# Adredes-weslee/elliptic-gnn-project

Measured on AMD Instinct MI355X. Metric: edges/s full-batch SAGE fwd+bwd, Elliptic 203k/234k/166-feat, 1→8 MI355X, higher is better.
Workload: dtype f32; 1 GPU; configs/sage.yaml + symmetrize_edges=true: SAGE 2L 166->128->2, dropout 0.5, full-batch train step (fwd+masked CE+bwd+clip+Adam); global_nodes=203769, global_edges=468710, feats=166, max_nodes_per_gpu=203769, max_edges_per_gpu=468710, parallelism=single, launch=hip-graph replay of the whole step

## Files before the change

elliptic_gnn_project_amd/_lib.py:

```python
from __future__ import annotations

import ctypes
import os
from pathlib import Path

import torch

PKG_DIR = Path(__file__).resolve().parent
LIB_PATH = Path(os.environ["GNNMP_LIB"]) if os.environ.get("GNNMP_LIB") else PKG_DIR / "libgnnmp.so"
ABI_VERSION = 32

DTYPE_F32 = 0
DTYPE_BF16 = 1

MATH_SPLIT_BF16 = 0
MATH_F32 = 1
MATH_HALF_PAIR = 2

PLANES_SPLIT_BF16 = 0
PLANES_HALF_PAIR = 1

GNN_OK = 0
_STATUS_EXC = {
    1: ValueError,
    2: IndexError,
    3: RuntimeError,
    4: RuntimeError,
    5: NotImplementedError,
}

LOOPS_KEEP = 0
LOOPS_REPLACE = 1

AGG_SUM = 0
AGG_MEAN = 1
AGG_MEAN_BWD = 2
AGG_GCN = 3
AGG_EDGE_W = 4

c_i64 = ctypes.c_int64
c_i32 = ctypes.c_int32
c_ptr = ctypes.c_void_p
c_size = ctypes.c_size_t


class GnnSplit(ctypes.Structure):
    _fields_ = [
        ("seg_len", c_i32),
        ("reserved", c_i32),
        ("num_long", c_i64),
        ("num_pieces", c_i64),
        ("ptr", c_ptr),
        ("nbr", c_ptr),
        ("piece0", c_ptr),
        ("piece_seg", c_ptr),
        ("long_seg", c_ptr),
        ("order", c_ptr),
    ]


class GnnGraph(ctypes.Structure):
    _fields_ = [
        ("num_nodes", c_i64),
        ("num_slots", c_i64),
        ("rowptr", c_ptr),
        ("col", c_ptr),
        ("colptr", c_ptr),
        ("row", c_ptr),
        ("csc2csr", c_ptr),
        ("csr_split", ctypes.POINTER(GnnSplit)),
        ("csc_split", ctypes.POINTER(GnnSplit)),
    ]


class GnnAggParams(ctypes.Structure):
    _fields_ = [
        ("mode", ctypes.c_int),
        ("transpose", c_i32),
        ("nodew", c_ptr),
        ("ew", c_ptr),
        ("heads", c_i32),
        ("addend", c_ptr),
        ("ld_add", c_i64),
        ("bias", c_ptr),
        ("relu", c_i32),
        ("part", c_ptr),
        ("part_bytes", c_size),
        ("dropout_p", ctypes.c_float),
        ("seed", ctypes.c_uint64),
        ("seed_ptr", c_ptr),
        ("addend2", c_ptr),
        ("ld_add2", c_i64),
    ]


class GnnGemmNTParams(ctypes.Structure):
    _fields_ = [
        ("M", c_i64), ("N", c_i64),
        ("a1", c_ptr), ("lda1", c_i64), ("k1", c_i64),
        ("a2", c_ptr), ("lda2", c_i64), ("k2", c_i64),
        ("bt", c_ptr), ("ldb", c_i64),
        ("w1", c_ptr), ("w2", c_ptr), ("ldw1", c_i64), ("ldw2", c_i64),
        ("c", c_ptr), ("ldc", c_i64),
        ("bias", c_ptr),
        ("relu", c_i32),
        ("dropout_p", ctypes.c_float),
        ("seed", ctypes.c_uint64),
        ("seed_ptr", c_ptr),
        ("proj", c_ptr), ("nproj", c_i32), ("z", c_ptr), ("ldz", c_i64),
        ("math", c_i32),
        ("workspace", c_ptr), ("workspace_bytes", c_size),
        ("a_dtype", c_i32), ("c_dtype", c_i32),
        ("mask", c_ptr), ("ldmask", c_i64), ("mask_scale", ctypes.c_float),
        ("a_planes", c_ptr), ("planes_ld", c_i64), ("planes_stride", c_i64), ("planes_col2", c_i64),
        ("planes_format", c_i32), ("keep_mask", c_ptr), ("b_ready", c_i32), ("planes_exp", c_i32),
        ("colsum_part", c_ptr), ("colsum_cap", c_i64),
        ("row_exp", c_ptr),
    ]


class GnnGemmTNParams(ctypes.Structure):
    _fields_ = [
        ("M", c_i64), ("Nr", c_i64),
        ("g", c_ptr), ("ldg", c_i64),
        ("dz", c_ptr), ("lddz", c_i64),
        ("proj", c_ptr), ("nproj", c_i32),
        ("h", c_ptr), ("ldh", c_i64), ("hscale", ctypes.c_float),
        ("gout", c_ptr), ("ldgout", c_i64),
        ("a1", c_ptr), ("lda1", c_i64), ("k1", c_i64),
        ("a2", c_ptr), ("lda2", c_i64), ("k2", c_i64),
        ("math", c_i32),
        ("a_dtype", c_i32), ("h_dtype", c_i32),
        ("a_planes", c_ptr), ("planes_ld", c_i64), ("planes_stride", c_i64), ("planes_col2", c_i64),
        ("planes_format", c_i32), ("g_dtype", c_i32), ("planes_exp", c_i32),
        ("sq_partial", c_ptr), ("sq_step", c_ptr), ("sq_skip_lo", c_i64), ("sq_skip_hi", c_i64), ("sq_cap", c_i64),
        ("row_exp", c_ptr),
        ("g_rowmax", c_ptr),
        ("dz_graph", c_ptr), ("dz_u", c_ptr), ("ldu", c_i64), ("dz_cols", c_i32),
    ]


RANK_TILE = 1024
RANK_BOOT_LDS_MAX_N = 32768
RANK_STATUS_NAN, RANK_STATUS_SEGMENT, RANK_STATUS_INDEX = 1, 2, 4
ROWMAX_ROWS = 16
ACTIVE_ROWS = 16


class GnnAggActive(ctypes.Structure):
    _fields_ = [("row_active", c_ptr), ("active_with", c_ptr), ("ld_active_with", c_i64), ("active_with_cols", c_i32)]


ACT_NONE = 0
ACT_ELU = 1


class GnnGatFwdParams(ctypes.Structure):
    _fields_ = [
        ("heads", c_i32), ("chans", c_i32), ("concat", c_i32),
        ("slope", ctypes.c_float),
        ("xh", c_ptr), ("ld_xh", c_i64),
        ("att_src", c_ptr), ("att_dst", c_ptr),
        ("bias", c_ptr),
        ("act", ctypes.c_int),
        ("dropout_p", ctypes.c_float),
        ("seed", ctypes.c_uint64), ("seed_ptr", c_ptr),
        ("a_src", c_ptr), ("a_dst", c_ptr),
        ("alpha", c_ptr),
        ("out", c_ptr), ("ldo", c_i64),
        ("edge_w", c_ptr),
        ("proj", c_ptr), ("nproj", c_i32), ("z", c_ptr), ("ldz", c_i64),
    ]


ADAM_MAX_TENSORS = 24
ADAM_SELF_MAX = 1 << 15


class GnnAdamTensor(ctypes.Structure):
    _fields_ = [("param", c_ptr), ("grad", c_ptr), ("exp_avg", c_ptr), ("exp_avg_sq", c_ptr), ("numel", c_i64)]


class GnnAdamGroup(ctypes.Structure):
    _fields_ = [
        ("num_tensors", c_i32),
        ("lr", ctypes.c_double), ("beta1", ctypes.c_double), ("beta2", ctypes.c_double), ("eps", ctypes.c_double),
        ("weight_decay", ctypes.c_double), ("max_norm", ctypes.c_double),
        ("tensors", GnnAdamTensor * ADAM_MAX_TENSORS),
        ("skip_nonfinite", c_i32),
        ("bump_counter", c_ptr),
        ("loss_partial", c_ptr), ("loss_nblk", c_i32), ("loss_scale", ctypes.c_float), ("loss_out", c_ptr),
        ("grad_sq_partial", c_ptr), ("grad_sq_nblk", c_i32),
    ]


class GnnCeSpec(ctypes.Structure):
    _fields_ = [
        ("y", c_ptr), ("mask", c_ptr), ("class_w", c_ptr), ("row_w", c_ptr),
        ("inv_denom", ctypes.c_float), ("focal", c_i32), ("focal_gamma", ctypes.c_float),
        ("reserved", c_i32 * 5),
    ]


EXPLAIN_STATUS_BLOCK = 1


FIT_THREADS = 1024
(FIT_STATUS_LABEL, FIT_STATUS_NAN, FIT_STATUS_EMPTY, FIT_STATUS_FLAT, FIT_STATUS_CLAMP_LOW, FIT_STATUS_CLAMP_HIGH,
 FIT_STATUS_MAXIT) = 1, 2, 4, 8, 16, 32, 64
CURVE_OUTPUTS = 8
CALIB_MAX_BINS = 32

REPORT_MAX_SEGMENTS = 2048
REPORT_STATUS_K, JOIN_STATUS_DUPLICATE, JOIN_STATUS_NEGATIVE, JOIN_STATUS_MISMATCH = 8, 16, 32, 64
ENSEMBLE_PROB, ENSEMBLE_LOGIT = 0, 1

LOGREG_MAX_D = 255
LOGREG_ROWS = 128
LOGREG_REDUCE_UNROLL = 4
ISOTONIC_CHUNK = 128
BASELINE_STATUS_ROW, BASELINE_STATUS_NAN = 1, 2

EPOCH_MAX_TENSORS = 64
EPOCH_CHUNK_BYTES = 16384


class GnnEpochTensor(ctypes.Structure):
    _fields_ = [("src", c_ptr), ("dst", c_ptr), ("bytes", c_i64)]


class GnnEpochTable(ctypes.Structure):
    _fields_ = [("num_tensors", c_i32), ("reserved", c_i32), ("tensors", GnnEpochTensor * EPOCH_MAX_TENSORS)]


class GnnEpochState(ctypes.Structure):
    _fields_ = [("epoch", c_i32), ("bad", c_i32), ("best_epoch", c_i32), ("stop_epoch", c_i32), ("status", c_i32),
                ("reserved", c_i32), ("best_val", ctypes.c_double)]


class GnnExplainStepParams(ctypes.Structure):
    _fields_ = [
        ("n", c_i64), ("F", c_i64),
        ("mask", c_ptr), ("ld_mask", c_i64),
        ("grad", c_ptr),
        ("dh", c_ptr), ("ld_dh", c_i64),
        ("x", c_ptr), ("ld_x", c_i64),
        ("h", c_ptr), ("ld_h", c_i64),
        ("exp_avg", c_ptr), ("exp_avg_sq", c_ptr), ("ld_state", c_i64),
        ("hard", c_ptr), ("hard_out", c_ptr), ("ld_hard", c_i64),
        ("block_of", c_ptr), ("num_blocks", c_i32), ("t", c_i32),
        ("size_scale", c_ptr), ("ent_scale", c_ptr),
        ("lr", ctypes.c_double), ("beta1", ctypes.c_double), ("beta2", ctypes.c_double), ("eps", ctypes.c_double),
        ("status", c_ptr),
    ]


SIGNATURES = {
    "gnn_abi_version": (ctypes.c_int, []),
    "gnn_status_string": (ctypes.c_char_p, [ctypes.c_int]),
    "gnn_last_error": (ctypes.c_char_p, []),
    "gnn_graph_workspace_size": (ctypes.c_int, [c_i64, c_i64, ctypes.POINTER(c_size)]),
    "gnn_graph_build": (
        ctypes.c_int,
        [c_ptr, c_i64, c_i64, ctypes.c_int, c_ptr, c_ptr, c_ptr, c_ptr, c_ptr, c_ptr, c_ptr, c_ptr, c_size, c_ptr],
    ),
    "gnn_split_workspace_size": (ctypes.c_int, [c_i64, ctypes.POINTER(c_size)]),
    "gnn_split_count": (ctypes.c_int, [c_ptr, c_i64, c_i32, c_ptr, c_ptr]),
    "gnn_split_build": (
        ctypes.c_int,
        [c_ptr, c_ptr, c_i64, c_i32, c_ptr, c_ptr, c_ptr, c_ptr, c_ptr, c_ptr, c_ptr, c_size, c_ptr],
    ),
    "gnn_in_degree_f32": (ctypes.c_int, [ctypes.POINTER(GnnGraph), c_ptr, c_ptr]),
    "gnn_gcn_norm_f32": (ctypes.c_int, [ctypes.POINTER(GnnGraph), c_ptr, c_ptr]),
    "gnn_aggregate_f32": (
        ctypes.c_int,
        [ctypes.POINTER(GnnGraph), ctypes.POINTER(GnnAggParams), c_ptr, c_i64, c_i64, c_ptr, c_i64, c_ptr],
    ),
    "gnn_aggregate_active_f32": (
        ctypes.c_int,
        [ctypes.POINTER(GnnGraph), ctypes.POINTER(GnnAggParams), c_ptr, c_i64, c_i64, c_ptr, c_i64,
         ctypes.POINTER(GnnAggActive), c_ptr],
    ),
    "gnn_aggregate_bf16": (
        ctypes.c_int,
        [ctypes.POINTER(GnnGraph), ctypes.POINTER(GnnAggParams), c_ptr, c_i64, c_i64, c_ptr, c_i64, c_ptr],
    ),
    "gnn_sage_mean_fwd_f32": (
        ctypes.c_int,
        [ctypes.POINTER(GnnGraph), c_ptr, c_ptr, c_i64, c_i64, c_ptr, c_i64, c_ptr],
    ),
    "gnn_split_planes_f32": (ctypes.c_int, [c_ptr, c_i64, c_i64, c_i64, c_ptr, c_i64, c_i64, c_i64, c_i64, c_ptr]),
    "gnn_sage_mean_fwd_planes": (
        ctypes.c_int,
        [ctypes.POINTER(GnnGraph), c_ptr, c_ptr, c_i64, c_i64, c_ptr, c_i64, c_i64, c_i64, c_ptr],
    ),
    "gnn_split_h2_f32": (ctypes.c_int, [c_ptr, c_i64, c_i64, c_i64, c_ptr, c_i64, c_i64, c_i64, c_i64, c_i32, c_ptr]),
    "gnn_sage_mean_fwd_h2": (
        ctypes.c_int,
        [ctypes.POINTER(GnnGraph), c_ptr, c_ptr, c_i64, c_i64, c_ptr, c_i64, c_i64, c_i64, c_i32,
         c_ptr, c_i64, ctypes.c_float, ctypes.c_uint64, c_ptr, ctypes.POINTER(GnnGemmNTParams),
         ctypes.POINTER(GnnSplit), c_ptr],
    ),
    "gnn_sage_out_mean_ce_f32": (
        ctypes.c_int,
        [ctypes.POINTER(GnnGraph), c_ptr, c_ptr, c_i64, c_i32, c_ptr, c_ptr, c_i64, c_ptr, c_ptr, c_ptr,
         ctypes.c_float, c_ptr, c_i64, c_ptr, c_i64, c_ptr, c_ptr, c_ptr, c_size, c_ptr],
    ),
    "gnn_sage_mean_bwd_f32": (
        ctypes.c_int,
        [ctypes.POINTER(GnnGraph), c_ptr, c_ptr, c_i64, c_i64, c_ptr, c_i64, c_ptr],
    ),
    "gnn_edge_dot_f32": (
        ctypes.c_int,
        [ctypes.POINTER(GnnGraph), c_ptr, c_ptr, c_ptr, c_i64, c_ptr, c_i64, c_i64, c_ptr, c_ptr],
    ),
    "gnn_gat_scores_f32": (
        ctypes.c_int,
        [c_i64, c_i32, c_i32, c_ptr, c_i64, c_ptr, c_ptr, c_ptr, c_ptr, c_ptr],
    ),
    "gnn_gat_fwd_f32": (
        ctypes.c_int,
        [ctypes.POINTER(GnnGraph), c_i32, c_i32, c_i32, ctypes.c_float, c_ptr, c_i64, c_ptr, c_ptr,
         c_ptr, c_ptr, c_ptr, c_i64, c_ptr],
    ),
    "gnn_gat_fwd_fused_f32": (ctypes.c_int, [ctypes.POINTER(GnnGraph), ctypes.POINTER(GnnGatFwdParams), c_ptr]),
    "gnn_gat_out_ce_f32": (
        ctypes.c_int,
        [ctypes.POINTER(GnnGraph), ctypes.POINTER(GnnGatFwdParams), c_ptr, c_ptr, c_ptr, ctypes.c_float, c_ptr, c_i64,
         c_ptr, c_ptr, c_ptr, c_size, c_ptr]),
    "gnn_gat_act_bwd_f32": (
        ctypes.c_int,
        [c_i64, c_i64, ctypes.c_int, ctypes.c_float, ctypes.c_uint64, c_ptr, c_ptr, c_i64, c_ptr, c_i64, c_ptr,
         c_i64, c_ptr],
    ),
    "gnn_gat_bwd_workspace_size": (ctypes.c_int, [c_i64, c_i64, c_i32, c_i32, ctypes.POINTER(c_size)]),
    "gnn_gat_bwd_f32": (
        ctypes.c_int,
        [ctypes.POINTER(GnnGraph), c_i32, c_i32, c_i32, ctypes.c_float, c_ptr, c_i64, c_ptr, c_ptr, c_ptr,
         c_ptr, c_ptr, c_ptr, c_i64, c_ptr, c_i64, c_ptr, c_ptr, c_ptr, c_size, c_ptr],
    ),
    "gnn_gat_bwd_act_proj_f32": (
        ctypes.c_int,
        [ctypes.POINTER(GnnGraph), c_i32, c_i32, ctypes.c_float, c_ptr, c_i64, c_ptr, c_ptr, c_ptr, c_ptr, c_ptr,
         c_i32, ctypes.c_float, ctypes.c_uint64, c_ptr, c_ptr, c_i64, c_ptr, c_i64, c_ptr, c_i32, c_ptr, c_i64,
         c_ptr, c_i64, c_ptr, c_ptr, c_ptr, c_ptr, c_size, c_ptr]),
    "gnn_gat_bwd_act_f32": (
        ctypes.c_int,
        [ctypes.POINTER(GnnGraph), c_i32, c_i32, ctypes.c_float, c_ptr, c_i64, c_ptr, c_ptr, c_ptr, c_ptr, c_ptr,
         c_i32, ctypes.c_float, ctypes.c_uint64, c_ptr, c_ptr, c_i64, c_ptr, c_i64, c_ptr, c_i64, c_ptr, c_i64,
         c_ptr, c_ptr, c_ptr, c_size, c_ptr],
    ),
    "gnn_gat_bwd_ew_f32": (
        ctypes.c_int,
        [ctypes.POINTER(GnnGraph), c_i32, c_i32, c_i32, ctypes.c_float, c_ptr, c_i64, c_ptr, c_ptr, c_ptr,
         c_ptr, c_ptr, c_ptr, c_i64, c_ptr, c_i64, c_ptr, c_ptr, c_ptr, c_ptr, c_ptr, c_size, c_ptr],
    ),
    "gnn_gemm_nt_workspace_size": (ctypes.c_int, [c_i64, c_i64, c_i64, ctypes.POINTER(c_size)]),
    "gnn_gemm_nt_f32": (ctypes.c_int, [ctypes.POINTER(GnnGemmNTParams), c_ptr]),
    "gnn_gemm_nt_prep_b": (ctypes.c_int, [ctypes.POINTER(GnnGemmNTParams), c_ptr]),
    "gnn_masked_ce_finish": (ctypes.c_int, [c_ptr, c_i32, ctypes.c_float, c_ptr, c_ptr]),
    "gnn_gemm_tn_workspace_size": (ctypes.c_int, [c_i64, c_i64, c_i64, c_i32, ctypes.POINTER(c_size)]),
    "gnn_gemm_tn_sq_blocks": (ctypes.c_int, [c_i64, ctypes.POINTER(c_i32)]),
    "gnn_gemm_tn_f32": (ctypes.c_int, [ctypes.POINTER(GnnGemmTNParams), c_ptr, c_ptr, c_size, c_ptr]),
    "gnn_gemm_tn_active_f32": (ctypes.c_int, [ctypes.POINTER(GnnGemmTNParams), c_ptr, c_ptr, c_ptr, c_size, c_ptr]),
    "gnn_gemm_tn_active_pays": (ctypes.c_int, [c_i64]),
    "gnn_gemm_tn_active_split": (ctypes.c_int, []),
    "gnn_gemm_tn_active_ring": (ctypes.c_int, []),
    "gnn_gemm_nt_planes_ok": (ctypes.c_int, [ctypes.POINTER(GnnGemmNTParams)]),
    "gnn_gemm_nt_colsum_blocks": (ctypes.c_int, [ctypes.POINTER(GnnGemmNTParams), ctypes.POINTER(c_i32)]),
    "gnn_colsum_finish_f32": (ctypes.c_int, [c_ptr, c_i32, c_i64, c_ptr, c_ptr]),
    "gnn_gemm_tn_planes_ok": (ctypes.c_int, [ctypes.POINTER(GnnGemmTNParams)]),
    "gnn_colsum_workspace_size": (ctypes.c_int, [c_i64, c_i64, ctypes.POINTER(c_size)]),
    "gnn_colsum_f32": (ctypes.c_int, [c_i64, c_i64, c_ptr, c_i64, c_ptr, c_ptr, c_size, c_ptr]),
    "gnn_masked_ce_workspace_size": (ctypes.c_int, [c_i64, ctypes.POINTER(c_size)]),
    "gnn_masked_ce_f32": (
        ctypes.c_int,
        [c_i64, c_i32, c_ptr, c_i64, c_ptr, c_ptr, c_ptr, ctypes.c_float, c_ptr, c_i64, c_ptr, c_ptr, c_size, c_ptr],
    ),
    "gnn_gcn_out_ce_f32": (
        ctypes.c_int,
        [ctypes.POINTER(GnnGraph), c_ptr, c_ptr, c_i64, c_i32, c_ptr, c_ptr, c_i64, c_ptr, c_ptr, c_ptr,
         ctypes.c_float, c_ptr, c_i64, c_ptr, c_ptr, c_ptr, c_size, c_ptr],
    ),
    "gnn_masked_ce_colsum_f32": (
        ctypes.c_int,
        [c_i64, c_i32, c_ptr, c_i64, c_ptr, c_ptr, c_ptr, ctypes.c_float, c_ptr, c_i64, c_ptr, c_ptr, c_size, c_ptr,
         c_ptr],
    ),
    "gnn_masked_ce_spec_f32": (
        ctypes.c_int,
        [c_i64, c_i32, c_ptr, c_i64, ctypes.POINTER(GnnCeSpec), c_ptr, c_i64, c_ptr, c_ptr, c_size, c_ptr, c_ptr],
    ),
    "gnn_sage_out_mean_ce_spec_f32": (
        ctypes.c_int,
        [ctypes.POINTER(GnnGraph), c_ptr, c_ptr, c_i64, c_i32, c_ptr, c_ptr, c_i64, ctypes.POINTER(GnnCeSpec),
         c_ptr, c_i64, c_ptr, c_i64, c_ptr, c_ptr, c_ptr, c_size, c_ptr],
    ),
    "gnn_gcn_out_ce_spec_f32": (
        ctypes.c_int,
        [ctypes.POINTER(GnnGraph), c_ptr, c_ptr, c_i64, c_i32, c_ptr, c_ptr, c_i64, ctypes.POINTER(GnnCeSpec),
         c_ptr, c_i64, c_ptr, c_ptr, c_ptr, c_size, c_ptr],
    ),
    "gnn_gat_out_ce_spec_f32": (
        ctypes.c_int,
        [ctypes.POINTER(GnnGraph), ctypes.POINTER(GnnGatFwdParams), ctypes.POINTER(GnnCeSpec), c_ptr, c_i64,
         c_ptr, c_ptr, c_ptr, c_size, c_ptr]),
    "gnn_clip_adam_workspace_size": (ctypes.c_int, [ctypes.POINTER(c_size)]),
    "gnn_neighbor_sample_workspace_size": (ctypes.c_int, [c_i64, c_i64, c_i64, ctypes.POINTER(c_size)]),
    "gnn_neighbor_sample": (
        ctypes.c_int,
        [ctypes.POINTER(GnnGraph), c_ptr, c_ptr, c_i64, c_i32, c_ptr, ctypes.c_uint64, c_ptr, c_i64, c_ptr, c_ptr,
         c_ptr, c_i64, c_ptr, c_ptr, c_ptr, c_size, c_ptr],
    ),
    "gnn_clip_adam_f32": (ctypes.c_int, [ctypes.POINTER(GnnAdamGroup), c_ptr, c_ptr, c_ptr, c_size, c_ptr]),
    "gnn_clip_adam_prep_f32": (ctypes.c_int, [ctypes.POINTER(GnnAdamGroup), c_ptr, c_ptr, c_ptr, c_size,
                                              ctypes.POINTER(GnnGemmNTParams), c_i32, c_ptr]),
    "gnn_bn_workspace_size": (ctypes.c_int, [c_i64, ctypes.POINTER(c_size)]),
    "gnn_bn_stats_f32": (
        ctypes.c_int,
        [c_ptr, c_i64, c_i64, c_i64, c_ptr, c_i32, ctypes.c_float, ctypes.c_float, c_ptr, c_ptr, c_ptr, c_ptr,
         c_ptr, c_ptr, c_size, c_ptr],
    ),
    "gnn_bn_finalize_f32": (
        ctypes.c_int, [c_ptr, c_i64, ctypes.c_float, ctypes.c_float, c_ptr, c_ptr, c_ptr, c_ptr, c_ptr, c_ptr],
    ),
    "gnn_bn_act_res_fwd_f32": (
        ctypes.c_int,
        [c_ptr, c_i64, c_ptr, c_i64, c_i64, c_i64, c_ptr, c_ptr, c_ptr, c_ptr, ctypes.c_float, ctypes.c_uint64,
         c_ptr, c_ptr, c_i64, c_ptr],
    ),
    "gnn_bn_act_bwd_reduce_f32": (
        ctypes.c_int,
        [c_ptr, c_i64, c_ptr, c_i64, c_i64, c_i64, c_ptr, c_ptr, c_ptr, c_ptr, ctypes.c_float, ctypes.c_uint64,
         c_ptr, c_ptr, c_ptr, c_size, c_ptr],
    ),
    "gnn_bn_act_bwd_f32": (
        ctypes.c_int,
        [c_ptr, c_i64, c_ptr, c_i64, c_i64, c_i64, c_ptr, c_ptr, c_ptr, c_ptr, ctypes.c_float, ctypes.c_uint64,
         c_ptr, c_ptr, c_ptr, c_ptr, c_i64, c_ptr],
    ),
    "gnn_bn_act_bwd_colsum_blocks": (ctypes.c_int, [c_i64, c_i64, ctypes.POINTER(c_i32)]),
    "gnn_bn_act_bwd_colsum_f32": (
        ctypes.c_int,
        [c_ptr, c_i64, c_ptr, c_i64, c_i64, c_i64, c_ptr, c_ptr, c_ptr, c_ptr, ctypes.c_float, ctypes.c_uint64,
         c_ptr, c_ptr, c_ptr, c_ptr, c_i64, c_ptr, c_ptr],
    ),
    "gnn_time_inject_sin_f32": (
        ctypes.c_int,
        [c_ptr, c_i64, c_i64, c_i64, c_ptr, c_i64, c_i64, c_ptr, c_i64, c_ptr],
    ),
    "gnn_rank_plan_workspace_size": (ctypes.c_int, [c_i64, c_i64, ctypes.POINTER(c_size)]),
    "gnn_rank_plan_build": (
        ctypes.c_int,
        [c_ptr, c_ptr, c_ptr, c_i64, c_i64, c_ptr, c_ptr, c_ptr, c_ptr, c_ptr, c_ptr, c_size, c_ptr],
    ),
    "gnn_rank_ap_workspace_size": (ctypes.c_int, [c_i64, c_i64, ctypes.POINTER(c_size)]),
    "gnn_rank_ap": (
        ctypes.c_int,
        [c_ptr, c_ptr, c_ptr, c_ptr, c_i64, c_i64, c_i64, c_ptr, c_ptr, c_ptr, c_ptr, c_ptr, c_size, c_ptr],
    ),
    "gnn_rank_bootstrap_workspace_size": (ctypes.c_int, [c_i64, c_i64, ctypes.POINTER(c_size)]),
    "gnn_rank_bootstrap": (
        ctypes.c_int,
        [c_ptr, c_ptr, c_ptr, c_ptr, c_ptr, c_ptr, c_ptr, c_ptr, c_i64, c_i64, c_i64, c_ptr, c_ptr, c_ptr, c_ptr,
         c_ptr, c_ptr, c_size, c_ptr],
    ),
    "gnn_edge_drop_workspace_size": (ctypes.c_int, [c_i64, ctypes.POINTER(c_size)]),
    "gnn_edge_drop": (ctypes.c_int, [c_ptr, c_i64, c_i64, ctypes.c_uint64, c_ptr, c_ptr, c_size, c_ptr]),
    "gnn_feature_noise_f32": (
        ctypes.c_int, [c_ptr, c_i64, c_i64, c_i64, ctypes.c_float, ctypes.c_uint64, c_ptr, c_i64, c_ptr]),
    "gnn_explain_mask_step_f32": (ctypes.c_int, [ctypes.POINTER(GnnExplainStepParams), c_ptr]),
    "gnn_temperature_fit_workspace_size": (ctypes.c_int, [c_i64, ctypes.POINTER(c_size)]),
    "gnn_temperature_fit": (
        ctypes.c_int, [c_ptr, c_i64, c_ptr, c_ptr, c_i64, c_ptr, c_ptr, c_ptr, c_ptr, c_size, c_ptr]),
    "gnn_rank_curve_workspace_size": (ctypes.c_int, [c_i64, ctypes.POINTER(c_size)]),
    "gnn_rank_curve": (
        ctypes.c_int,
        [c_ptr, c_ptr, c_ptr, c_ptr, c_ptr, c_i64, c_i64, ctypes.c_double, c_ptr, c_ptr, c_size, c_ptr]),
    "gnn_threshold_calibration_workspace_size": (ctypes.c_int, [c_i64, c_i32, ctypes.POINTER(c_size)]),
    "gnn_threshold_calibration": (
        ctypes.c_int,
        [c_ptr, c_ptr, c_ptr, c_i64, ctypes.c_double, ctypes.POINTER(ctypes.c_double), c_i32, c_ptr, c_ptr, c_ptr,
         c_ptr, c_ptr, c_ptr, c_size, c_ptr]),
    "gnn_hub_rank_workspace_size": (ctypes.c_int, [c_i64, c_i64, ctypes.POINTER(c_size)]),
    "gnn_hub_rank": (ctypes.c_int, [c_ptr, c_i64, c_i64, c_ptr, c_ptr, c_ptr, c_ptr, c_ptr, c_ptr, c_size, c_ptr]),
    "gnn_hub_ablate_workspace_size": (ctypes.c_int, [c_i64, ctypes.POINTER(c_size)]),
    "gnn_hub_ablate": (ctypes.c_int, [c_ptr, c_i64, c_ptr, c_i64, c_i64, c_ptr, c_ptr, c_size, c_ptr]),
    "gnn_rank_hits_at_workspace_size": (ctypes.c_int, [c_i64, ctypes.POINTER(c_size)]),
    "gnn_rank_hits_at": (
        ctypes.c_int, [c_ptr, c_ptr, c_ptr, c_i64, c_i64, c_ptr, c_i64, c_ptr, c_ptr, c_ptr, c_ptr, c_ptr, c_size, c_ptr]),
    "gnn_segment_threshold_counts_workspace_size": (ctypes.c_int, [c_i64, c_i64, ctypes.POINTER(c_size)]),
    "gnn_segment_threshold_counts": (
        ctypes.c_int, [c_ptr, c_ptr, c_ptr, c_ptr, c_i64, c_i64, ctypes.c_double, c_ptr, c_ptr, c_ptr, c_size, c_ptr]),
    "gnn_id_join_workspace_size": (ctypes.c_int, [c_i64, ctypes.POINTER(c_size)]),
    "gnn_id_join": (ctypes.c_int, [c_ptr, c_ptr, c_i64, c_ptr, c_ptr, c_ptr, c_size, c_ptr]),
    "gnn_ensemble_pair": (ctypes.c_int, [c_ptr, c_ptr, c_ptr, c_i64, c_i32, c_ptr, c_ptr, c_ptr]),
    "gnn_column_moments_workspace_size": (ctypes.c_int, [c_i64, c_i64, ctypes.POINTER(c_size)]),
    "gnn_column_moments": (
        ctypes.c_int, [c_ptr, c_i64, c_i64, c_ptr, c_i64, c_i64, c_ptr, c_ptr, c_ptr, c_ptr, c_size, c_ptr]),
    "gnn_logreg_eval_workspace_size": (ctypes.c_int, [c_i64, c_i64, ctypes.POINTER(c_size)]),
    "gnn_logreg_eval": (
        ctypes.c_int,
        [c_ptr, c_i64, c_i64, c_ptr, c_i64, c_i64, c_ptr, c_ptr, c_ptr, ctypes.c_double, ctypes.c_double,
         ctypes.c_double, c_ptr, c_i32, c_ptr, c_ptr, c_ptr, c_ptr, c_ptr, c_size, c_ptr]),
    "gnn_logreg_predict": (
        ctypes.c_int, [c_ptr, c_i64, c_i64, c_ptr, c_i64, c_i64, c_ptr, c_ptr, c_ptr, c_ptr, c_ptr, c_ptr, c_ptr]),
    "gnn_isotonic_fit_workspace_size": (ctypes.c_int, [c_i64, ctypes.POINTER(c_size)]),
    "gnn_isotonic_fit": (
        ctypes.c_int, [c_ptr, c_ptr, c_ptr, c_ptr, c_ptr, c_i64, c_i64, c_ptr, c_ptr, c_ptr, c_ptr, c_size, c_ptr]),
    "gnn_isotonic_apply": (ctypes.c_int, [c_ptr, c_ptr, c_ptr, c_ptr, c_i64, c_ptr, c_ptr, c_ptr, c_ptr]),
    "gnn_epoch_keep_best": (
        ctypes.c_int, [c_ptr, c_ptr, c_ptr, ctypes.POINTER(GnnEpochTable), c_i32, c_i32, c_ptr, c_ptr, c_ptr, c_ptr]),
}

_LIB: ctypes.CDLL | None = None


class GnnmpError(RuntimeError):
    pass


def load() -> ctypes.CDLL:
    global _LIB
    if _LIB is not None:
        return _LIB
    if not LIB_PATH.exists():
        raise GnnmpError(
            f"{LIB_PATH} not found: build it with `make -C {PKG_DIR / 'csrc'}` "
            "(or __graft_entry__.build()).  The MI355X kernels are required; there is no CPU fallback."
        )
    lib = ctypes.CDLL(str(LIB_PATH), mode=ctypes.RTLD_GLOBAL)
    for name, (res, args) in SIGNATURES.items():
        fn = getattr(lib, name)
        fn.restype = res
        fn.argtypes = args
    ver = lib.gnn_abi_version()
    if ver != ABI_VERSION:
        raise GnnmpError(f"libgnnmp ABI {ver} != expected {ABI_VERSION}; rebuild the library")
    _LIB = lib
    return lib


def check(status: int, what: str = "") -> None:
    if status == GNN_OK:
        return
    lib = load()
    msg = lib.gnn_last_error().decode(errors="replace")
    kind = lib.gnn_status_string(status).decode()
    exc = _STATUS_EXC.get(status, GnnmpError)
    raise exc(f"libgnnmp {what or 'call'} failed ({kind}): {msg}")


def stream_handle(device: torch.device | None = None) -> int:
    return torch.cuda.current_stream(device).cuda_stream


def ptr(t: torch.Tensor | None) -> int | None:
    return None if t is None else t.data_ptr()


CALLS = [0]


def call(name: str, *args) -> None:
    lib = load()
    CALLS[0] += 1
    check(getattr(lib, name)(*args), name)
```

elliptic_gnn_project_amd/csrc/gemm_common.hpp:

```cpp
#pragma once
#include "common.hpp"

#include <utility>

typedef float floatx16 __attribute__((ext_vector_type(16)));

namespace gnnmp {

template <typename F, int... I>
__device__ __forceinline__ void static_for_impl(F&& f, std::integer_sequence<int, I...>) {
  (f(std::integral_constant<int, I>{}), ...);
}
template <int N, typename F>
__device__ __forceinline__ void static_for(F&& f) {
  static_for_impl(f, std::make_integer_sequence<int, N>{});
}

namespace gemm {
inline bool aligned(const void* ptr, int bytes) { return (reinterpret_cast<uintptr_t>(ptr) % bytes) == 0; }
}

template <int V, int... Vs, typename F>
void with_rung(int v, F&& f) {
  if constexpr (sizeof...(Vs) == 0) f(std::integral_constant<int, V>{});
  else if (v <= V) f(std::integral_constant<int, V>{});
  else with_rung<Vs...>(v, f);
}

constexpr uint32_t kDropGolden = 0x9E3779B1u;
__device__ __forceinline__ bool keep_premixed(uint32_t h, uint64_t seed, uint32_t keep_thresh) {
  h ^= (uint32_t)(seed >> 32);
  h ^= h >> 16;
  h *= 0x85EBCA6Bu;
  h ^= h >> 13;
  h *= 0xC2B2AE35u;
  h ^= h >> 16;
  return (h >> 8) < keep_thresh;
}
__device__ __forceinline__ bool keep_elem(uint64_t seed, uint32_t idx, uint32_t keep_thresh) {
  uint32_t h = idx * kDropGolden + (uint32_t)seed;
  h ^= (uint32_t)(seed >> 32);
  h ^= h >> 16;
  h *= 0x85EBCA6Bu;
  h ^= h >> 13;
  h *= 0xC2B2AE35u;
  h ^= h >> 16;
  return (h >> 8) < keep_thresh;
}

constexpr int BN = 128;

struct NTArgs {
  int64_t M;
  int32_t Nc;
  const float* a1; int64_t lda1; int32_t k1;
  const float* a2; int64_t lda2; int32_t k2;
  const float* bt; int64_t ldb;
  const float* w1; const float* w2; int64_t ldw1, ldw2;
  int32_t wvec2;
  int32_t wvec;
  float* c; int64_t ldc;
  const float* bias;
  int32_t relu;
  int32_t dropout; uint32_t keep_thresh; float drop_scale; uint64_t seed; const uint64_t* seed_ptr;
  const float* proj; int32_t nproj; float* z; int64_t ldz;
  int32_t a_bf16;
  int32_t c_bf16;
  const float* mask; int64_t ldmask; float mask_scale;
  const uint16_t* ap; int32_t ap_ld; int32_t ap_col2; int64_t ap_ps;
  int32_t ap_h2;
  int32_t ap_exp;
  const uint32_t* kmask;
  float* colsum_part;
  int32_t* rowexp;
};

struct H2Prep {
  const float* w1; const float* w2;
  int64_t ldw1, ldw2;
  int32_t k1, k2, Nc, col2;
  int32_t blocks;
  uint4* img; float* colscale;
  float a_unscale;
  int32_t gblocks;
};

__device__ __forceinline__ float bf16_to_f32(uint16_t b) { return __uint_as_float((uint32_t)b << 16); }
__device__ __forceinline__ uint16_t f32_to_bf16(float f) {
  return __builtin_bit_cast(uint16_t, (__bf16)f);
}

template <bool CBF = false>
__device__ __forceinline__ void nt_epilogue(const NTArgs& a, floatx16 (&acc)[4], int64_t m0, int n0, int lane,
                                            int wave, uint64_t seed) {
#pragma unroll
  for (int once = 0; once < 1; ++once) {
    const int64_t rbase = m0 + wave * 32 + 4 * (lane >> 5);
    const uint32_t hstep = (uint32_t)a.Nc * kDropGolden;
#pragma unroll
    for (int t = 0; t < 4; ++t) {
      const int col = n0 + t * 32 + (lane & 31);
      const bool colok = col < a.Nc;
      const float bv = (a.bias && colok) ? a.bias[col] : 0.0f;
      const uint32_t h0 = ((uint32_t)rbase * (uint32_t)a.Nc + (uint32_t)col) * kDropGolden + (uint32_t)seed;
#pragma unroll
      for (int r = 0; r < 16; ++r) {
        const int64_t row = rbase + (r & 3) + 8 * (r >> 2);
        float v = acc[t][r] + bv;
        if (a.relu) v = fmaxf(v, 0.0f);
        if (a.dropout)
          v = keep_premixed(h0 + (uint32_t)((r & 3) + 8 * (r >> 2)) * hstep, seed, a.keep_thresh) ? v * a.drop_scale
                                                                                                 : 0.0f;
        if (!colok) v = 0.0f;
        if constexpr (CBF) {
          const uint16_t b = f32_to_bf16(v);
          v = bf16_to_f32(b);
          if (a.c && row < a.M && colok) reinterpret_cast<uint16_t*>(a.c)[row * a.ldc + col] = b;
        } else {
          if (a.c && row < a.M && colok) a.c[row * a.ldc + col] = v;
        }
        acc[t][r] = v;
      }
    }
    if (a.nproj > 0) {
      float pw[4][4];
#pragma unroll
      for (int q = 0; q < 4; ++q)
#pragma unroll
        for (int t = 0; t < 4; ++t) {
          const int col = n0 + t * 32 + (lane & 31);
          pw[q][t] = (q < a.nproj && col < a.Nc) ? a.proj[(int64_t)q * a.Nc + col] : 0.0f;
        }
      const bool hi16 = lane & 16, hi8 = lane & 8;
      const int qsel = (hi16 ? 2 : 0) + (hi8 ? 1 : 0);
#pragma unroll
      for (int r = 0; r < 16; ++r) {
        float ps[4];
#pragma unroll
        for (int q = 0; q < 4; ++q) {
          float sum = acc[0][r] * pw[q][0];
          sum = fmaf(acc[1][r], pw[q][1], sum);
          sum = fmaf(acc[2][r], pw[q][2], sum);
          ps[q] = fmaf(acc[3][r], pw[q][3], sum);
        }
        const float s0 = hi16 ? ps[0] : ps[2], s1 = hi16 ? ps[1] : ps[3];
        const float k0 = (hi16 ? ps[2] : ps[0]) + __shfl_xor(s0, 16);
        const float k1 = (hi16 ? ps[3] : ps[1]) + __shfl_xor(s1, 16);
        float m = (hi8 ? k1 : k0) + __shfl_xor(hi8 ? k0 : k1, 8);
        m += __shfl_xor(m, 4);
        m += __shfl_xor(m, 2);
        m += __shfl_xor(m, 1);
        const int64_t row = rbase + (r & 3) + 8 * (r >> 2);
        if ((lane & 7) == 0 && qsel < a.nproj && row < a.M) a.z[row * a.ldz + qsel] = m;
      }
    }
  }
}

constexpr int TN_THREADS = 1024;
constexpr int KT_PER_WAVE = 3;
constexpr int KMAX = 4 * KT_PER_WAVE * 32;
constexpr int TN_APITCH = KMAX;
constexpr int MAXPROJ = 4;

struct TNArgs {
  int64_t M;
  int32_t Nr;
  const float* g; int64_t ldg;
  const float* dz; int64_t lddz; const float* proj; int32_t nproj;
  const float* h; int64_t ldh; float hscale;
  float* gout; int64_t ldgout;
  const float* a1; int64_t lda1; int32_t k1;
  const float* a2; int64_t lda2; int32_t k2;
  float* slab; int64_t slab_stride;
  int64_t rows_per_block;
  int32_t want_db;
  int32_t a_bf16;
  int32_t h_bf16;
  int32_t g_bf16;
  const uint16_t* ap; int32_t ap_ld; int32_t ap_col2; int64_t ap_ps;
  int32_t ap_h2;
  int32_t ap_exp;
  const int32_t* rowexp;
  const uint32_t* growmax;
  const int32_t* cptr; const int32_t* cnbr; const float* cu; int64_t ldu; int32_t ccols;
  const uint8_t* dz_active;
  int32_t slab_empty;
};
template <typename F>
void tn_forms(const TNArgs& a, F&& f) {
  auto pick = [](bool v, auto&& g) { if (v) g(std::true_type{}); else g(std::false_type{}); };
  pick(a.dz != nullptr, [&](auto proj) {
    pick(a.h != nullptr, [&](auto mask) { pick(a.gout != nullptr, [&](auto gout) { f(proj, mask, gout); }); });
  });
}

template <typename Args>
bool image_cols_ok(const Args& a) {
  return gemm::aligned(a.ap, 16) && a.k1 >= 1 && a.k1 <= a.ap_col2 && a.ap_col2 % 8 == 0 && a.ap_col2 + a.k2 <= a.ap_ld;
}
template <typename Args>
bool image_planes_ok(const Args& a, int planes) {
  return a.ap_ps >= a.M * (int64_t)a.ap_ld && planes * a.ap_ps * 2 < ((int64_t)1 << 31);
}

constexpr int TN_ACT_CAP = 512;

void launch_nt_f32(const NTArgs& a, int avec, hipStream_t st);
void launch_tn_f32(const TNArgs& a, int nblk, hipStream_t st);
constexpr int kRedOut = 16;
void launch_slab_reduce(const float* slab, int64_t stride, int nred, float* out, int64_t n_out,
                        const gnn_gemm_tn_params* sq, hipStream_t st, bool empty = false);

void launch_nt_x3(const NTArgs& a, void* ws, size_t ws_bytes, hipStream_t st);
size_t nt_x3_workspace(int64_t k1, int64_t k2);
void launch_tn_x3(const TNArgs& a, int nblk, hipStream_t st);
bool nt_h2s_ok(const NTArgs& a);
size_t nt_h2s_workspace(int64_t k1, int64_t k2);
void launch_nt_h2s(const NTArgs& a, void* ws, hipStream_t st);
bool tn_h2s_ok(const TNArgs& a);
void launch_tn_h2s(const TNArgs& a, int nblk, hipStream_t st);

bool nt_ws_ok(const NTArgs& a);
size_t nt_ws_tail_offset(int64_t k1, int64_t k2);
void launch_nt_ws(const NTArgs& a, uint4* img, hipStream_t st);
bool nt_planes_ok(const NTArgs& a);
constexpr int NT_PHASE_PREP = 1, NT_PHASE_RUN = 2, NT_PHASE_ALL = 3;
void launch_nt_ws_planes(const NTArgs& a, uint4* img, hipStream_t st, int phase = NT_PHASE_ALL);
bool nt_img16_ok(const NTArgs& a);
void launch_nt_img16(const NTArgs& a, uint4* img, hipStream_t st, int phase = NT_PHASE_ALL);
bool nt_h2_ok(const NTArgs& a);
H2Prep h2_prep_of(const NTArgs& a, uint4* img);
gnn_status nt_h2_prep_from_params(const gnn_gemm_nt_params* p, H2Prep* out, const char* fn);
void launch_nt_h2(const NTArgs& a, uint4* img, hipStream_t st, int phase = NT_PHASE_ALL);
void launch_prep_h2(const H2Prep& p, hipStream_t st);
bool tn_h2_ok(const TNArgs& a);
constexpr int TN_ACT_SPLIT = 4, TN_ACT_RING = 1;
void launch_tn_h2(const TNArgs& a, int nblk, hipStream_t st, bool ks = false, bool act_split = false);
bool tn_planes_ok(const TNArgs& a);
void launch_tn_planes(const TNArgs& a, int nblk, hipStream_t st);
bool tn_img16_ok(const TNArgs& a);
void launch_tn_img16(const TNArgs& a, int nblk, hipStream_t st);
__device__ __forceinline__ void split3_pair(float a, float b, uint32_t& h, uint32_t& m, uint32_t& l) {
  typedef __bf16 bf16x2_ __attribute__((ext_vector_type(2)));
  typedef float f32x2_ __attribute__((ext_vector_type(2)));
  h = __builtin_bit_cast(uint32_t, __builtin_convertvector(f32x2_{a, b}, bf16x2_));
  a -= __uint_as_float(h << 16);
  b -= __uint_as_float(h & 0xffff0000u);
  m = __builtin_bit_cast(uint32_t, __builtin_convertvector(f32x2_{a, b}, bf16x2_));
  a -= __uint_as_float(m << 16);
  b -= __uint_as_float(m & 0xffff0000u);
  l = __builtin_bit_cast(uint32_t, __builtin_convertvector(f32x2_{a, b}, bf16x2_));
}

__device__ __forceinline__ void split_h2_pair(float a, float b, uint32_t& h, uint32_t& l) {
  typedef _Float16 h2_ __attribute__((ext_vector_type(2)));
  typedef float f32x2_ __attribute__((ext_vector_type(2)));
  const h2_ hv = __builtin_convertvector(f32x2_{a, b}, h2_);
  h = __builtin_bit_cast(uint32_t, hv);
  const float ra = (a - (float)hv[0]) * 2048.0f;
  const float rb = (b - (float)hv[1]) * 2048.0f;
  l = __builtin_bit_cast(uint32_t, __builtin_convertvector(f32x2_{ra, rb}, h2_));
}

__device__ __forceinline__ uint32_t h2_scale_pair(uint32_t h, float s) {
  typedef _Float16 h2_ __attribute__((ext_vector_type(2)));
  typedef float f32x2_ __attribute__((ext_vector_type(2)));
  const h2_ v = __builtin_bit_cast(h2_, h);
  return __builtin_bit_cast(uint32_t, __builtin_convertvector(f32x2_{(float)v[0] * s, (float)v[1] * s}, h2_));
}

enum NTSkinny { SKINNY_NONE, SKINNY_N, SKINNY_K };
NTSkinny nt_skinny_form(const NTArgs& a);
void launch_nt_skinny(const NTArgs& a, hipStream_t st);
int nt_skinny_k_blocks(const NTArgs& a);
int tn_skinny_blocks(int64_t M);
bool tn_skinny_ok(const TNArgs& a);
void launch_tn_skinny(const TNArgs& a, int nblk, hipStream_t st);


__device__ __forceinline__ float h2_col_exp2(float m) {
  if (!(m > 0.f) || !isfinite(m)) return 1.0f;
  int E;
  frexpf(m, &E);
  return ldexpf(1.0f, E - 4);
}
template <int NW>
__device__ __forceinline__ void ws_prep_h2_finish(const H2Prep& a, int n, const float (&v)[12]) {
  constexpr int ROW = 16 * 24 + 4;
  __shared__ float wrow[NW][ROW];
  const int lane = threadIdx.x & 63, wave = threadIdx.x >> 6;
  const bool live = n < a.Nc;
  float* row = wrow[wave];
  const int ncols = 16 * a.blocks;
  for (int kk = lane; kk < ncols; kk += 64) row[kk] = 0.f;
  float m = 0.f;
#pragma unroll
  for (int i = 0; i < 6; ++i) {
    m = fmaxf(m, lane + 64 * i < a.k1 ? fabsf(v[i]) : 0.f);
    m = fmaxf(m, lane + 64 * i < a.k2 ? fabsf(v[6 + i]) : 0.f);
  }
#pragma unroll
  for (int o = 32; o >= 1; o >>= 1) m = fmaxf(m, __shfl_xor(m, o));
  const float sc = live ? h2_col_exp2(m) : 1.0f;
  if (lane == 0) a.colscale[n] = sc * (1.0f / 2048.0f) * a.a_unscale;
#pragma unroll
  for (int i = 0; i < 6; ++i) {
    const int k = lane + 64 * i;
    if (live && k < a.k1) row[k] = v[i];
    if (live && k < a.k2) row[a.col2 + k] = v[6 + i];
  }
  __builtin_amdgcn_s_waitcnt(0xc07f);
  __builtin_amdgcn_wave_barrier();
  const float inv = 1.0f / sc;
  for (int q = lane; q < 2 * a.blocks; q += 64) {
    const int s = q >> 1, kh = q & 1;
    uint32_t hw[4], lw[4], pw[4];
#pragma unroll
    for (int j = 0; j < 4; ++j) {
      const float v0 = row[16 * s + 8 * kh + 2 * j] * inv, v1 = row[16 * s + 8 * kh + 2 * j + 1] * inv;
      split_h2_pair(v0, v1, hw[j], lw[j]);
      pw[j] = h2_scale_pair(hw[j], 2048.0f);
    }
    const int64_t slot = 2 * n + kh;
    a.img[((int64_t)s * 3 + 0) * 256 + slot] = make_uint4(pw[0], pw[1], pw[2], pw[3]);
    a.img[((int64_t)s * 3 + 1) * 256 + slot] = make_uint4(hw[0], hw[1], hw[2], hw[3]);
    a.img[((int64_t)s * 3 + 2) * 256 + slot] = make_uint4(lw[0], lw[1], lw[2], lw[3]);
  }
}
template <int NTH>
__device__ __forceinline__ void ws_prep_h2_cols(const H2Prep& a, int blk) {
  constexpr int NW = NTH / 64;
  const int lane = threadIdx.x & 63, wave = threadIdx.x >> 6;
  const int n = blk * NW + wave;
  if (n >= BN) return;
  const int nc = n < a.Nc ? n : 0;
  const int k1m = a.k1 - 1, k2m = a.k2 > 0 ? a.k2 - 1 : 0;
  const float* w1 = a.w1 + (int64_t)nc * a.ldw1;
  const float* w2 = (a.w2 ? a.w2 : a.w1) + (int64_t)nc * (a.w2 ? a.ldw2 : a.ldw1);
  float v[12];
#pragma unroll
  for (int i = 0; i < 6; ++i) {
    v[i] = w1[min(lane + 64 * i, k1m)];
    v[6 + i] = w2[min(lane + 64 * i, k2m)];
  }
  ws_prep_h2_finish<NW>(a, n, v);
}
constexpr int WS_PREP_THREADS = 1024;

}
```

elliptic_gnn_project_amd/csrc/gemm_dispatch.hip:

```cpp
#include "common.hpp"

#include <algorithm>
#include <cstdlib>

#include "gemm_common.hpp"

using namespace gnnmp;
using gemm::aligned;

namespace {

bool bad_dtype(int32_t d) { return d != GNN_DTYPE_F32 && d != GNN_DTYPE_BF16; }
bool bad_math(int32_t m) { return m != GNN_MATH_SPLIT_BF16 && m != GNN_MATH_F32 && m != GNN_MATH_HALF_PAIR; }

template <typename P, typename A>
void image_args(const P* p, A* a) {
  if (!p->a_planes) return;
  a->ap = static_cast<const uint16_t*>(p->a_planes);
  a->ap_ld = (int32_t)std::min<int64_t>(p->planes_ld, INT32_MAX);
  a->ap_col2 = (int32_t)std::min<int64_t>(p->planes_col2, INT32_MAX);
  a->ap_ps = p->planes_stride;
  a->ap_h2 = p->planes_format == GNN_PLANES_HALF_PAIR;
  a->ap_exp = a->ap_h2 ? p->planes_exp : 0;
}
template <typename P>
const char* image_args_bad(const P* p) {
  if (!p->a_planes) return nullptr;
  if (p->planes_format != GNN_PLANES_SPLIT_BF16 && p->planes_format != GNN_PLANES_HALF_PAIR) return "bad planes_format";
  if (p->planes_format == GNN_PLANES_HALF_PAIR && (p->planes_exp < -100 || p->planes_exp > 100))
    return "planes_exp outside [-100, 100]";
  return nullptr;
}


gnn_status nt_args(const gnn_gemm_nt_params* p, NTArgs* out, const char* fn) {
  if (!p) return fail(GNN_ERR_INVALID_ARG, fn, "null params");
  NTArgs a{};
  a.M = p->M; a.Nc = (int32_t)p->N;
  a.a1 = p->a1; a.lda1 = p->lda1; a.k1 = (int32_t)p->k1;
  a.a2 = p->a2; a.lda2 = p->lda2; a.k2 = (int32_t)p->k2;
  a.bt = p->bt; a.ldb = p->ldb; a.w1 = p->w1; a.w2 = p->w2; a.ldw1 = p->ldw1; a.ldw2 = p->ldw2; a.c = p->c;
  a.ldc = p->ldc; a.bias = p->bias; a.relu = p->relu;
  a.dropout = p->dropout_p > 0.f;
  a.keep_thresh = (uint32_t)((1.0 - (double)p->dropout_p) * 16777216.0);
  a.drop_scale = a.dropout ? (float)(1.0 / (1.0 - (double)p->dropout_p)) : 1.0f;
  a.seed = p->seed; a.seed_ptr = p->seed_ptr;
  a.proj = p->proj; a.nproj = p->nproj; a.z = p->z; a.ldz = p->ldz;
  a.wvec2 = a.w1 && (a.ldw1 % 2 == 0) && (a.k1 % 2 == 0) && aligned(a.w1, 8) &&
            (a.k2 == 0 || ((a.ldw2 % 2 == 0) && (a.k2 % 2 == 0) && aligned(a.w2, 8)));
  auto wv = [&](int v) {
    return a.w1 && (a.ldw1 % v == 0) && (a.k1 % v == 0) && aligned(a.w1, 4 * v) &&
           (a.k2 == 0 || ((a.ldw2 % v == 0) && (a.k2 % v == 0) && aligned(a.w2, 4 * v)));
  };
  a.wvec = wv(4) ? 4 : (wv(2) ? 2 : 1);
  a.a_bf16 = p->a_dtype == GNN_DTYPE_BF16; a.c_bf16 = p->c_dtype == GNN_DTYPE_BF16;
  a.mask = p->mask; a.ldmask = p->ldmask; a.mask_scale = p->mask_scale;
  image_args(p, &a);
  a.kmask = p->a_planes ? p->keep_mask : nullptr; a.colsum_part = p->colsum_part; a.rowexp = p->row_exp;
  *out = a;
  if (!fn) return GNN_OK;

  const bool planes_only = p->a_planes && !p->a1;
  if (p->M < 0 || p->N < 1 || p->k1 < 1 || p->k2 < 0 || (!p->a1 && !p->a_planes) ||
      (p->k2 > 0 && !p->a2 && !planes_only))
    return fail(GNN_ERR_INVALID_ARG, fn, "bad shapes / null operands");
  if (!p->bt && !(p->w1 && (p->k2 == 0 || p->w2)))
    return fail(GNN_ERR_INVALID_ARG, fn, "need bt or w1 (and w2 when k2 > 0)");
  if (p->w1 && (p->N > BN || p->ldw1 < p->k1 || (p->k2 > 0 && p->ldw2 < p->k2)))
    return fail(GNN_ERR_INVALID_ARG, fn, "w1/w2 form needs N <= 128 and ldw >= k");
  if ((!planes_only && (p->lda1 < p->k1 || (p->k2 > 0 && p->lda2 < p->k2))) || (p->bt && p->ldb < p->N) ||
      (p->c && p->ldc < p->N))
    return fail(GNN_ERR_INVALID_ARG, fn, "bad leading dimensions");
  if (p->nproj < 0 || p->nproj > 4 || (p->nproj > 0 && (p->N > BN || !p->proj || !p->z || p->ldz < p->nproj)))
    return fail(GNN_ERR_INVALID_ARG, fn, "projection needs N <= 128, nproj <= 4, proj and z");
  if (p->dropout_p < 0.f || p->dropout_p >= 1.f) return fail(GNN_ERR_INVALID_ARG, fn, "dropout p in [0,1)");
  if (p->dropout_p > 0.f && (int64_t)p->M * (int64_t)p->N >= ((int64_t)1 << 32))
    return fail(GNN_ERR_UNSUPPORTED, fn, "dropout element index (rows x width) must be < 2^32");
  if (bad_math(p->math)) return fail(GNN_ERR_INVALID_ARG, fn, "bad math mode");
  if (bad_dtype(p->a_dtype) || bad_dtype(p->c_dtype)) return fail(GNN_ERR_INVALID_ARG, fn, "bad dtype");
  if (p->M == 0) return GNN_OK;
  if (p->mask && p->ldmask < p->N) return fail(GNN_ERR_INVALID_ARG, fn, "bad ldmask");
  if (const char* why = image_args_bad(p)) return fail(GNN_ERR_INVALID_ARG, fn, why);
  if (a.kmask && (!a.ap_h2 || !a.dropout || !aligned(a.kmask, 4)))
    return fail(GNN_ERR_INVALID_ARG, fn, "keep_mask needs a half-pair image A and dropout_p > 0");
  return GNN_OK;
}

enum NTKernel {
  NT_NONE, NT_IMG_H2, NT_IMG_BF16, NT_IMG_SPLIT,
  NT_SKINNY_N, NT_SKINNY_K, NT_X3_BF16, NT_H2S, NT_X3, NT_F32_V4, NT_F32_V2, NT_F32_V1
};
struct NTPick { NTKernel kernel; gnn_status status; const char* why; };

NTPick nt_select(const gnn_gemm_nt_params* p, const NTArgs& a, int phase) {
  auto run = [](NTKernel k) { return NTPick{k, GNN_OK, nullptr}; };
  auto no = [](gnn_status s, const char* why) { return NTPick{NT_NONE, s, why}; };
  auto ws = [&](size_t need) { return p->workspace && p->workspace_bytes >= need; };
  if (p->row_exp && (p->a_planes || p->colsum_part || phase != NT_PHASE_ALL))
    return no(GNN_ERR_UNSUPPORTED, "row_exp needs the in-kernel half-pair NT over f32 A1 / A2");
  if (a.M == 0 && phase != NT_PHASE_PREP) return run(NT_NONE);
  const NTSkinny skinny = nt_skinny_form(a);
  if (p->colsum_part) {
    if (skinny != SKINNY_K || p->a_planes || phase != NT_PHASE_ALL)
      return no(GNN_ERR_UNSUPPORTED, "colsum_part needs the skinny-K form (k1 <= 8, k2 = 0, 8 < N <= 256)");
    if (p->colsum_cap < (int64_t)nt_skinny_k_blocks(a) * p->N || !aligned(p->colsum_part, 4))
      return no(GNN_ERR_INVALID_ARG, "colsum_cap < gnn_gemm_nt_colsum_blocks x N");
    return run(NT_SKINNY_K);
  }
  const bool split = p->math != GNN_MATH_F32;
  if (p->a_planes) {
    const bool img = split && !p->mask, planes_only = !p->a1;
    const size_t img_bytes = (size_t)(a.ap_ld / 16) * 3 * 256 * sizeof(uint4);
    if (a.ap_h2) {
      if (img && nt_h2_ok(a) && ws(img_bytes + BN * sizeof(float))) return run(NT_IMG_H2);
      if (planes_only) return no(GNN_ERR_UNSUPPORTED, "half-pair image A outside the half-pair kernel's shapes");
    }
    if (a.a_bf16) {
      if (img && nt_img16_ok(a) && ws(img_bytes)) return run(NT_IMG_BF16);
      return no(GNN_ERR_UNSUPPORTED, "bf16 image A outside the image kernel's shapes");
    }
    if (img && nt_planes_ok(a) && ws(img_bytes)) return run(NT_IMG_SPLIT);
    if (planes_only) return no(GNN_ERR_UNSUPPORTED, "split-image A outside the planes kernel's shapes");
  }
  if (phase != NT_PHASE_ALL)
    return no(phase == NT_PHASE_PREP ? GNN_ERR_UNSUPPORTED : GNN_ERR_INVALID_ARG,
              "a separate B prep (prep_b / b_ready) needs an image-A kernel (gnn_gemm_nt_planes_ok)");
  const bool h2s = p->math == GNN_MATH_HALF_PAIR && nt_h2s_ok(a) && ws(nt_h2s_workspace(a.k1, a.k2));
  if (p->row_exp && !h2s)
    return no(GNN_ERR_UNSUPPORTED, "row_exp needs the in-kernel half-pair NT (GNN_MATH_HALF_PAIR, the w1/w2 "
                                   "form, N <= 128, k1 / k2 multiples of 16, k1 + k2 <= 128, f32, a workspace)");
  if (!p->row_exp && skinny != SKINNY_NONE)
    return run(skinny == SKINNY_N ? NT_SKINNY_N : NT_SKINNY_K);
  if (p->mask) return no(GNN_ERR_UNSUPPORTED, "the mask epilogue needs a skinny shape (K <= 8 or N <= 8)");
  if (a.a_bf16 || a.c_bf16) {
    if (!a.a_bf16 || !a.w1 || a.Nc > BN || !split)
      return no(GNN_ERR_UNSUPPORTED, "bf16 NT needs bf16 A, the w1/w2 form, N <= 128 and split math");
    return run(NT_X3_BF16);
  }
  if (h2s) return run(NT_H2S);
  if (split && a.w1 && a.Nc <= BN) return run(NT_X3);
  auto av = [&](int v) {
    return (a.k1 % v == 0) && (a.lda1 % v == 0) && aligned(a.a1, 4 * v) &&
           (a.k2 == 0 || ((a.k2 % v == 0) && (a.lda2 % v == 0) && aligned(a.a2, 4 * v)));
  };
  return run(av(4) ? NT_F32_V4 : av(2) ? NT_F32_V2 : NT_F32_V1);
}

NTPick nt_select_query(const gnn_gemm_nt_params* p, NTArgs* a, bool colsum) {
  gnn_gemm_nt_params q = *p;
  q.workspace = &q; q.workspace_bytes = SIZE_MAX; q.b_ready = 0;
  if (colsum) { q.colsum_part = reinterpret_cast<float*>(&q); q.colsum_cap = INT64_MAX; }
  nt_args(&q, a, nullptr);
  return nt_select(&q, *a, NT_PHASE_ALL);
}

gnn_status gemm_nt_dispatch(const gnn_gemm_nt_params* p, gnn_stream_t stream, const char* fn, int phase) {
  NTArgs a;
  if (const gnn_status s = nt_args(p, &a, fn)) return s;
  if (phase == NT_PHASE_ALL && p->b_ready) phase = NT_PHASE_RUN;
  const NTPick k = nt_select(p, a, phase);
  if (k.why) return fail(k.status, fn, k.why);
  hipStream_t st = (hipStream_t)stream;
  uint4* img = static_cast<uint4*>(p->workspace);
  if (k.kernel > NT_IMG_SPLIT) a.ap = nullptr;
  switch (k.kernel) {
    case NT_NONE: return GNN_OK;
    case NT_IMG_H2: launch_nt_h2(a, img, st, phase); break;
    case NT_IMG_BF16: launch_nt_img16(a, img, st, phase); break;
    case NT_IMG_SPLIT: launch_nt_ws_planes(a, img, st, phase); break;
    case NT_SKINNY_N:
    case NT_SKINNY_K: launch_nt_skinny(a, st); break;
    case NT_X3_BF16:
    case NT_X3: launch_nt_x3(a, p->workspace, p->workspace_bytes, st); break;
    case NT_H2S: launch_nt_h2s(a, p->workspace, st); break;
    default: launch_nt_f32(a, k.kernel == NT_F32_V4 ? 4 : k.kernel == NT_F32_V2 ? 2 : 1, st); break;
  }
  return hip_check(hipGetLastError(), fn);
}

}

extern "C" gnn_status gnn_gemm_nt_workspace_size(int64_t N, int64_t k1, int64_t k2, size_t* bytes) {
  if (!bytes || N < 1 || k1 < 1 || k2 < 0) return fail(GNN_ERR_INVALID_ARG, __func__, "bad args");
  *bytes = N <= BN ? std::max(nt_x3_workspace(k1, k2), (size_t)21 * 3 * 256 * 16 + BN * sizeof(float)) : 0;
  return GNN_OK;
}

extern "C" gnn_status gnn_gemm_nt_f32(const gnn_gemm_nt_params* p, gnn_stream_t stream) {
  return gemm_nt_dispatch(p, stream, __func__, NT_PHASE_ALL);
}
extern "C" gnn_status gnn_gemm_nt_prep_b(const gnn_gemm_nt_params* p, gnn_stream_t stream) {
  return gemm_nt_dispatch(p, stream, __func__, NT_PHASE_PREP);
}

extern "C" gnn_status gnn_gemm_nt_colsum_blocks(const gnn_gemm_nt_params* p, int32_t* nb) {
  if (!p || !nb) return fail(GNN_ERR_INVALID_ARG, __func__, "null");
  NTArgs a;
  *nb = nt_select_query(p, &a, true).kernel == NT_SKINNY_K ? nt_skinny_k_blocks(a) : 0;
  return GNN_OK;
}

extern "C" int gnn_gemm_nt_planes_ok(const gnn_gemm_nt_params* p) {
  if (!p || !p->a_planes) return 0;
  NTArgs a;
  const NTKernel k = nt_select_query(p, &a, false).kernel;
  return k >= NT_IMG_H2 && k <= NT_IMG_SPLIT;
}

namespace gnnmp {
gnn_status nt_h2_prep_from_params(const gnn_gemm_nt_params* p, H2Prep* out, const char* fn) {
  NTArgs a;
  if (const gnn_status s = nt_args(p, &a, fn)) return s;
  if (nt_select(p, a, NT_PHASE_PREP).kernel != NT_IMG_H2 || !aligned(p->workspace, 16))
    return fail(GNN_ERR_UNSUPPORTED, fn, "prep_b needs NT params that select the half-pair NT (and its workspace)");
  *out = h2_prep_of(a, static_cast<uint4*>(p->workspace));
  return GNN_OK;
}
}


namespace {

struct TNRows { int blocks; int64_t rows; };
TNRows tn_rows(int64_t M, int cap) {
  const int64_t chunks = ceil_div(M, 32);
  if (chunks <= 0) return {1, 0};
  const int64_t per = ceil_div(chunks, cap);
  return {(int)ceil_div(chunks, per), per * 32};
}
constexpr int kTnBlocks = 256, kTnBlocksNarrow = 768;
bool tn_narrow(int64_t Nr, int64_t Kc, int32_t nproj) { return Nr <= 64 && Kc <= 128 && !nproj; }

int64_t tn_ksplit_max_m() {
  static const int64_t v = [] {
    const char* e = std::getenv("GNNMP_TN_KSPLIT_MAXM");
    return e ? std::atoll(e) : (int64_t)32768;
  }();
  return v;
}
TNRows tn_dz_rows(int64_t M) { return tn_rows(M, M <= tn_ksplit_max_m() ? kTnBlocks / 2 : kTnBlocks); }

bool tn_wave_per_group(int64_t rows_per_block) { return (rows_per_block + 63) / 64 + 1 <= 8; }
bool tn_csc_in_kernel(int64_t rows_per_block) {
  static const int v = [] {
    const char* e = std::getenv("GNNMP_TN_CSC_INKERNEL");
    return e ? std::atoi(e) : -1;
  }();
  if (rows_per_block > 1792) return false;
  if (v >= 0) return v != 0;
  return tn_wave_per_group(rows_per_block);
}
bool tn_active_pays(int64_t M) { return M >= 16 && !tn_wave_per_group(tn_dz_rows(M).rows); }
int64_t tn_active_bytes(int64_t M) { return (ceil_div(M, GNN_ACTIVE_ROWS) + 15) / 16 * 16; }
bool env_off(const char* name) {
  const char* e = std::getenv(name);
  return e && e[0] == '0' && !e[1];
}
bool tn_active_split() { return !env_off("GNNMP_TN_ACTIVE_SPLIT"); }
bool tn_empty_skip() { return !env_off("GNNMP_TN_EMPTY_SKIP"); }

int64_t tn_out_floats(int64_t Nr, int64_t Kc, int32_t nproj) { return Nr * Kc + Nr + (int64_t)nproj * Nr + nproj; }
int64_t tn_slab_stride(int64_t n_out) { return (n_out + 63) / 64 * 64; }
unsigned red_blocks(int64_t n_out) { return (unsigned)ceil_div(ceil_div(n_out, 4), kRedOut); }

gnn_status tn_args(const gnn_gemm_tn_params* p, TNArgs* out, const char* fn) {
  TNArgs a{};
  a.M = p->M; a.Nr = (int32_t)p->Nr;
  a.g = p->g; a.ldg = p->ldg; a.dz = p->dz; a.lddz = p->lddz; a.proj = p->proj; a.nproj = p->dz ? p->nproj : 0;
  a.h = p->h; a.ldh = p->ldh; a.hscale = p->hscale;
  a.gout = p->gout; a.ldgout = p->ldgout;
  a.a1 = p->a1; a.lda1 = p->lda1; a.k1 = (int32_t)p->k1;
  a.a2 = p->a2; a.lda2 = p->lda2; a.k2 = (int32_t)p->k2;
  a.slab_stride = tn_slab_stride(tn_out_floats(p->Nr, p->k1 + p->k2, a.nproj));
  a.rows_per_block = tn_rows(p->M, kTnBlocks).rows;
  a.a_bf16 = p->a_dtype == GNN_DTYPE_BF16; a.h_bf16 = p->h_dtype == GNN_DTYPE_BF16; a.g_bf16 = p->g_dtype == GNN_DTYPE_BF16;
  image_args(p, &a);
  a.growmax = (a.ap_h2 && !a.dz && a.g) ? p->g_rowmax : nullptr;
  a.rowexp = p->row_exp;
  if (const gnn_graph* cg = p->dz_graph) {
    a.cptr = cg->colptr; a.cnbr = cg->row; a.cu = p->dz_u; a.ldu = p->ldu; a.ccols = p->dz_cols;
  }
  *out = a;
  if (!fn) return GNN_OK;

  if (p->M < 0 || p->Nr < 1 || p->Nr > 128 || p->k1 < 1 || p->k2 < 0 || p->k1 + p->k2 > KMAX)
    return fail(GNN_ERR_UNSUPPORTED, fn, "needs 1 <= Nr <= 128 and k1 + k2 <= 384");
  const bool planes_only = p->a_planes && !p->a1;
  if (!planes_only && (!p->a1 || (p->k2 > 0 && !p->a2) || p->lda1 < p->k1 || (p->k2 > 0 && p->lda2 < p->k2)))
    return fail(GNN_ERR_INVALID_ARG, fn, "bad A operands");
  if (p->dz) {
    if (p->nproj < 1 || p->nproj > MAXPROJ || !p->proj || p->lddz < p->nproj)
      return fail(GNN_ERR_INVALID_ARG, fn, "dz form needs 1 <= nproj <= 4 and proj");
  } else if (!p->g || p->ldg < p->Nr) {
    return fail(GNN_ERR_INVALID_ARG, fn, "need g (or dz + proj)");
  }
  if (p->h && p->ldh < p->Nr) return fail(GNN_ERR_INVALID_ARG, fn, "bad ldh");
  if (bad_math(p->math)) return fail(GNN_ERR_INVALID_ARG, fn, "bad math mode");
  if (p->gout && p->ldgout < p->Nr) return fail(GNN_ERR_INVALID_ARG, fn, "bad ldgout");
  return GNN_OK;
}

enum TNKernel { TN_IMG_H2, TN_IMG_BF16, TN_IMG_SPLIT, TN_SKINNY, TN_H2S, TN_X3, TN_F32 };
enum TNCsc { TN_CSC_READ, TN_CSC_IN_KERNEL, TN_CSC_CALL_SIDE };
enum TNFlags { TN_FLAGS_NONE, TN_FLAGS_CALLER, TN_FLAGS_WORKSPACE };
struct TNPlan {
  TNKernel kernel;
  int blocks, nred;
  int64_t rows_per_block;
  bool ksplit;
  bool act_split;
  bool empty;
  TNCsc csc;
  TNFlags flags;
  size_t flags_off;
  gnn_status status; const char* why;
};

TNPlan tn_plan(const gnn_gemm_tn_params* p, const TNArgs& a, size_t ws_bytes, const uint8_t* dz_active) {
  TNPlan pl{};
  auto run = [&](TNKernel k) { pl.kernel = k; return pl; };
  auto no = [&](gnn_status s, const char* why) { pl.status = s; pl.why = why; return pl; };
  auto rows = [&](TNRows r) { pl.blocks = pl.nred = r.blocks; pl.rows_per_block = r.rows; };
  const size_t slab_bytes = (size_t)a.slab_stride * sizeof(float);
  rows(tn_rows(a.M, kTnBlocks));
  const size_t slabs_end = (size_t)pl.blocks * slab_bytes;
  const gnn_graph* cg = p->dz_graph;
  if (cg && (!p->dz || !p->dz_u || !cg->colptr || !cg->row || cg->num_nodes != p->M || p->dz_cols < 1 ||
             p->dz_cols > 2 || p->dz_cols > p->nproj || p->ldu < p->dz_cols))
    return no(GNN_ERR_INVALID_ARG, "dz_graph needs the dz form, dz_u, 1 <= dz_cols <= 2 and num_nodes == M");
  if (bad_dtype(p->a_dtype) || bad_dtype(p->h_dtype) || bad_dtype(p->g_dtype)) return no(GNN_ERR_INVALID_ARG, "bad dtype");
  if (a.g_bf16 && !(a.ap && a.a_bf16))
    return no(GNN_ERR_UNSUPPORTED, "bf16 g / gout need the bf16-image TN (a bf16 a_planes)");
  if (a.h_bf16 && !a.a_bf16) return no(GNN_ERR_UNSUPPORTED, "bf16 h needs bf16 A");
  if (const char* why = image_args_bad(p)) return no(GNN_ERR_INVALID_ARG, why);
  const bool split = p->math != GNN_MATH_F32, planes_only = a.ap && !a.a1;
  if (a.ap_h2) {
    if (dz_active && !(tn_h2_ok(a) && a.dz && !a.gout && !a.cptr))
      return no(GNN_ERR_UNSUPPORTED, "dz_active outside the half-pair dz-form TN's shapes");
    if (split && tn_h2_ok(a)) {
      if (a.dz) rows(tn_dz_rows(a.M));
      pl.csc = !a.cptr ? TN_CSC_READ : tn_csc_in_kernel(pl.rows_per_block) ? TN_CSC_IN_KERNEL : TN_CSC_CALL_SIDE;
      if (dz_active) {
        pl.flags = TN_FLAGS_CALLER;
      } else if (pl.csc == TN_CSC_CALL_SIDE && tn_active_pays(a.M)) {
        pl.flags = TN_FLAGS_WORKSPACE;
        pl.flags_off = slabs_end;
        if (ws_bytes < slabs_end + (size_t)tn_active_bytes(a.M) || !aligned(a.slab, 16))
          return no(GNN_ERR_WORKSPACE, "workspace too small for the activity flags (gnn_gemm_tn_workspace_size)");
      }
      if (pl.flags != TN_FLAGS_NONE && pl.rows_per_block / GNN_ACTIVE_ROWS > TN_ACT_CAP)
        return no(GNN_ERR_UNSUPPORTED, "dz_active: row block beyond the chunk list's capacity");
      pl.ksplit = a.dz && a.M <= tn_ksplit_max_m() && pl.flags == TN_FLAGS_NONE;
      if (pl.ksplit) pl.blocks = 2 * pl.nred;
      if (pl.flags != TN_FLAGS_NONE) {
        pl.act_split = tn_active_split();
        if (pl.act_split) pl.blocks = TN_ACT_SPLIT * pl.nred;
        pl.empty = tn_empty_skip() && a.slab_stride > tn_out_floats(a.Nr, a.k1 + a.k2, a.nproj);
      }
      return run(TN_IMG_H2);
    }
    if (planes_only) return no(GNN_ERR_UNSUPPORTED, "half-pair image A outside the half-pair kernel's shapes");
  }
  if (a.cptr)
    return no(GNN_ERR_UNSUPPORTED, "dz_graph outside the half-pair dz-form TN (gnn_gemm_tn_planes_ok)");
  if (a.ap && !a.ap_h2) {
    if (a.a_bf16) {
      if (!split || !tn_img16_ok(a)) return no(GNN_ERR_UNSUPPORTED, "bf16 image A outside the image kernel's shapes");
      return run(TN_IMG_BF16);
    }
    if (split && tn_planes_ok(a)) return run(TN_IMG_SPLIT);
    if (planes_only) return no(GNN_ERR_UNSUPPORTED, "split-image A outside the planes kernel's shapes");
  }
  if (tn_skinny_ok(a)) {
    pl.blocks = pl.nred = tn_skinny_blocks(a.M);
    if (ws_bytes < (size_t)pl.blocks * slab_bytes) return no(GNN_ERR_WORKSPACE, "workspace too small");
    return run(TN_SKINNY);
  }
  const int64_t ldmax = std::max({a.lda1, a.k2 > 0 ? a.lda2 : 0, a.h ? a.ldh : 0, a.g ? a.ldg : 0, a.dz ? a.lddz : 0});
  const bool off32 = (a.M + 32) * ldmax < ((int64_t)1 << 31);
  if (a.a_bf16 && (!split || !off32 || a.M < 16))
    return no(GNN_ERR_UNSUPPORTED, "bf16 TN needs split math, M >= 16 and M*ld < 2^31");
  if (p->math == GNN_MATH_HALF_PAIR && tn_h2s_ok(a) && off32) {
    const TNRows narrow = tn_rows(a.M, kTnBlocksNarrow);
    if (tn_narrow(a.Nr, a.k1 + a.k2, a.nproj) && ws_bytes >= (size_t)narrow.blocks * slab_bytes) rows(narrow);
    return run(TN_H2S);
  }
  if (split && off32 && a.M >= 16) return run(TN_X3);
  return run(TN_F32);
}

gnn_status gemm_tn_dispatch(const gnn_gemm_tn_params* p, float* out, void* workspace, size_t workspace_bytes,
                            gnn_stream_t stream, const uint8_t* dz_active = nullptr) {
  const char* fn = dz_active ? "gnn_gemm_tn_active_f32" : "gnn_gemm_tn_f32";
  if (!p || !out) return fail(GNN_ERR_INVALID_ARG, fn, "null params/out");
  if (dz_active) {
    if (!p->dz || !p->h || p->gout || p->dz_graph || !p->a_planes || p->planes_format != GNN_PLANES_HALF_PAIR ||
        p->math == GNN_MATH_F32 || p->M < 16)
      return fail(GNN_ERR_UNSUPPORTED, fn, "dz_active needs the half-pair dz form with h, no gout, no dz_graph, M >= 16");
    if (!aligned(dz_active, 16)) return fail(GNN_ERR_INVALID_ARG, fn, "dz_active must be 16-byte aligned");
  }
  TNArgs a;
  if (const gnn_status s = tn_args(p, &a, fn)) return s;
  a.slab = static_cast<float*>(workspace);
  const int64_t n_out = tn_out_floats(a.Nr, a.k1 + a.k2, a.nproj);
  if (!workspace || workspace_bytes < (size_t)tn_rows(a.M, kTnBlocks).blocks * a.slab_stride * sizeof(float))
    return fail(GNN_ERR_WORKSPACE, fn, "workspace too small");
  if (p->sq_partial && (!p->sq_step || p->sq_cap < 2 * (int64_t)red_blocks(n_out) + 1 || p->sq_skip_lo > p->sq_skip_hi))
    return fail(GNN_ERR_INVALID_ARG, fn, "sq_partial needs sq_step, sq_cap >= 2 nb + 1, skip_lo <= skip_hi");
  hipStream_t st = (hipStream_t)stream;
  if (p->M == 0) {
    if (!p->sq_partial) return hip_check(hipMemsetAsync(out, 0, n_out * sizeof(float), st), fn);
    launch_slab_reduce(a.slab, a.slab_stride, 0, out, n_out, p, st);
    return hip_check(hipGetLastError(), fn);
  }
  const TNPlan pl = tn_plan(p, a, workspace_bytes, dz_active);
  if (pl.why) return fail(pl.status, fn, pl.why);
  uint8_t* ws_flags = pl.flags == TN_FLAGS_WORKSPACE ? static_cast<uint8_t*>(workspace) + pl.flags_off : nullptr;
  if (pl.csc == TN_CSC_CALL_SIDE) {
    gnn_agg_params ag{};
    ag.mode = GNN_AGG_SUM; ag.transpose = 1;
    gnn_agg_active act{ws_flags, p->dz + p->dz_cols, p->lddz, a.nproj - p->dz_cols};
    const gnn_status s = gnn_aggregate_active_f32(p->dz_graph, &ag, p->dz_u, p->ldu, p->dz_cols,
                                                  const_cast<float*>(p->dz), p->lddz, &act, stream);
    if (s != GNN_OK) return s;
    a.cptr = nullptr;
  }
  a.rows_per_block = pl.rows_per_block;
  a.dz_active = pl.flags == TN_FLAGS_CALLER ? dz_active : ws_flags;
  a.slab_empty = pl.empty;
  if (pl.kernel >= TN_SKINNY) a.ap = nullptr;
  if (pl.kernel <= TN_SKINNY) a.rowexp = nullptr;
  switch (pl.kernel) {
    case TN_IMG_H2: launch_tn_h2(a, pl.blocks, st, pl.ksplit, pl.act_split); break;
    case TN_IMG_BF16: launch_tn_img16(a, pl.blocks, st); break;
    case TN_IMG_SPLIT: launch_tn_planes(a, pl.blocks, st); break;
    case TN_SKINNY: launch_tn_skinny(a, pl.blocks, st); break;
    case TN_H2S: launch_tn_h2s(a, pl.blocks, st); break;
    case TN_X3: launch_tn_x3(a, pl.blocks, st); break;
    case TN_F32: launch_tn_f32(a, pl.blocks, st); break;
  }
  if (const gnn_status s = hip_check(hipGetLastError(), fn)) return s;
  launch_slab_reduce(a.slab, a.slab_stride, pl.nred, out, n_out, p, st, pl.empty);
  return hip_check(hipGetLastError(), fn);
}

}

extern "C" gnn_status gnn_gemm_tn_workspace_size(int64_t M, int64_t Nr, int64_t Kc, int32_t nproj, size_t* bytes) {
  if (!bytes || M < 0 || Nr < 1 || Kc < 1 || nproj < 0) return fail(GNN_ERR_INVALID_ARG, __func__, "bad args");
  int64_t nb = tn_rows(M, kTnBlocks).blocks;
  if (Nr <= 8 && nproj == 0) nb = std::max<int64_t>(nb, tn_skinny_blocks(M));
  if (tn_narrow(Nr, Kc, nproj)) nb = std::max<int64_t>(nb, tn_rows(M, kTnBlocksNarrow).blocks);
  *bytes = (size_t)nb * tn_slab_stride(tn_out_floats(Nr, Kc, nproj)) * sizeof(float);
  if (nproj > 0 && tn_active_pays(M)) *bytes += (size_t)tn_active_bytes(M);
  return GNN_OK;
}

extern "C" int gnn_gemm_tn_active_pays(int64_t M) { return tn_active_pays(M) ? 1 : 0; }
extern "C" int gnn_gemm_tn_active_split(void) { return TN_ACT_SPLIT; }
extern "C" int gnn_gemm_tn_active_ring(void) { return TN_ACT_RING; }
extern "C" gnn_status gnn_gemm_tn_sq_blocks(int64_t n_out, int32_t* nb) {
  if (!nb || n_out < 1) return fail(GNN_ERR_INVALID_ARG, __func__, "bad args");
  *nb = (int32_t)red_blocks(n_out);
  return GNN_OK;
}

extern "C" gnn_status gnn_gemm_tn_f32(const gnn_gemm_tn_params* p, float* out, void* workspace,
                                      size_t workspace_bytes, gnn_stream_t stream) {
  return gemm_tn_dispatch(p, out, workspace, workspace_bytes, stream);
}
extern "C" gnn_status gnn_gemm_tn_active_f32(const gnn_gemm_tn_params* p, const uint8_t* dz_active, float* out,
                                             void* workspace, size_t workspace_bytes, gnn_stream_t stream) {
  return gemm_tn_dispatch(p, out, workspace, workspace_bytes, stream, dz_active);
}

extern "C" int gnn_gemm_tn_planes_ok(const gnn_gemm_tn_params* p) {
  if (!p || !p->a_planes || p->M < 1 || p->Nr < 1 || p->Nr > 128) return 0;
  TNArgs a;
  tn_args(p, &a, nullptr);
  const TNPlan pl = tn_plan(p, a, SIZE_MAX, nullptr);
  return !pl.why && pl.kernel <= TN_IMG_SPLIT && pl.csc != TN_CSC_CALL_SIDE;
}
```

elliptic_gnn_project_amd/csrc/gemm_planes.hip:

```cpp
#include "gemm_common.hpp"

typedef __bf16 bf16x8 __attribute__((ext_vector_type(8)));
typedef short s16x4 __attribute__((ext_vector_type(4)));
typedef unsigned int u32x4 __attribute__((ext_vector_type(4)));
typedef __bf16 bf16x2v_t __attribute__((ext_vector_type(2)));
typedef float f32x2v_t __attribute__((ext_vector_type(2)));

namespace gnnmp {
using gemm::aligned;
namespace {

__global__ __launch_bounds__(256) void split_planes_kernel(const float* __restrict__ x, int64_t ldx, int64_t rows,
                                                           int32_t F, uint16_t* __restrict__ img, int64_t ld,
                                                           int64_t ps, int32_t width) {
  const int hw = width >> 1;
  const int64_t i = (int64_t)blockIdx.x * 256 + threadIdx.x;
  if (i >= rows * hw) return;
  const int64_t r = i / hw;
  const int c = 2 * (int)(i - r * hw);
  const float* xr = x + r * ldx;
  const float a = c < F ? xr[c] : 0.0f;
  const float b = c + 1 < F ? xr[c + 1] : 0.0f;
  uint32_t h, m, l;
  split3_pair(a, b, h, m, l);
  uint32_t* d = reinterpret_cast<uint32_t*>(img + r * ld + c);
  d[0] = h;
  d[ps >> 1] = m;
  d[ps] = l;
}

__global__ __launch_bounds__(256) void split_h2_kernel(const float* __restrict__ x, int64_t ldx, int64_t rows,
                                                       int32_t F, uint16_t* __restrict__ img, int64_t ld, int64_t ps,
                                                       int32_t width, float s) {
  const int hw = width >> 1;
  const int64_t i = (int64_t)blockIdx.x * 256 + threadIdx.x;
  if (i >= rows * hw) return;
  const int64_t r = i / hw;
  const int c = 2 * (int)(i - r * hw);
  const float* xr = x + r * ldx;
  const float a = c < F ? xr[c] * s : 0.0f;
  const float b = c + 1 < F ? xr[c + 1] * s : 0.0f;
  uint32_t h, l;
  split_h2_pair(a, b, h, l);
  uint32_t* d = reinterpret_cast<uint32_t*>(img + r * ld + c);
  d[0] = h;
  d[ps >> 1] = l;
}

constexpr int PT_ROWS = 16;
constexpr int PT_AP = 352;
constexpr int PT_APL = PT_ROWS * PT_AP;
constexpr int PT_GP = 24;
constexpr int PT_GPL = 128 * PT_GP;
constexpr int PT_MAXLD = 336;

__device__ __forceinline__ s16x4 tr_read(const uint16_t* p) {
  return __builtin_amdgcn_ds_read_tr16_b64_v4i16((__attribute__((address_space(3))) s16x4*)(p));
}

__device__ __forceinline__ bf16x8 cat_frag(s16x4 a, s16x4 b) {
  typedef short s16x8 __attribute__((ext_vector_type(8)));
  const s16x8 v = {a[0], a[1], a[2], a[3], b[0], b[1], b[2], b[3]};
  return __builtin_bit_cast(bf16x8, v);
}

template <bool PROJ, bool MASK, int KT, bool GOUT, int LAB = 0, int KS = 1, int NW = 4>
__global__ __launch_bounds__(64 * NW) void gemm_tn_planes_kernel(TNArgs a) {
  constexpr int RG = NW / KS;
  static_assert((NW == 4 || NW == 8) && (RG == 2 || RG == 4) && RG * KS == NW, "wave layout");
  constexpr bool EVEN = KT % KS == 0;
  constexpr int KW = (KT + KS - 1) / KS;
  constexpr int T = 64 * NW;
  constexpr int NP = (3 * PT_ROWS * (PT_MAXLD / 8) + T - 1) / T;
  constexpr int RP = PT_ROWS / (T / 128);
  __shared__ __attribute__((aligned(16))) uint16_t Gt[2][3 * PT_GPL];
  __shared__ __attribute__((aligned(16))) uint16_t At[2][3 * PT_APL];
  __shared__ float dzL[2][256];
  constexpr int NU = 2 * NP + RP / 2 + 2 * RP + RP + 3;
  const int tid = threadIdx.x;
  const int lane = tid & 63;
  const int wave = tid >> 6;
  const int ld = a.ap_ld;
  const int pr = ld >> 3;
  const int64_t mbeg = (int64_t)blockIdx.x * a.rows_per_block;
  const int64_t mend = min(a.M, mbeg + a.rows_per_block);
  const int nch = mend > mbeg ? (int)((mend - mbeg + PT_ROWS - 1) / PT_ROWS) : 0;

  const int wr = wave % RG;
  const int kg = wave / RG;
  const int t0 = kg * KT / KS;
  const int ntl = (kg + 1) * KT / KS - t0;
  floatx16 acc[KW];
#pragma unroll
  for (int t = 0; t < KW; ++t)
#pragma unroll
    for (int r = 0; r < 16; ++r) acc[t][r] = 0.0f;

  const __amdgpu_buffer_rsrc_t arsrc =
      __builtin_amdgcn_make_buffer_rsrc(const_cast<uint16_t*>(a.ap), 0, (int)(3 * a.ap_ps * 2), 0x00020000);
  uint32_t goff[NP], loff[NP];
#pragma unroll
  for (int j = 0; j < NP; ++j) {
    const int q = tid + T * j;
    const int per_plane = PT_ROWS * pr;
    const bool ok = q < 3 * per_plane;
    const int p = q / per_plane, rr = q - p * per_plane;
    const int row = rr / pr, c16 = rr - row * pr;
    goff[j] = ok ? (uint32_t)(((int64_t)p * a.ap_ps + (int64_t)row * ld + 8 * c16) * 2) : 0u;
    loff[j] = ok ? (uint32_t)((p * PT_APL + row * PT_AP + 8 * c16) * 2)
                 : (uint32_t)(((tid & 15) * PT_AP + PT_MAXLD + 8 * ((tid >> 4) & 1)) * 2);
  }

  const int gn = tid & 127, go = tid >> 7;
  const bool gcol = gn < a.Nr;
  const int gnc = gcol ? gn : 0;
  const float* gbase = MASK ? a.h + gnc : a.g + gnc;
  const int gld = MASK ? (int)a.ldh : (int)a.ldg;
  const float* g2base = a.g + gnc;
  const int g2ld = (int)a.ldg;
  const int zr = (tid & 63) / MAXPROJ, zq = (tid & 63) % MAXPROJ;
  const int zqc = PROJ ? min(zq, a.nproj - 1) : 0;
  float pcol[MAXPROJ];
#pragma unroll
  for (int q = 0; q < MAXPROJ; ++q) pcol[q] = (PROJ && q < a.nproj && gcol) ? a.proj[q * a.Nr + gn] : 0.0f;

  const int Mi = (int)a.M;
  auto ldbase = [&](int c) { return min((int)mbeg + c * PT_ROWS, Mi - PT_ROWS); };
  const int clast = max(nch - 1, 0);
  u32x4 ra[NP];
  float rg[RP], rg2[RP];
  float rz = 0.f;
  auto load_a = [&](int j, int c) {
    ra[j] = __builtin_amdgcn_raw_buffer_load_b128(arsrc, (int)goff[j], ldbase(c) * ld * 2, 0);
  };
  auto load_g = [&](int c) {
    const int mb = ldbase(c);
    if constexpr (MASK || !PROJ) {
      uint32_t o = (uint32_t)((mb + RP * go) * gld);
#pragma unroll
      for (int i = 0; i < RP; ++i) {
        rg[i] = gbase[o];
        o += (uint32_t)gld;
      }
    }
    if constexpr (MASK && !PROJ) {
      uint32_t o2 = (uint32_t)((mb + RP * go) * g2ld);
#pragma unroll
      for (int i = 0; i < RP; ++i) {
        rg2[i] = g2base[o2];
        o2 += (uint32_t)g2ld;
      }
    }
  };
  auto load_z = [&](int c) {
    if constexpr (PROJ) rz = a.dz[(uint32_t)((ldbase(c) + zr) * (int)a.lddz + zqc)];
  };
  auto put_z = [&](int k) {
    if constexpr (PROJ) {
      const int mb = ldbase(k);
      const bool ok = tid < PT_ROWS * MAXPROJ && zq < a.nproj && zr >= (int)mbeg + k * PT_ROWS - mb &&
                      zr < (int)mend - mb;
      if (T == 256 || tid < 256) dzL[k & 1][tid] = ok ? rz : 0.0f;
    }
  };

  float db = 0.f, dzs = 0.f;
  float dw2[MAXPROJ] = {0.f, 0.f, 0.f, 0.f};
  float e[RP];
  uint32_t w[RP / 2][3];
  float4 zv[RP];
  float zsv[RP];
  auto z_read = [&](int c, int i0, int n) {
    if constexpr (PROJ) {
      const int buf = c & 1;
#pragma unroll
      for (int i = i0; i < i0 + n; ++i) {
        const int r = RP * go + i;
        zv[i] = *reinterpret_cast<const float4*>(&dzL[buf][r * MAXPROJ]);
        zsv[i] = dzL[buf][r * MAXPROJ + (gn & (MAXPROJ - 1))];
      }
    }
  };
  auto put_a = [&](int j, int c) {
    *reinterpret_cast<u32x4*>(reinterpret_cast<char*>(At[c & 1]) + loff[j]) = ra[j];
  };
  auto g_row = [&](int i, int c, int half) {
    if (half == 0) {
      if constexpr (PROJ) {
        const float4 z = zv[i];
        float g = z.x * pcol[0];
        g = fmaf(z.y, pcol[1], g);
        g = fmaf(z.z, pcol[2], g);
        e[i] = fmaf(z.w, pcol[3], g);
        if constexpr (MASK) {
          dw2[0] = fmaf(z.x, rg[i], dw2[0]);
          dw2[1] = fmaf(z.y, rg[i], dw2[1]);
          dw2[2] = fmaf(z.z, rg[i], dw2[2]);
          dw2[3] = fmaf(z.w, rg[i], dw2[3]);
        }
      } else {
        e[i] = MASK ? rg2[i] : rg[i];
      }
      return;
    }
    const int mb = ldbase(c);
    const int r = RP * go + i;
    const bool ok = r >= (int)mbeg + c * PT_ROWS - mb && r < (int)mend - mb && gcol;
    float g = e[i];
    if constexpr (PROJ) dzs += gn < MAXPROJ ? zsv[i] : 0.0f;
    if constexpr (MASK) g = rg[i] > 0.0f ? g * a.hscale : 0.0f;
    if constexpr (!PROJ) g = ok ? g : 0.0f;
    db += g;
    if constexpr (GOUT) {
      if (a.gout && ok) a.gout[(int64_t)(mb + r) * a.ldgout + gn] = g;
    }
    e[i] = g;
  };
  auto split_half = [&](int j, int half) {
    typedef __bf16 bf16x2_ __attribute__((ext_vector_type(2)));
    typedef float f32x2_ __attribute__((ext_vector_type(2)));
    float& x0 = e[2 * j];
    float& x1 = e[2 * j + 1];
    if (half == 0) {
      const uint32_t h = __builtin_bit_cast(uint32_t, __builtin_convertvector(f32x2_{x0, x1}, bf16x2_));
      w[j][0] = h;
      x0 -= __uint_as_float(h << 16);
      x1 -= __uint_as_float(h & 0xffff0000u);
    } else {
      const uint32_t m = __builtin_bit_cast(uint32_t, __builtin_convertvector(f32x2_{x0, x1}, bf16x2_));
      w[j][1] = m;
      const float y0 = x0 - __uint_as_float(m << 16);
      const float y1 = x1 - __uint_as_float(m & 0xffff0000u);
      w[j][2] = __builtin_bit_cast(uint32_t, __builtin_convertvector(f32x2_{y0, y1}, bf16x2_));
    }
  };
  auto g_put = [&](int c) {
    uint16_t* gd = Gt[c & 1] + gn * PT_GP + RP * go;
#pragma unroll
    for (int p = 0; p < 3; ++p) {
      if constexpr (RP == 8) *reinterpret_cast<uint4*>(gd + p * PT_GPL) = make_uint4(w[0][p], w[1][p], w[2][p], w[3][p]);
      else *reinterpret_cast<uint2*>(gd + p * PT_GPL) = make_uint2(w[0][p], w[1][p]);
    }
  };
  auto unit = [&](int k, int c) {
    constexpr int A0 = 0, Z0 = 2 * NP, G0 = Z0 + RP / 2, S0 = G0 + 2 * RP, P0 = S0 + RP;
    if (k < Z0) {
      if (k & 1) load_a(k >> 1, min(c + 2, clast));
      else put_a(k >> 1, c + 1);
    } else if (k < G0) {
      z_read(c + 1, 2 * (k - Z0), 2);
    } else if (k < S0) {
      g_row((k - G0) >> 1, c + 1, (k - G0) & 1);
    } else if (k < P0) {
      split_half((k - S0) >> 1, (k - S0) & 1);
    } else if (k == P0) {
      g_put(c + 1);
    } else if (k == P0 + 1) {
      load_g(min(c + 2, clast));
    } else if (k == P0 + 2) {
      put_z(c + 2);
      load_z(min(c + 3, clast));
    }
    (void)A0;
  };
  static_assert(2 * NP + RP / 2 + 2 * RP + RP + 3 == NU, "slot count");

  const int gfo = (32 * wr + (lane & 31)) * PT_GP + 8 * (lane >> 5);
  const int grp = lane >> 4, li = lane & 15;
  const int afo = (8 * (grp >> 1) + (li >> 2)) * PT_AP + 16 * (grp & 1) + 4 * (li & 3);
  auto afrag = [&](const uint16_t* base, int t, int p) {
    const uint16_t* q = base + p * PT_APL + t * 32;
    return cat_frag(tr_read(q), tr_read(q + 4 * PT_AP));
  };
#define PT_FENCE __builtin_amdgcn_sched_barrier(0)
  auto compute = [&](int c) {
    const int buf = c & 1;
    bf16x8 gf[3], af[2][3];
#pragma unroll
    for (int p = 0; p < 3; ++p) gf[p] = *reinterpret_cast<const bf16x8*>(Gt[buf] + p * PT_GPL + gfo);
    const uint16_t* ab = At[buf] + afo;
#pragma unroll
    for (int p = 0; p < 3; ++p) af[0][p] = afrag(ab, t0, p);
    constexpr int pa[6] = {1, 2, 0, 1, 0, 0}, pb[6] = {1, 0, 2, 0, 1, 0};
#pragma unroll
    for (int t = 0; t < KW; ++t) {
      if (t + 1 < KW && !(LAB & 4)) {
#pragma unroll
        for (int p = 0; p < 3; ++p) af[(t + 1) & 1][p] = afrag(ab, t0 + t + 1, p);
      }
#pragma unroll
      for (int m = 0; m < 6; ++m) {
        PT_FENCE;
        if constexpr (!(LAB & 1)) {
          if (EVEN || t < ntl)
            acc[t] = __builtin_amdgcn_mfma_f32_32x32x16_bf16(gf[pa[m]], af[(LAB & 4) ? 0 : (t & 1)][pb[m]], acc[t], 0, 0, 0);
        }
        PT_FENCE;
        if (6 * t + m < NU && !(LAB & 2)) unit(6 * t + m, c);
      }
      PT_FENCE;
    }
#pragma unroll
    for (int u = 6 * KW; u < NU; ++u)
      if (!(LAB & 2)) unit(u, c);
    if constexpr ((LAB & 1) != 0) {
#pragma unroll
      for (int t = 0; t < KW; ++t) acc[t][0] += (float)gf[0][0] + (float)af[0][0][0] + (float)af[1][1][1];
    }
  };
#undef PT_FENCE

  if (nch > 0) {
    rz = PROJ ? a.dz[(uint32_t)((ldbase(0) + zr) * (int)a.lddz + zqc)] : 0.f;
    put_z(0);
    load_z(min(1, clast));
    put_z(1);
    load_z(min(2, clast));
#pragma unroll
    for (int j = 0; j < NP; ++j) load_a(j, 0);
    load_g(0);
    __syncthreads();
#pragma unroll
    for (int j = 0; j < NP; ++j) put_a(j, 0);
    z_read(0, 0, RP);
#pragma unroll
    for (int i = 0; i < RP; ++i) {
      g_row(i, 0, 0);
      g_row(i, 0, 1);
    }
#pragma unroll
    for (int j = 0; j < RP / 2; ++j) split3_pair(e[2 * j], e[2 * j + 1], w[j][0], w[j][1], w[j][2]);
    g_put(0);
#pragma unroll
    for (int j = 0; j < NP; ++j) load_a(j, min(1, clast));
    load_g(min(1, clast));
    __syncthreads();
    for (int c = 0; c < nch; ++c) {
      compute(c);
      if constexpr (!(LAB & 8)) __syncthreads();
    }
  }

  float* slab = a.slab + (int64_t)blockIdx.x * a.slab_stride;
  const int Kc = a.k1 + a.k2;
#pragma unroll
  for (int t = 0; t < KW; ++t) {
    if (!EVEN && t >= ntl) break;
    const int kp = (t0 + t) * 32 + (lane & 31);
    const bool s1 = kp < a.k1;
    const bool s2 = kp >= a.ap_col2 && kp < a.ap_col2 + a.k2;
#pragma unroll
    for (int r = 0; r < 16; ++r) {
      const int row = 32 * wr + (r & 3) + 8 * (r >> 2) + 4 * (lane >> 5);
      const int64_t idx = s1 ? (int64_t)row * a.k1 + kp : (int64_t)a.Nr * a.k1 + (int64_t)row * a.k2 + (kp - a.ap_col2);
      if (row < a.Nr && (s1 || s2)) slab[idx] = acc[t][r];
    }
  }
  __syncthreads();
  float* red = reinterpret_cast<float*>(&At[0][0]);
  constexpr int ns = 2 + MAXPROJ;
  red[(go * 128 + gn) * ns + 0] = db;
  red[(go * 128 + gn) * ns + 1] = dzs;
#pragma unroll
  for (int q = 0; q < MAXPROJ; ++q) red[(go * 128 + gn) * ns + 2 + q] = dw2[q];
  __syncthreads();
  constexpr int NGO = T / 128;
  auto comb = [&](int col, int f) {
    float v = red[col * ns + f];
#pragma unroll
    for (int o = 1; o < NGO; ++o) v += red[(o * 128 + col) * ns + f];
    return v;
  };
  if (tid < 128 && tid < a.Nr) {
    float* side = slab + (int64_t)a.Nr * Kc;
    side[tid] = comb(tid, 0);
    for (int q = 0; q < a.nproj; ++q) side[a.Nr + q * a.Nr + tid] = comb(tid, 2 + q);
  }
  if (PROJ && tid < a.nproj) slab[(int64_t)a.Nr * Kc + a.Nr + a.nproj * a.Nr + tid] = comb(tid, 1);
}

template <int NW>
__device__ __forceinline__ float tn_csc_fold(const TNArgs& a, int64_t mbeg, int64_t mend, float* buf, float* dzb,
                                             int lane, int wave) {
  constexpr int CAP = 256, NI = CAP / 64, LCAP = 32;
  const int F = a.ccols, nq = a.nproj;
  const int64_t nrows = a.M;
  float* dz = const_cast<float*>(a.dz);
  float zm = 0.f;
  for (int64_t r0 = ((mbeg >> 6) + wave) * 64; r0 < mend; r0 += 64 * NW) {
    const int64_t r = r0 + lane;
    const bool rok = r < nrows;
    const int32_t pbeg = a.cptr[rok ? r : nrows];
    const int32_t pend = a.cptr[rok ? r + 1 : nrows];
    const int32_t base = __builtin_amdgcn_readfirstlane(a.cptr[r0]);
    const int32_t wend = __builtin_amdgcn_readfirstlane(a.cptr[min(r0 + 64, nrows)]);
    float dv[MAXPROJ];
    const int64_t rc = min(r, nrows - 1);
#pragma unroll
    for (int q = 0; q < MAXPROJ; ++q) dv[q] = a.dz[rc * a.lddz + min(max(q, F), nq - 1)];
    float acc[2] = {0.f, 0.f};
    for (int32_t pb = base; pb < wend; pb += CAP) {
      const int32_t pe = min(pb + CAP, wend);
      int32_t nn[NI];
#pragma unroll
      for (int i = 0; i < NI; ++i) {
        const int32_t k = pb + lane + 64 * i;
        nn[i] = a.cnbr[k < pe ? k : pb];
      }
      float xv[NI][2];
#pragma unroll
      for (int i = 0; i < NI; ++i) {
        const float* xr = a.cu + (int64_t)nn[i] * a.ldu;
#pragma unroll
        for (int f = 0; f < 2; ++f) xv[i][f] = xr[f < F ? f : 0];
      }
#pragma unroll
      for (int i = 0; i < NI; ++i) {
#pragma unroll
        for (int f = 0; f < 2; ++f) buf[f * CAP + lane + 64 * i] = f < F ? xv[i][f] : 0.0f;
      }
      __builtin_amdgcn_s_waitcnt(0xc07f);
      __builtin_amdgcn_wave_barrier();
      const int32_t lo = max(pbeg, pb), hi0 = min(pend, pe);
      const int32_t hi = min(hi0, lo + LCAP);
      float q1[2] = {0.f, 0.f}, q2[2] = {0.f, 0.f}, q3[2] = {0.f, 0.f};
      int32_t k = lo;
      for (; k + 3 < hi; k += 4) {
#pragma unroll
        for (int f = 0; f < 2; ++f) {
          acc[f] += buf[f * CAP + (k - pb)];
          q1[f] += buf[f * CAP + (k + 1 - pb)];
          q2[f] += buf[f * CAP + (k + 2 - pb)];
          q3[f] += buf[f * CAP + (k + 3 - pb)];
        }
      }
      for (; k < hi; ++k) {
#pragma unroll
        for (int f = 0; f < 2; ++f) acc[f] += buf[f * CAP + (k - pb)];
      }
#pragma unroll
      for (int f = 0; f < 2; ++f) acc[f] += (q1[f] + q2[f]) + q3[f];
      uint64_t longm = __ballot(hi0 - lo > LCAP);
      while (longm) {
        const int L = __builtin_ctzll(longm);
        longm &= longm - 1;
        const int32_t s0 = __builtin_amdgcn_readlane(lo, L) + LCAP, s1 = __builtin_amdgcn_readlane(hi0, L);
        float part[2] = {0.f, 0.f};
        for (int32_t k2 = s0 + lane; k2 < s1; k2 += 64) {
#pragma unroll
          for (int f = 0; f < 2; ++f) part[f] += buf[f * CAP + (k2 - pb)];
        }
#pragma unroll
        for (int f = 0; f < 2; ++f) {
#pragma unroll
          for (int off = 32; off >= 1; off >>= 1) part[f] += __shfl_xor(part[f], off);
          if (lane == L) acc[f] += part[f];
        }
      }
      __builtin_amdgcn_wave_barrier();
    }
    if (rok && r >= mbeg && r < mend) {
#pragma unroll
      for (int f = 0; f < 2; ++f)
        if (f < F) dz[r * a.lddz + f] = acc[f];
      float v[MAXPROJ];
#pragma unroll
      for (int q = 0; q < MAXPROJ; ++q) v[q] = q == 0 ? acc[0] : (q == 1 && F > 1) ? acc[1] : dv[q];
      float sr = 0.f;
#pragma unroll
      for (int q = 0; q < MAXPROJ; ++q) {
        sr += q < nq ? fabsf(v[q]) : 0.f;
        dzb[(r - mbeg) * MAXPROJ + q] = v[q];
      }
      zm = fmaxf(zm, sr);
    }
  }
  return zm;
}

template <int KT, bool GOUT, int LAB = 0, int NW = 4, bool GF = false, int KS = 1, bool CSC = false, bool ACT = false,
          int RD = 1>
__global__ __launch_bounds__(64 * NW) void gemm_tn_h2_kernel(TNArgs a) {
  static_assert(NW == 4 || NW == 8, "4 or 8 waves");
  static_assert(KS == 1 || (KS == 2 && NW == 8) || (ACT && KS <= 4), "split-K: the 8-wave form (ACT: up to 4 ways)");
  static_assert(!ACT || (NW == 8 && !GOUT && !GF && !CSC && !(LAB & 16)), "ACT: the plain dz form");
  static_assert(RD == 1 || (ACT && RD <= 4), "the deep register ring: the flag-driven form");
  constexpr int T = 64 * NW;
  constexpr int KTB = (KT + KS - 1) / KS;
  constexpr int NPA = ((ACT && KS > 1 ? 2 * PT_ROWS * 4 * KTB : 2 * PT_ROWS * (PT_MAXLD / 8)) + T - 1) / T;
  constexpr int RP = PT_ROWS / (T / 128);
  constexpr int KTW = NW == 4 ? KTB : (KTB + 1) / 2;
  __shared__ __attribute__((aligned(16))) uint16_t Gt[2][3 * PT_GPL];
  __shared__ __attribute__((aligned(16))) uint16_t At[2][2 * PT_APL];
  __shared__ float dzL[2][256];
  __shared__ float redm[2 * NW];
  __shared__ int32_t clist[ACT ? TN_ACT_CAP : 1];
  __shared__ int32_t actw[NW];
  constexpr int NU = 2 * NPA + RP / 2 + 2 * RP + RP / 2 + 3;
  constexpr int NG = 3 * KTW;
  constexpr int RING = (LAB & 16) ? 2 : RD;
  constexpr int RGN = RD;
  constexpr int RZ = RD;
  const int tid = threadIdx.x;
  const int lane = tid & 63;
  const int wave = tid >> 6;
  const int ld = a.ap_ld;
  const int kpart = KS == 1 ? 0 : (int)(blockIdx.x % KS);
  const int rblk = KS == 1 ? (int)blockIdx.x : (int)(blockIdx.x / KS);
  const int kt0 = (kpart * KT + KS - 1) / KS;
  const int ktb = ((kpart + 1) * KT + KS - 1) / KS - kt0;
  const int pr = min(4 * ktb, (ld - 32 * kt0) >> 3);
  const int64_t mbeg = (int64_t)rblk * a.rows_per_block;
  const int64_t mend = min(a.M, mbeg + a.rows_per_block);
  const int Mi = (int)a.M;
  int nch = mend > mbeg ? (int)((mend - mbeg + PT_ROWS - 1) / PT_ROWS) : 0;
  if constexpr (ACT) {
    const int nf = (Mi + PT_ROWS - 1) / PT_ROWS;
    const int q0 = (int)(mbeg / PT_ROWS), q1 = min(nf, (int)((mbeg + a.rows_per_block) / PT_ROWS));
    const int q = q0 + tid;
    const bool on = q < q1 && a.dz_active[q] != 0;
    const uint64_t bm = __ballot(on);
    if (lane == 0) actw[wave] = __popcll(bm);
    __syncthreads();
    int wbase = 0, n_act = 0;
#pragma unroll
    for (int w2 = 0; w2 < NW; ++w2) {
      const int v = actw[w2];
      wbase += w2 < wave ? v : 0;
      n_act += v;
    }
    const int pos = wbase + __popcll(bm & ((1ull << lane) - 1ull));
    if (on && pos < TN_ACT_CAP) clist[pos] = q;
    __syncthreads();
    nch = min(n_act, TN_ACT_CAP);
    if (a.slab_empty) {
      if (kpart == 0 && tid == 0)
        reinterpret_cast<uint32_t*>(a.slab + (int64_t)rblk * a.slab_stride)[a.slab_stride - 1] = nch == 0 ? 1u : 0u;
      if (nch == 0) return;
    }
  }
  typedef _Float16 f16x8 __attribute__((ext_vector_type(8)));
  const int wrow = 32 * (wave & 3);
  const int tbase = NW == 4 ? 0 : (wave >> 2) * KTW;
  const int ntl = NW == 4 ? KT : max(0, min(KTW, ktb - tbase));

  floatx16 acc[KTW];
#pragma unroll
  for (int t = 0; t < KTW; ++t)
#pragma unroll
    for (int r = 0; r < 16; ++r) acc[t][r] = 0.0f;

  const __amdgpu_buffer_rsrc_t arsrc =
      __builtin_amdgcn_make_buffer_rsrc(const_cast<uint16_t*>(a.ap), 0, (int)(2 * a.ap_ps * 2), 0x00020000);
  uint32_t goff[NPA], loff[NPA];
#pragma unroll
  for (int j = 0; j < NPA; ++j) {
    const int q = tid + T * j;
    const int per_plane = PT_ROWS * pr;
    const bool ok = q < 2 * per_plane;
    const int p = q / per_plane, rr = q - p * per_plane;
    const int row = rr / pr, c16 = rr - row * pr;
    goff[j] = ok ? (uint32_t)(((int64_t)p * a.ap_ps + (int64_t)row * ld + 32 * kt0 + 8 * c16) * 2) : 0u;
    loff[j] = ok ? (uint32_t)((p * PT_APL + row * PT_AP + 8 * c16) * 2)
                 : (uint32_t)(((tid & 15) * PT_AP + PT_MAXLD + 8 * ((tid >> 4) & 1)) * 2);
  }

  const int gn = tid & 127, go = tid >> 7;
  const bool gcol = gn < a.Nr;
  const int gnc = gcol ? gn : 0;
  const float* hb = GF ? a.g + gnc : a.h + gnc;
  const int hld = GF ? (int)a.ldg : (int)a.ldh;
  const int zr = (tid & 63) / MAXPROJ, zq = (tid & 63) % MAXPROJ;
  const int zqc = min(zq, a.nproj - 1);
  float pcol[MAXPROJ];
#pragma unroll
  for (int q = 0; q < MAXPROJ; ++q) pcol[q] = (!GF && q < a.nproj && gcol) ? a.proj[q * a.Nr + gn] : 0.0f;

  float gsc = 1.f, gunsc = 1.f;
  float zm_fold = 0.f;
  auto scan_scale = [&]() __attribute__((always_inline)) {
    float zm = zm_fold;
    const int nq = a.nproj;
    if (GF && a.growmax) {
      const int64_t q1 = (mend + GNN_ROWMAX_ROWS - 1) / GNN_ROWMAX_ROWS;
      for (int64_t q = mbeg / GNN_ROWMAX_ROWS + tid; q < q1; q += T) zm = fmaxf(zm, __uint_as_float(a.growmax[q]));
    } else if constexpr (GF) {
      constexpr int SU = 16;
      const int n4 = (a.Nr + 3) >> 2;
      const int64_t npc = (mend - mbeg) * n4;
      for (int64_t q0 = tid; q0 < npc; q0 += SU * T) {
        float4 v[SU];
#pragma unroll
        for (int u = 0; u < SU; ++u) {
          const int64_t q = min(q0 + (int64_t)T * u, npc - 1);
          const int64_t r = mbeg + q / n4;
          const int c4 = (int)(q - (q / n4) * n4) * 4;
          v[u] = *reinterpret_cast<const float4*>(a.g + r * a.ldg + c4);
        }
#pragma unroll
        for (int u = 0; u < SU; ++u) {
          const int64_t q = q0 + (int64_t)T * u;
          const int c4 = (int)(min(q, npc - 1) % n4) * 4;
          float m = fabsf(v[u].x);
          m = fmaxf(m, c4 + 1 < a.Nr ? fabsf(v[u].y) : 0.f);
          m = fmaxf(m, c4 + 2 < a.Nr ? fabsf(v[u].z) : 0.f);
          m = fmaxf(m, c4 + 3 < a.Nr ? fabsf(v[u].w) : 0.f);
          zm = fmaxf(zm, q < npc ? m : 0.f);
        }
      }
    }
    if constexpr (ACT) {
      constexpr int CP = T / PT_ROWS;
      for (int k0 = tid / PT_ROWS; k0 < nch; k0 += 4 * CP) {
        float v[4][MAXPROJ];
#pragma unroll
        for (int u = 0; u < 4; ++u) {
          const int64_t r = min(clist[min(k0 + CP * u, nch - 1)] * PT_ROWS + (tid & (PT_ROWS - 1)), Mi - 1);
#pragma unroll
          for (int q = 0; q < MAXPROJ; ++q) v[u][q] = a.dz[r * a.lddz + min(q, nq - 1)];
        }
#pragma unroll
        for (int u = 0; u < 4; ++u) {
          float s = 0.f;
#pragma unroll
          for (int q = 0; q < MAXPROJ; ++q) s += q < nq ? fabsf(v[u][q]) : 0.f;
          zm = fmaxf(zm, k0 + CP * u < nch ? s : 0.f);
        }
      }
    }
    for (int64_t r0 = mbeg + tid; !GF && !CSC && !ACT && r0 < mend; r0 += 4 * T) {
      float v[4][MAXPROJ];
#pragma unroll
      for (int u = 0; u < 4; ++u) {
        const int64_t r = min(r0 + (int64_t)T * u, mend - 1);
#pragma unroll
        for (int q = 0; q < MAXPROJ; ++q) v[u][q] = a.dz[r * a.lddz + min(q, nq - 1)];
      }
#pragma unroll
      for (int u = 0; u < 4; ++u) {
        float s = 0.f;
#pragma unroll
        for (int q = 0; q < MAXPROJ; ++q) s += q < nq ? fabsf(v[u][q]) : 0.f;
        zm = fmaxf(zm, r0 + (int64_t)T * u < mend ? s : 0.f);
      }
    }
    float pm = 0.f;
#pragma unroll
    for (int q = 0; q < MAXPROJ; ++q) pm = fmaxf(pm, fabsf(pcol[q]));
#pragma unroll
    for (int o = 32; o > 0; o >>= 1) {
      zm = fmaxf(zm, __shfl_xor(zm, o));
      pm = fmaxf(pm, __shfl_xor(pm, o));
    }
    if (lane == 0) {
      redm[wave] = zm;
      redm[NW + wave] = pm;
    }
    __syncthreads();
    zm = redm[0];
    pm = redm[NW];
#pragma unroll
    for (int w = 1; w < NW; ++w) {
      zm = fmaxf(zm, redm[w]);
      pm = fmaxf(pm, redm[NW + w]);
    }
    const float bound = GF ? zm : zm * pm * a.hscale;
    int E = 0;
    if (bound > 0.f && isfinite(bound)) frexpf(bound, &E);
    gsc = ldexpf(1.0f, 4 - E);
    gunsc = ldexpf(1.0f, E - 4 - 11 - a.ap_exp);
  };

  const int clast = max(nch - 1, 0);
  auto cid = [&](int c) __attribute__((always_inline)) { return __builtin_amdgcn_readfirstlane(clist[c]); };
  auto ldbase = [&](int c) __attribute__((always_inline)) {
    if constexpr (ACT) return min(cid(c) * PT_ROWS, Mi - PT_ROWS);
    else return min((int)mbeg + c * PT_ROWS, Mi - PT_ROWS);
  };
  auto zrange = [&](int k, int& lo, int& hi) __attribute__((always_inline)) {
    if constexpr (ACT) {
      const int q = cid(min(k, clast)), mb = min(q * PT_ROWS, Mi - PT_ROWS);
      lo = k < nch ? q * PT_ROWS - mb : PT_ROWS;
      hi = min(Mi, (q + 1) * PT_ROWS) - mb;
    } else {
      const int mb = ldbase(k);
      lo = (int)mbeg + k * PT_ROWS - mb;
      hi = (int)mend - mb;
    }
  };
  int ab2 = 0, ab3 = 0, az2lo = 0, az2hi = 0, glo = 0;
  u32x4 ra[RING][NPA];
  float rg[RGN][RP];
  float rz[RZ] = {};
  auto load_a_at = [&](int s, int j, int mb) __attribute__((always_inline)) {
    ra[s][j] = __builtin_amdgcn_raw_buffer_load_b128(arsrc, (int)goff[j], mb * ld * 2, 0);
  };
  auto load_a = [&](int s, int j, int c) __attribute__((always_inline)) { load_a_at(s, j, ldbase(c)); };
  auto load_g_at = [&](int sg, int mb) __attribute__((always_inline)) {
    uint32_t o = (uint32_t)((mb + RP * go) * hld);
#pragma unroll
    for (int i = 0; i < RP; ++i) {
      rg[sg][i] = hb[o];
      o += (uint32_t)hld;
    }
  };
  auto load_g = [&](int sg, int c) __attribute__((always_inline)) { load_g_at(sg, ldbase(c)); };
  auto load_z_at = [&](int sz, int mb) __attribute__((always_inline)) {
    if constexpr (!GF) rz[sz] = a.dz[(uint32_t)((mb + zr) * (int)a.lddz + zqc)];
  };
  auto load_z = [&](int sz, int c) __attribute__((always_inline)) { load_z_at(sz, ldbase(c)); };
  auto put_zlh = [&](int k, int lo, int hi, float v) __attribute__((always_inline)) {
    if constexpr (GF) return;
    const bool ok = tid < PT_ROWS * MAXPROJ && zq < a.nproj && zr >= lo && zr < hi;
    if (T == 256 || tid < 256) dzL[k & 1][tid] = ok ? v : 0.0f;
  };
  auto put_zv = [&](int k, float v) __attribute__((always_inline)) {
    if constexpr (GF) return;
    int lo, hi;
    zrange(k, lo, hi);
    put_zlh(k, lo, hi, v);
  };
  auto put_z = [&](int k) __attribute__((always_inline)) { put_zv(k, rz[0]); };

  float db = 0.f, dzs = 0.f;
  float dw2[MAXPROJ] = {0.f, 0.f, 0.f, 0.f};
  float e[RP];
  uint32_t w[RP / 2][3];
  float4 zv[RP];
  float zsv[RP];
  auto z_read = [&](int c, int i0, int n) __attribute__((always_inline)) {
    if constexpr (GF) return;
    const int buf = c & 1;
#pragma unroll
    for (int i = i0; i < i0 + n; ++i) {
      const int r = RP * go + i;
      zv[i] = *reinterpret_cast<const float4*>(&dzL[buf][r * MAXPROJ]);
      zsv[i] = dzL[buf][r * MAXPROJ + (gn & (MAXPROJ - 1))];
    }
  };
  auto put_a = [&](int s, int j, int c) __attribute__((always_inline)) {
    *reinterpret_cast<u32x4*>(reinterpret_cast<char*>(At[c & 1]) + loff[j]) = ra[s][j];
  };
  auto g_row = [&](int i, int c, int half, int sg) __attribute__((always_inline)) {
    if constexpr (GF) {
      if (half == 0) return;
      const int mb = ldbase(c);
      const int r = RP * go + i;
      const bool ok = r >= (int)mbeg + c * PT_ROWS - mb && r < (int)mend - mb && gcol;
      const float g = ok ? rg[sg][i] : 0.0f;
      db += g;
      e[i] = g * gsc;
      return;
    }
    if constexpr (ACT) rg[sg][i] = RP * go + i >= glo ? rg[sg][i] : 0.0f;
    if (half == 0) {
      const float4 z = zv[i];
      float g = z.x * pcol[0];
      g = fmaf(z.y, pcol[1], g);
      g = fmaf(z.z, pcol[2], g);
      e[i] = fmaf(z.w, pcol[3], g);
      dw2[0] = fmaf(z.x, rg[sg][i], dw2[0]);
      dw2[1] = fmaf(z.y, rg[sg][i], dw2[1]);
      dw2[2] = fmaf(z.z, rg[sg][i], dw2[2]);
      dw2[3] = fmaf(z.w, rg[sg][i], dw2[3]);
      return;
    }
    float g = e[i];
    dzs += gn < MAXPROJ ? zsv[i] : 0.0f;
    g = rg[sg][i] > 0.0f ? g * a.hscale : 0.0f;
    db += g;
    if constexpr (GOUT) {
      const int mb = ldbase(c);
      const int r = RP * go + i;
      const bool ok = r >= (int)mbeg + c * PT_ROWS - mb && r < (int)mend - mb && gcol;
      if (a.gout && ok) a.gout[(int64_t)(mb + r) * a.ldgout + gn] = g;
    }
    e[i] = g * gsc;
  };
  auto split_pair = [&](int j) __attribute__((always_inline)) {
    split_h2_pair(e[2 * j], e[2 * j + 1], w[j][1], w[j][2]);
    w[j][0] = h2_scale_pair(w[j][1], 2048.0f);
  };
  auto g_put = [&](int c) __attribute__((always_inline)) {
    uint16_t* gd = Gt[c & 1] + gn * PT_GP + RP * go;
#pragma unroll
    for (int p = 0; p < 3; ++p) {
      if constexpr (RP == 8) *reinterpret_cast<uint4*>(gd + p * PT_GPL) = make_uint4(w[0][p], w[1][p], w[2][p], w[3][p]);
      else *reinterpret_cast<uint2*>(gd + p * PT_GPL) = make_uint2(w[0][p], w[1][p]);
    }
  };
  auto unit = [&](int k, int c, int par) __attribute__((always_inline)) {
    constexpr int Z0 = 2 * NPA, G0 = Z0 + RP / 2, S0 = G0 + 2 * RP, P0 = S0 + RP / 2;
    const int sa = RING == 1 ? 0 : (par + 1) % RING;
    const int sg = RGN == 1 ? 0 : (par + 1) % RGN;
    const int sz = RZ == 1 ? 0 : (par + 2) % RZ;
    if (k < Z0) {
      if (k & 1) {
        if constexpr (ACT) load_a_at(sa, k >> 1, ab2);
        else load_a(sa, k >> 1, min(c + 1 + RING, clast));
      } else {
        put_a(sa, k >> 1, c + 1);
      }
    } else if (k < G0) {
      z_read(c + 1, 2 * (k - Z0), 2);
    } else if (k < S0) {
      g_row((k - G0) >> 1, c + 1, (k - G0) & 1, sg);
    } else if (k < P0) {
      split_pair(k - S0);
    } else if (k == P0) {
      g_put(c + 1);
    } else if (k == P0 + 1) {
      if constexpr (ACT) load_g_at(sg, ab2);
      else load_g(sg, min(c + 1 + RGN, clast));
    } else if (k == P0 + 2) {
      if constexpr (ACT) {
        put_zlh(c + 2, az2lo, az2hi, rz[sz]);
        load_z_at(sz, ab3);
      } else {
        put_z(c + 2);
        load_z(0, min(c + 3, clast));
      }
    }
  };

  const int gfo = (wrow + (lane & 31)) * PT_GP + 8 * (lane >> 5);
  const int grp = lane >> 4, li = lane & 15;
  const int afo = (8 * (grp >> 1) + (li >> 2)) * PT_AP + 16 * (grp & 1) + 4 * (li & 3);
  auto afrag = [&](const uint16_t* base, int t, int p) __attribute__((always_inline)) {
    const uint16_t* q = base + p * PT_APL + t * 32;
    return __builtin_bit_cast(f16x8, cat_frag(tr_read(q), tr_read(q + 4 * PT_AP)));
  };
#define TH_FENCE __builtin_amdgcn_sched_barrier(0)
  auto compute = [&](int c, auto parc) __attribute__((always_inline)) {
    constexpr int par = decltype(parc)::value;
    const int buf = c & 1;
    if constexpr (ACT) {
      glo = az2lo;
      zrange(c + 2, az2lo, az2hi);
      ab2 = ldbase(min(c + 1 + RD, clast));
      ab3 = ldbase(min(c + 2 + RD, clast));
    }
    f16x8 gf[3], af[2][2];
#pragma unroll
    for (int p = 0; p < 3; ++p) gf[p] = *reinterpret_cast<const f16x8*>(Gt[buf] + p * PT_GPL + gfo);
    const uint16_t* ab = At[buf] + afo;
#pragma unroll
    for (int p = 0; p < 2; ++p) af[0][p] = afrag(ab, tbase, p);
    constexpr int pg[3] = {2, 1, 0}, pa[3] = {0, 1, 0};
    static_for<KTW>([&](auto tc) __attribute__((always_inline)) {
      constexpr int t = decltype(tc)::value;
      if constexpr (t + 1 < KTW && !(LAB & 4)) {
#pragma unroll
        for (int p = 0; p < 2; ++p) af[(t + 1) & 1][p] = afrag(ab, tbase + t + 1, p);
      }
      static_for<3>([&](auto mc) __attribute__((always_inline)) {
        constexpr int m = decltype(mc)::value;
        constexpr int gap = 3 * t + m;
        TH_FENCE;
        if constexpr (!(LAB & 1)) {
          if (NW == 4 || t < ntl)
            acc[t] = __builtin_amdgcn_mfma_f32_32x32x16_f16(gf[pg[m]], af[(LAB & 4) ? 0 : (t & 1)][pa[m]], acc[t], 0, 0, 0);
        }
        TH_FENCE;
        if constexpr (!(LAB & 2)) {
          static_for<(gap + 1) * NU / NG - gap * NU / NG>([&](auto uc) __attribute__((always_inline)) {
            unit(gap * NU / NG + decltype(uc)::value, c, par);
          });
        }
      });
      TH_FENCE;
    });
    if constexpr (NU > NG) {}
    if constexpr ((LAB & 1) != 0) {
#pragma unroll
      for (int t = 0; t < KTW; ++t) acc[t][0] += (float)gf[0][0] + (float)af[0][0][0] + (float)af[1][1][1];
    }
  };
#undef TH_FENCE

  if (nch > 0) {
#pragma unroll
    for (int j = 0; j < NPA; ++j) load_a(0, j, 0);
#pragma unroll
    for (int s = 1; s < RING; ++s) {
#pragma unroll
      for (int j = 0; j < NPA; ++j) load_a(s, j, min(s, clast));
    }
    load_g(0, 0);
#pragma unroll
    for (int s = 1; s < RGN; ++s) load_g(s, min(s, clast));
    float* dzb = reinterpret_cast<float*>(&At[0][0]) + NW * 2 * 256;
    if constexpr (CSC && !GF) {
      zm_fold = tn_csc_fold<NW>(a, mbeg, mend, reinterpret_cast<float*>(&At[0][0]) + wave * 2 * 256, dzb, lane, wave);
      __syncthreads();
    }
    float rz0 = 0.f, rz1 = 0.f;
    if constexpr (CSC && !GF) {
      auto dzb_at = [&](int c) __attribute__((always_inline)) {
        const int64_t rl = ldbase(c) + zr - mbeg;
        return (rl >= 0 && rl < mend - mbeg) ? dzb[rl * MAXPROJ + zq] : 0.f;
      };
      rz0 = dzb_at(0);
      rz1 = dzb_at(min(1, clast));
    } else if constexpr (!GF) {
      rz0 = a.dz[(uint32_t)((ldbase(0) + zr) * (int)a.lddz + zqc)];
      rz1 = a.dz[(uint32_t)((ldbase(min(1, clast)) + zr) * (int)a.lddz + zqc)];
    }
#pragma unroll
    for (int s = 0; s < RZ; ++s) load_z((2 + s) % RZ, min(2 + s, clast));
    put_zv(0, rz0);
    put_zv(1, rz1);
    scan_scale();
#pragma unroll
    for (int j = 0; j < NPA; ++j) put_a(0, j, 0);
    z_read(0, 0, RP);
    if constexpr (ACT) {
      zrange(0, glo, az2hi);
      zrange(1, az2lo, az2hi);
    }
#pragma unroll
    for (int i = 0; i < RP; ++i) {
      g_row(i, 0, 0, 0);
      g_row(i, 0, 1, 0);
    }
#pragma unroll
    for (int j = 0; j < RP / 2; ++j) split_pair(j);
    g_put(0);
#pragma unroll
    for (int j = 0; j < NPA; ++j) load_a(0, j, min(RING, clast));
    load_g(0, min(RGN, clast));
    __syncthreads();
    if constexpr (RD == 1) {
      for (int c = 0; c < nch; c += 2) {
        compute(c, std::integral_constant<int, 0>{});
        __syncthreads();
        if (c + 1 < nch) {
          compute(c + 1, std::integral_constant<int, 1>{});
          __syncthreads();
        }
      }
    } else {
      for (int c = 0; c < nch; c += RD) {
        static_for<RD>([&](auto ic) __attribute__((always_inline)) {
          constexpr int i = decltype(ic)::value;
          if (c + i < nch) {
            compute(c + i, ic);
            __syncthreads();
          }
        });
      }
    }
  }

  float* slab = a.slab + (int64_t)rblk * a.slab_stride;
  const int Kc = a.k1 + a.k2;
#pragma unroll
  for (int t = 0; t < KTW; ++t) {
    if (NW == 8 && t >= ntl) break;
    const int kp = (kt0 + tbase + t) * 32 + (lane & 31);
    const bool s1 = kp < a.k1;
    const bool s2 = kp >= a.ap_col2 && kp < a.ap_col2 + a.k2;
#pragma unroll
    for (int r = 0; r < 16; ++r) {
      const int row = wrow + (r & 3) + 8 * (r >> 2) + 4 * (lane >> 5);
      const int64_t idx = s1 ? (int64_t)row * a.k1 + kp : (int64_t)a.Nr * a.k1 + (int64_t)row * a.k2 + (kp - a.ap_col2);
      if constexpr ((LAB & 128) != 0) {
        if (row < a.Nr && (s1 || s2) && acc[t][r] == 1.2345f) slab[idx] = 0.f;
      } else {
        if (row < a.Nr && (s1 || s2)) slab[idx] = acc[t][r] * gunsc;
      }
    }
  }
  __syncthreads();
  float* red = reinterpret_cast<float*>(&At[0][0]);
  constexpr int ns = 2 + MAXPROJ;
  red[(go * 128 + gn) * ns + 0] = db;
  red[(go * 128 + gn) * ns + 1] = dzs;
#pragma unroll
  for (int q = 0; q < MAXPROJ; ++q) red[(go * 128 + gn) * ns + 2 + q] = dw2[q];
  __syncthreads();
  constexpr int NGO = T / 128;
  auto comb = [&](int col, int f) __attribute__((always_inline)) {
    float v = red[col * ns + f];
#pragma unroll
    for (int o = 1; o < NGO; ++o) v += red[(o * 128 + col) * ns + f];
    return v;
  };
  if (kpart != 0) return;
  if (tid < 128 && tid < a.Nr) {
    float* side = slab + (int64_t)a.Nr * Kc;
    side[tid] = comb(tid, 0);
    for (int q = 0; q < a.nproj; ++q) side[a.Nr + q * a.Nr + tid] = comb(tid, 2 + q);
  }
  if (tid < a.nproj) slab[(int64_t)a.Nr * Kc + a.Nr + a.nproj * a.Nr + tid] = comb(tid, 1);
}

template <bool PROJ, bool MASK, int KT, bool GOUT, int D, bool GB = false>
__global__ __launch_bounds__(256) void gemm_tn_img16_kernel(TNArgs a) {
  constexpr int NPA = 3;
  __shared__ __attribute__((aligned(16))) uint16_t Gt[2][PT_GPL];
  __shared__ __attribute__((aligned(16))) uint16_t At[2][PT_APL];
  __shared__ float dzL[2][256];
  const int tid = threadIdx.x;
  const int lane = tid & 63;
  const int wave = tid >> 6;
  const int ld = a.ap_ld;
  const int pr = ld >> 3;
  const int64_t mbeg = (int64_t)blockIdx.x * a.rows_per_block;
  const int64_t mend = min(a.M, mbeg + a.rows_per_block);
  const int nch = mend > mbeg ? (int)((mend - mbeg + PT_ROWS - 1) / PT_ROWS) : 0;

  floatx16 acc[KT];
#pragma unroll
  for (int t = 0; t < KT; ++t)
#pragma unroll
    for (int r = 0; r < 16; ++r) acc[t][r] = 0.0f;

  const __amdgpu_buffer_rsrc_t arsrc =
      __builtin_amdgcn_make_buffer_rsrc(const_cast<uint16_t*>(a.ap), 0, (int)(a.ap_ps * 2), 0x00020000);
  uint32_t goff[NPA], loff[NPA];
#pragma unroll
  for (int j = 0; j < NPA; ++j) {
    const int q = tid + 256 * j;
    const bool ok = q < PT_ROWS * pr;
    const int row = q / pr, c16 = q - row * pr;
    goff[j] = ok ? (uint32_t)(((int64_t)row * ld + 8 * c16) * 2) : 0u;
    loff[j] = ok ? (uint32_t)((row * PT_AP + 8 * c16) * 2)
                 : (uint32_t)(((tid & 15) * PT_AP + PT_MAXLD + 8 * ((tid >> 4) & 1)) * 2);
  }
  const int gc4 = tid & 31, rp = tid >> 5;
  const int n0 = 4 * gc4;
  const bool gcol = n0 < a.Nr;
  const int n0c = gcol ? n0 : 0;
  const uint16_t* hbase = reinterpret_cast<const uint16_t*>(a.h) + n0c;
  const float* gbase = a.g + n0c;
  const uint16_t* gbase16 = reinterpret_cast<const uint16_t*>(a.g) + n0c;
  const int zr = (tid & 63) / MAXPROJ, zq = (tid & 63) % MAXPROJ;
  const int zqc = PROJ ? min(zq, a.nproj - 1) : 0;
  float pcol[4][MAXPROJ];
#pragma unroll
  for (int j = 0; j < 4; ++j)
#pragma unroll
    for (int q = 0; q < MAXPROJ; ++q) pcol[j][q] = (PROJ && q < a.nproj && gcol) ? a.proj[q * a.Nr + n0 + j] : 0.0f;

  const int Mi = (int)a.M;
  auto ldbase = [&](int c) { return min((int)mbeg + c * PT_ROWS, Mi - PT_ROWS); };
  const int clast = max(nch - 1, 0);
  u32x4 ra[D][NPA];
  uint2 rh[D][2];
  float4 rg[D][2];
  uint2 rgb[D][2];
  float rz[D];
  auto load_chunk = [&](int d, int c) {
    const int mb = ldbase(c);
#pragma unroll
    for (int j = 0; j < NPA; ++j) ra[d][j] = __builtin_amdgcn_raw_buffer_load_b128(arsrc, (int)goff[j], mb * ld * 2, 0);
#pragma unroll
    for (int i = 0; i < 2; ++i) {
      const uint32_t row = (uint32_t)(mb + 2 * rp + i);
      if constexpr (MASK) rh[d][i] = *reinterpret_cast<const uint2*>(hbase + row * (uint32_t)a.ldh);
      if constexpr (!PROJ && GB) rgb[d][i] = *reinterpret_cast<const uint2*>(gbase16 + row * (uint32_t)a.ldg);
      else if constexpr (!PROJ) rg[d][i] = *reinterpret_cast<const float4*>(gbase + row * (uint32_t)a.ldg);
    }
  };
  auto load_z = [&](int d, int c) {
    if constexpr (PROJ) rz[d] = a.dz[(uint32_t)((ldbase(c) + zr) * (int)a.lddz + zqc)];
  };
  auto put_z = [&](int d, int k) {
    if constexpr (PROJ) {
      const int mb = ldbase(k);
      const bool ok = tid < PT_ROWS * MAXPROJ && zq < a.nproj && zr >= (int)mbeg + k * PT_ROWS - mb && zr < (int)mend - mb;
      dzL[k & 1][tid] = ok ? rz[d] : 0.0f;
    }
  };

  float db[4] = {0.f, 0.f, 0.f, 0.f};
  float dzs[MAXPROJ] = {0.f, 0.f, 0.f, 0.f};
  float dw2[4][MAXPROJ];
#pragma unroll
  for (int j = 0; j < 4; ++j)
#pragma unroll
    for (int q = 0; q < MAXPROJ; ++q) dw2[j][q] = 0.f;
  auto put_chunk = [&](int d, int c) {
    const int buf = c & 1;
#pragma unroll
    for (int j = 0; j < NPA; ++j) *reinterpret_cast<u32x4*>(reinterpret_cast<char*>(At[buf]) + loff[j]) = ra[d][j];
    const int mb = ldbase(c);
    float gv[2][4];
#pragma unroll
    for (int i = 0; i < 2; ++i) {
      const int r = 2 * rp + i;
      const bool ok = r >= (int)mbeg + c * PT_ROWS - mb && r < (int)mend - mb && gcol;
      float hv[4];
      if constexpr (MASK) {
        hv[0] = __uint_as_float(rh[d][i].x << 16);
        hv[1] = __uint_as_float(rh[d][i].x & 0xffff0000u);
        hv[2] = __uint_as_float(rh[d][i].y << 16);
        hv[3] = __uint_as_float(rh[d][i].y & 0xffff0000u);
      }
      float4 z = {0.f, 0.f, 0.f, 0.f};
      if constexpr (PROJ) {
        z = *reinterpret_cast<const float4*>(&dzL[buf][r * MAXPROJ]);
        if (gc4 == 0) {
          dzs[0] += z.x; dzs[1] += z.y; dzs[2] += z.z; dzs[3] += z.w;
        }
      }
#pragma unroll
      for (int j = 0; j < 4; ++j) {
        float e;
        if constexpr (PROJ) {
          e = z.x * pcol[j][0];
          e = fmaf(z.y, pcol[j][1], e);
          e = fmaf(z.z, pcol[j][2], e);
          e = fmaf(z.w, pcol[j][3], e);
          if constexpr (MASK) {
            dw2[j][0] = fmaf(z.x, hv[j], dw2[j][0]);
            dw2[j][1] = fmaf(z.y, hv[j], dw2[j][1]);
            dw2[j][2] = fmaf(z.z, hv[j], dw2[j][2]);
            dw2[j][3] = fmaf(z.w, hv[j], dw2[j][3]);
          }
        } else if constexpr (GB) {
          const uint32_t wd = j < 2 ? rgb[d][i].x : rgb[d][i].y;
          e = __uint_as_float((j & 1) ? (wd & 0xffff0000u) : (wd << 16));
        } else {
          e = j == 0 ? rg[d][i].x : j == 1 ? rg[d][i].y : j == 2 ? rg[d][i].z : rg[d][i].w;
        }
        float g = e;
        if constexpr (MASK) g = hv[j] > 0.0f ? g * a.hscale : 0.0f;
        if constexpr (!PROJ) g = ok ? g : 0.0f;
        db[j] += g;
        gv[i][j] = g;
      }
      if constexpr (GOUT && GB) {
        if (a.gout && ok)
          *reinterpret_cast<uint2*>(reinterpret_cast<uint16_t*>(a.gout) + (int64_t)(mb + r) * a.ldgout + n0) = make_uint2(
              __builtin_bit_cast(uint32_t, __builtin_convertvector((f32x2v_t){gv[i][0], gv[i][1]}, bf16x2v_t)),
              __builtin_bit_cast(uint32_t, __builtin_convertvector((f32x2v_t){gv[i][2], gv[i][3]}, bf16x2v_t)));
      } else if constexpr (GOUT) {
        if (a.gout && ok)
          *reinterpret_cast<float4*>(a.gout + (int64_t)(mb + r) * a.ldgout + n0) =
              make_float4(gv[i][0], gv[i][1], gv[i][2], gv[i][3]);
      }
    }
#pragma unroll
    for (int j = 0; j < 4; ++j)
      *reinterpret_cast<uint32_t*>(Gt[buf] + (n0 + j) * PT_GP + 2 * rp) =
          __builtin_bit_cast(uint32_t, __builtin_convertvector((f32x2v_t){gv[0][j], gv[1][j]}, bf16x2v_t));
  };

  const int gfo = (32 * wave + (lane & 31)) * PT_GP + 8 * (lane >> 5);
  const int grp = lane >> 4, li = lane & 15;
  const int afo = (8 * (grp >> 1) + (li >> 2)) * PT_AP + 16 * (grp & 1) + 4 * (li & 3);
  auto compute = [&](int c) {
    const int buf = c & 1;
    const bf16x8 gf = *reinterpret_cast<const bf16x8*>(Gt[buf] + gfo);
    const uint16_t* ab = At[buf] + afo;
#pragma unroll
    for (int t = 0; t < KT; ++t) {
      const uint16_t* q = ab + t * 32;
      acc[t] = __builtin_amdgcn_mfma_f32_32x32x16_bf16(gf, cat_frag(tr_read(q), tr_read(q + 4 * PT_AP)), acc[t], 0, 0, 0);
    }
  };

  if (nch > 0) {
#pragma unroll
    for (int d = 0; d < D; ++d) {
      load_chunk(d, min(d, clast));
      load_z(d, min(d, clast));
    }
    put_z(0, 0);
    put_z(1, 1);
    load_z(0, min(D, clast));
    load_z(1, min(D + 1, clast));
    __syncthreads();
    put_chunk(0, 0);
    load_chunk(0, min(D, clast));
    __syncthreads();
    for (int c0 = 0; c0 < nch; c0 += D) {
      static_for<D>([&](auto dc) {
        constexpr int d = decltype(dc)::value;
        const int c = c0 + d;
        if (c < nch) {
          constexpr int d1 = (d + 1) % D, d2 = (d + 2) % D;
          put_chunk(d1, c + 1);
          load_chunk(d1, min(c + 1 + D, clast));
          put_z(d2, c + 2);
          load_z(d2, min(c + 2 + D, clast));
          compute(c);
          __syncthreads();
        }
      });
    }
  }

  float* slab = a.slab + (int64_t)blockIdx.x * a.slab_stride;
  const int Kc = a.k1 + a.k2;
#pragma unroll
  for (int t = 0; t < KT; ++t) {
    const int kp = t * 32 + (lane & 31);
    const bool s1 = kp < a.k1;
    const bool s2 = kp >= a.ap_col2 && kp < a.ap_col2 + a.k2;
#pragma unroll
    for (int r = 0; r < 16; ++r) {
      const int row = 32 * wave + (r & 3) + 8 * (r >> 2) + 4 * (lane >> 5);
      const int64_t idx = s1 ? (int64_t)row * a.k1 + kp : (int64_t)a.Nr * a.k1 + (int64_t)row * a.k2 + (kp - a.ap_col2);
      if (row < a.Nr && (s1 || s2)) slab[idx] = acc[t][r];
    }
  }
  constexpr int ns = 1 + MAXPROJ;
#pragma unroll
  for (int j = 0; j < 4; ++j) {
    db[j] += __shfl_xor(db[j], 32);
#pragma unroll
    for (int q = 0; q < MAXPROJ; ++q) dw2[j][q] += __shfl_xor(dw2[j][q], 32);
  }
#pragma unroll
  for (int q = 0; q < MAXPROJ; ++q) dzs[q] += __shfl_xor(dzs[q], 32);
  __syncthreads();
  float* red = reinterpret_cast<float*>(&At[0][0]);
  if (lane < 32) {
#pragma unroll
    for (int j = 0; j < 4; ++j) {
      red[(wave * 128 + n0 + j) * ns] = db[j];
#pragma unroll
      for (int q = 0; q < MAXPROJ; ++q) red[(wave * 128 + n0 + j) * ns + 1 + q] = dw2[j][q];
    }
    if (gc4 == 0) {
#pragma unroll
      for (int q = 0; q < MAXPROJ; ++q) red[4 * 128 * ns + wave * MAXPROJ + q] = dzs[q];
    }
  }
  __syncthreads();
  if (tid < 128 && tid < a.Nr) {
    float* side = slab + (int64_t)a.Nr * Kc;
    const float* rr = red + tid * ns;
    side[tid] = ((rr[0] + rr[128 * ns]) + rr[2 * 128 * ns]) + rr[3 * 128 * ns];
    for (int q = 0; q < a.nproj; ++q)
      side[a.Nr + q * a.Nr + tid] = ((rr[1 + q] + rr[128 * ns + 1 + q]) + rr[2 * 128 * ns + 1 + q]) + rr[3 * 128 * ns + 1 + q];
  }
  if (PROJ && tid < a.nproj) {
    const float* rz4 = red + 4 * 128 * ns;
    slab[(int64_t)a.Nr * Kc + a.Nr + a.nproj * a.Nr + tid] =
        ((rz4[tid] + rz4[MAXPROJ + tid]) + rz4[2 * MAXPROJ + tid]) + rz4[3 * MAXPROJ + tid];
  }
}

}

bool tn_img16_ok(const TNArgs& a) {
  if (!a.ap || a.ap_h2 || !a.a_bf16 || (a.h && !a.h_bf16)) return false;
  const int gb = a.g_bf16 ? 8 : 16;
  if (a.Nr % 4 || (a.h && (a.ldh % 4 || !aligned(a.h, 8))) || (a.g && !a.dz && (a.ldg % 4 || !aligned(a.g, gb))) ||
      (a.gout && (a.ldgout % 4 || !aligned(a.gout, gb))))
    return false;
  if ((a.ap_ld != 256 && a.ap_ld != 336) || !image_cols_ok(a) || !image_planes_ok(a, 1) || a.M < PT_ROWS) return false;
  const int64_t ldmax = std::max({a.h ? a.ldh : 0, a.g ? a.ldg : 0, a.dz ? a.lddz : 0});
  return (a.M + 32) * ldmax < ((int64_t)1 << 31);
}

void launch_tn_img16(const TNArgs& a, int nblk, hipStream_t st) {
  with_rung<8, 11>(a.ap_ld == 256 ? 8 : 11, [&](auto kt) {
    tn_forms(a, [&](auto proj, auto mask, auto gout) {
      if (a.g_bf16) gemm_tn_img16_kernel<proj(), mask(), kt(), gout(), 4, true><<<nblk, 256, 0, st>>>(a);
      else gemm_tn_img16_kernel<proj(), mask(), kt(), gout(), 4><<<nblk, 256, 0, st>>>(a);
    });
  });
}

bool tn_h2_ok(const TNArgs& a) {
  if (!a.ap || !a.ap_h2 || a.a_bf16 || a.h_bf16 || a.g_bf16) return false;
  const bool gf = !a.dz && a.g && !a.h && !a.gout;
  if (gf) {
    if ((a.ap_ld != 336 && a.ap_ld != 176) || a.ldg % 4 || !aligned(a.g, 16)) return false;
  } else if (!a.dz || !a.proj || !a.h || a.nproj < 1 || a.ap_ld != 336) {
    return false;
  }
  if (a.cptr && (gf || a.gout || !a.cnbr || !a.cu || a.ccols < 1 || a.ccols > 2 || a.ccols > a.nproj ||
                 a.ldu < a.ccols || a.M * a.ldu >= ((int64_t)1 << 31)))
    return false;
  if (!image_cols_ok(a) || !image_planes_ok(a, 2) || a.M < PT_ROWS) return false;
  const int64_t ldmax = gf ? a.ldg : std::max({a.ldh, a.lddz});
  return (a.M + 32) * ldmax < ((int64_t)1 << 31);
}

void launch_tn_h2(const TNArgs& a, int nblk, hipStream_t st, bool ks, bool act_split) {
  if (!a.dz) {
    if (a.ap_ld == 176) gemm_tn_h2_kernel<6, false, 0, 8, true><<<nblk, 512, 0, st>>>(a);
    else gemm_tn_h2_kernel<11, false, 0, 8, true><<<nblk, 512, 0, st>>>(a);
    return;
  }
  if (a.dz_active) {
    if (act_split) gemm_tn_h2_kernel<11, false, 0, 8, false, TN_ACT_SPLIT, false, true, TN_ACT_RING><<<nblk, 512, 0, st>>>(a);
    else gemm_tn_h2_kernel<11, false, 0, 8, false, 1, false, true><<<nblk, 512, 0, st>>>(a);
    return;
  }
  if (a.cptr) {
    if (ks) gemm_tn_h2_kernel<11, false, 0, 8, false, 2, true><<<nblk, 512, 0, st>>>(a);
    else gemm_tn_h2_kernel<11, false, 0, 8, false, 1, true><<<nblk, 512, 0, st>>>(a);
    return;
  }
  if (ks) {
    if (a.gout) gemm_tn_h2_kernel<11, true, 0, 8, false, 2><<<nblk, 512, 0, st>>>(a);
    else gemm_tn_h2_kernel<11, false, 0, 8, false, 2><<<nblk, 512, 0, st>>>(a);
    return;
  }
  if (a.gout) gemm_tn_h2_kernel<11, true, 0, 8><<<nblk, 512, 0, st>>>(a);
  else gemm_tn_h2_kernel<11, false, 0, 8><<<nblk, 512, 0, st>>>(a);
}

bool tn_planes_ok(const TNArgs& a) {
  if (!a.ap || a.ap_h2 || a.a_bf16 || a.h_bf16 || a.g_bf16) return false;
  if (a.ap_ld % 16 || a.ap_ld > PT_MAXLD || a.ap_ld < 32) return false;
  if (!image_cols_ok(a) || !image_planes_ok(a, 3) || a.M < PT_ROWS) return false;
  const int64_t ldmax = std::max({a.h ? a.ldh : 0, a.g ? a.ldg : 0, a.dz ? a.lddz : 0});
  return (a.M + 32) * ldmax < ((int64_t)1 << 31);
}

void launch_tn_planes(const TNArgs& a, int nblk, hipStream_t st) {
  with_rung<4, 6, 8, 11>((a.ap_ld + 31) / 32, [&](auto kt) {
    tn_forms(a, [&](auto proj, auto mask, auto gout) {
      constexpr bool P = proj(), MK = mask(), GO = gout();
      constexpr int KT = kt();
      if (a.Nr <= 64) {
        gemm_tn_planes_kernel<P, MK, KT, GO, 0, 4, 8><<<nblk, 512, 0, st>>>(a);
      } else if constexpr (KT <= 8) {
        gemm_tn_planes_kernel<P, MK, KT, GO, 0, 2, 8><<<nblk, 512, 0, st>>>(a);
      } else {
        gemm_tn_planes_kernel<P, MK, KT, GO><<<nblk, 256, 0, st>>>(a);
      }
    });
  });
}

}

using namespace gnnmp;

extern "C" gnn_status gnn_split_h2_f32(const float* x, int64_t ldx, int64_t rows, int64_t F, void* img, int64_t ld,
                                       int64_t plane_stride, int64_t col0, int64_t width, int32_t scale_exp,
                                       gnn_stream_t stream) {
  if (scale_exp < -100 || scale_exp > 100) return fail(GNN_ERR_INVALID_ARG, __func__, "scale_exp outside [-100, 100]");
  if (rows < 0 || F < 0 || ldx < F || width < F || (width & 1) || (col0 & 1) || col0 < 0 || col0 + width > ld ||
      plane_stride < rows * ld || (plane_stride & 1) || (ld & 1))
    return fail(GNN_ERR_INVALID_ARG, __func__, "bad shapes (width >= F, even width / col0 / ld / plane_stride)");
  if (rows == 0 || width == 0) return GNN_OK;
  if (!x && F > 0) return fail(GNN_ERR_INVALID_ARG, __func__, "null x");
  if (!img || (reinterpret_cast<uintptr_t>(img) & 3)) return fail(GNN_ERR_INVALID_ARG, __func__, "null or unaligned image");
  const int64_t n = rows * (width / 2);
  split_h2_kernel<<<(unsigned)ceil_div(n, 256), 256, 0, (hipStream_t)stream>>>(
      x, ldx, rows, (int32_t)F, static_cast<uint16_t*>(img) + col0, ld, plane_stride, (int32_t)width,
      ldexpf(1.0f, scale_exp));
  return hip_check(hipGetLastError(), __func__);
}

extern "C" gnn_status gnn_split_planes_f32(const float* x, int64_t ldx, int64_t rows, int64_t F, void* img, int64_t ld,
                                           int64_t plane_stride, int64_t col0, int64_t width, gnn_stream_t stream) {
  if (rows < 0 || F < 0 || ldx < F || width < F || (width & 1) || (col0 & 1) || col0 < 0 || col0 + width > ld ||
      plane_stride < rows * ld || (plane_stride & 1) || (ld & 1))
    return fail(GNN_ERR_INVALID_ARG, __func__, "bad shapes (width >= F, even width / col0 / ld / plane_stride)");
  if (rows == 0 || width == 0) return GNN_OK;
  if (!x && F > 0) return fail(GNN_ERR_INVALID_ARG, __func__, "null x");
  if (!img || (reinterpret_cast<uintptr_t>(img) & 3)) return fail(GNN_ERR_INVALID_ARG, __func__, "null or unaligned image");
  const int64_t n = rows * (width / 2);
  split_planes_kernel<<<(unsigned)ceil_div(n, 256), 256, 0, (hipStream_t)stream>>>(
      x, ldx, rows, (int32_t)F, static_cast<uint16_t*>(img) + col0, ld, plane_stride, (int32_t)width);
  return hip_check(hipGetLastError(), __func__);
}
```

elliptic_gnn_project_amd/csrc/lab/lab_tn_active.hip:

```cpp
#define GNNMP_LAB 1
#include "../gemm_planes.hip"
#include "../gemm_ws.hip"
#include "../gemm_f32.hip"

#include <algorithm>
#include <cmath>
#include <cstdio>
#include <cstdlib>
#include <cstring>
#include <random>
#include <vector>

namespace gnnmp {
void set_last_error(const std::string&) {}
}

#define CK(x)                                                                         \
  do {                                                                                \
    hipError_t e_ = (x);                                                              \
    if (e_ != hipSuccess) {                                                           \
      std::fprintf(stderr, "%s:%d %s\n", __FILE__, __LINE__, hipGetErrorString(e_)); \
      std::exit(1);                                                                   \
    }                                                                                 \
  } while (0)

using namespace gnnmp;

__global__ void split_h2_kernel(const float* x, int64_t n2, uint16_t* img, int64_t ps) {
  const int64_t i = (int64_t)blockIdx.x * 256 + threadIdx.x;
  if (i >= n2) return;
  uint32_t h, l;
  split_h2_pair(x[2 * i], x[2 * i + 1], h, l);
  reinterpret_cast<uint32_t*>(img)[i] = h;
  reinterpret_cast<uint32_t*>(img + ps)[i] = l;
}

constexpr int NRB = 255;
template <int LAB, int KS, int RD>
void tn(const TNArgs& a) {
  gemm_tn_h2_kernel<11, false, LAB, 8, false, KS, false, true, RD><<<KS * NRB, 512>>>(a);
}

int main(int argc, char** argv) {
  const int rounds = argc > 1 ? std::atoi(argv[1]) : 15;
  const int64_t M = 203769, F = 166, LD = 336, NR = 128;
  const int64_t rpb = ceil_div(ceil_div(M, 32), 256) * 32;
  const int b_lo = 100, b_hi = 150;
  std::vector<float> hx(M * LD, 0.f);
  {
    std::mt19937 g(1);
    std::normal_distribution<float> d(0.f, 1.f);
    for (int64_t r = 0; r < M; ++r)
      for (int c = 0; c < F; ++c) {
        hx[r * LD + c] = d(g) * 0.7f;
        hx[r * LD + 168 + c] = d(g);
      }
  }
  auto up = [](const std::vector<float>& h) {
    float* p;
    CK(hipMalloc(&p, h.size() * 4));
    CK(hipMemcpy(p, h.data(), h.size() * 4, hipMemcpyHostToDevice));
    return p;
  };
  float* xa = up(hx);
  uint16_t* imh;
  CK(hipMalloc(&imh, 2 * M * LD * 2));
  split_h2_kernel<<<(unsigned)ceil_div(M * LD / 2, 256), 256>>>(xa, M * LD / 2, imh, M * LD);
  std::vector<float> hp(4 * NR), hh(M * NR), hdz(M * 4, 0.f);
  const int64_t nf = ceil_div(M, 16);
  std::vector<uint8_t> hfl((nf + 15) / 16 * 16, 0);
  {
    std::mt19937 g(5);
    std::normal_distribution<float> d(0.f, 1.f);
    for (auto& v : hp) v = d(g);
    for (auto& v : hh) v = d(g);
    for (int64_t r = b_lo * rpb; r < std::min(M, b_hi * rpb); ++r) {
      for (int q = 0; q < 4; ++q) hdz[r * 4 + q] = d(g) * 1e-5f;
      hfl[r / 16] = 1;
    }
  }
  float *proj = up(hp), *dh = up(hh), *ddz = up(hdz);
  uint8_t* dfl;
  CK(hipMalloc(&dfl, hfl.size()));
  CK(hipMemcpy(dfl, hfl.data(), hfl.size(), hipMemcpyHostToDevice));

  const int64_t nout = NR * 332 + NR + 4 * NR + 4;
  const int64_t stride = (nout + 63) / 64 * 64;
  float *slab, *out;
  CK(hipMalloc(&slab, NRB * stride * 4));
  CK(hipMalloc(&out, stride * 4));
  TNArgs ta{};
  ta.M = M; ta.Nr = NR; ta.dz = ddz; ta.lddz = 4; ta.proj = proj; ta.nproj = 4; ta.h = dh; ta.ldh = NR; ta.hscale = 2.f;
  ta.k1 = F; ta.k2 = F; ta.slab = slab; ta.slab_stride = stride; ta.rows_per_block = rpb;
  ta.ap = imh; ta.ap_ld = LD; ta.ap_col2 = 168; ta.ap_ps = M * LD; ta.ap_h2 = 1;
  ta.dz_active = dfl;
  TNArgs te = ta;
  te.slab_empty = 1;
  const unsigned rb = (unsigned)ceil_div(ceil_div(nout, 4), kRedOut);

  struct V { const char* name; void (*f)(const TNArgs&); bool empty; std::vector<float> t; bool ablation = false; };
  std::vector<V> vs = {
      {"TN first form (1 block / row block, ring 1)", tn<0, 1, 1>, false, {}},
      {"TN first form, no MFMA", tn<1, 1, 1>, false, {}, true},
      {"TN first form, no staging", tn<2, 1, 1>, false, {}, true},
      {"TN first form, empty slabs skipped", tn<0, 1, 1>, true, {}},
      {"TN ring 2", tn<0, 1, 2>, false, {}},
      {"TN ring 3", tn<0, 1, 3>, false, {}},
      {"TN split 2 ring 2", tn<0, 2, 2>, false, {}},
      {"TN split 2 ring 3", tn<0, 2, 3>, false, {}},
      {"TN split 3 ring 3", tn<0, 3, 3>, false, {}},
      {"TN split 4 ring 1", tn<0, 4, 1>, false, {}},
      {"TN split 4 ring 2", tn<0, 4, 2>, false, {}},
      {"TN split 4 ring 3", tn<0, 4, 3>, false, {}},
      {"TN split 4 ring 4", tn<0, 4, 4>, false, {}},
      {"TN split 4 ring 3, empty slabs skipped", tn<0, 4, 3>, true, {}},
      {"TN split 3 ring 1", tn<0, 3, 1>, false, {}},
      {"TN split 3 ring 1, empty slabs skipped", tn<0, 3, 1>, true, {}},
      {"TN split 4 ring 1, empty slabs skipped", tn<0, 4, 1>, true, {}},
      {"TN split 4 ring 1, no MFMA", tn<1, 4, 1>, false, {}, true},
      {"TN split 4 ring 1, no staging", tn<2, 4, 1>, false, {}, true},
  };
  const size_t nsl = (size_t)NRB * stride;
  std::vector<float> r0(nsl), r1(nsl);
  for (size_t v = 0; v < vs.size(); ++v) {
    if (vs[v].ablation) continue;
    CK(hipMemset(slab, 0, nsl * 4));
    vs[v].f(vs[v].empty ? te : ta);
    CK(hipDeviceSynchronize());
    CK(hipMemcpy((v ? r1 : r0).data(), slab, nsl * 4, hipMemcpyDeviceToHost));
    if (!v) continue;
    size_t ndiff = 0;
    for (int b = 0; b < NRB; ++b)
      for (int64_t j = 0; j < nout; ++j) ndiff += std::memcmp(&r0[b * stride + j], &r1[b * stride + j], 4) != 0;
    std::printf("%-48s %zu slab words differ from the first form's\n", vs[v].name, ndiff);
  }
  hipEvent_t e0, e1;
  CK(hipEventCreate(&e0));
  CK(hipEventCreate(&e1));
  std::vector<float> tred[2];
  for (int r = 0; r < rounds + 2; ++r) {
    for (auto& v : vs) {
      CK(hipEventRecord(e0));
      v.f(v.empty ? te : ta);
      CK(hipEventRecord(e1));
      CK(hipEventSynchronize(e1));
      float ms;
      CK(hipEventElapsedTime(&ms, e0, e1));
      if (r >= 2) v.t.push_back(ms * 1e3f);
    }
    for (int em = 0; em < 2; ++em) {
      CK(hipEventRecord(e0));
      if (em) slab_reduce_kernel<true><<<rb, 256>>>(slab, stride, NRB, out, nout, SqOut{});
      else slab_reduce_kernel<false><<<rb, 256>>>(slab, stride, NRB, out, nout, SqOut{});
      CK(hipEventRecord(e1));
      CK(hipEventSynchronize(e1));
      float ms;
      CK(hipEventElapsedTime(&ms, e0, e1));
      if (r >= 2) tred[em].push_back(ms * 1e3f);
    }
  }
  auto med = [](std::vector<float>& t) {
    std::sort(t.begin(), t.end());
    return t[t.size() / 2];
  };
  for (auto& v : vs) std::printf("%-48s %7.1f us (min %.1f)\n", v.name, med(v.t), v.t[0]);
  std::printf("%-48s %7.1f us (min %.1f)\n", "slab reduce, every slab read", med(tred[0]), tred[0][0]);
  std::printf("%-48s %7.1f us (min %.1f)\n", "slab reduce, empty slabs skipped", med(tred[1]), tred[1][0]);
  return 0;
}
```

include/gnnmp.h:

```cpp
#ifndef GNNMP_H_
#define GNNMP_H_

#include <stddef.h>
#include <stdint.h>

#ifdef __cplusplus
extern "C" {
#endif

#define GNNMP_ABI_VERSION 32

typedef struct ihipStream_t* gnn_stream_t;

typedef enum {
  GNN_OK = 0,
  GNN_ERR_INVALID_ARG = 1,
  GNN_ERR_INDEX_OUT_OF_RANGE = 2,
  GNN_ERR_HIP = 3,
  GNN_ERR_WORKSPACE = 4,
  GNN_ERR_UNSUPPORTED = 5
} gnn_status;

typedef enum {
  GNN_LOOPS_KEEP = 0,
  GNN_LOOPS_REPLACE = 1
} gnn_loop_mode;

typedef struct {
  int32_t seg_len;
  int32_t reserved;
  int64_t num_long;
  int64_t num_pieces;
  const int32_t* ptr;
  const int32_t* nbr;
  const int32_t* piece0;
  const int32_t* piece_seg;
  const int32_t* long_seg;
  const int32_t* order;
} gnn_split;

typedef struct {
  int64_t num_nodes;
  int64_t num_slots;
  const int32_t* rowptr;
  const int32_t* col;
  const int32_t* colptr;
  const int32_t* row;
  const int32_t* csc2csr;
  const gnn_split* csr_split;
  const gnn_split* csc_split;
} gnn_graph;

int gnn_abi_version(void);
const char* gnn_status_string(gnn_status s);
const char* gnn_last_error(void);

gnn_status gnn_graph_workspace_size(int64_t num_nodes, int64_t num_edges, size_t* bytes);

gnn_status gnn_graph_build(const int64_t* edge_index, int64_t num_edges, int64_t num_nodes,
                           gnn_loop_mode loops, int32_t* rowptr, int32_t* col, int32_t* csr_eid,
                           int32_t* colptr, int32_t* row, int32_t* csc2csr, int32_t* stats,
                           void* workspace, size_t workspace_bytes, gnn_stream_t stream);

gnn_status gnn_split_workspace_size(int64_t num_segs, size_t* bytes);
gnn_status gnn_split_count(const int32_t* ptr, int64_t num_segs, int32_t seg_len, int64_t* counts,
                           gnn_stream_t stream);
gnn_status gnn_split_build(const int32_t* ptr, const int32_t* nbr, int64_t num_segs, int32_t seg_len,
                           int32_t* tptr, int32_t* tnbr, int32_t* piece0, int32_t* piece_seg,
                           int32_t* long_seg, int32_t* order, void* workspace, size_t workspace_bytes,
                           gnn_stream_t stream);

gnn_status gnn_in_degree_f32(const gnn_graph* g, float* deg, gnn_stream_t stream);

gnn_status gnn_gcn_norm_f32(const gnn_graph* g, float* dinv, gnn_stream_t stream);

typedef enum {
  GNN_AGG_SUM = 0,
  GNN_AGG_MEAN = 1,
  GNN_AGG_MEAN_BWD = 2,
  GNN_AGG_GCN = 3,
  GNN_AGG_EDGE_W = 4
} gnn_agg_mode;

typedef struct {
  gnn_agg_mode mode;
  int32_t transpose;
  const float* nodew;
  const float* ew;
  int32_t heads;
  const float* addend;
  int64_t ld_add;
  const float* bias;
  int32_t relu;
  float* part;
  size_t part_bytes;
  float dropout_p;
  uint64_t seed;
  const int64_t* seed_ptr;
  const float* addend2;
  int64_t ld_add2;
} gnn_agg_params;

gnn_status gnn_aggregate_f32(const gnn_graph* g, const gnn_agg_params* p, const float* x,
                             int64_t ldx, int64_t F, float* y, int64_t ldy, gnn_stream_t stream);

#define GNN_ACTIVE_ROWS 16

typedef struct {
  uint8_t* row_active;
  const float* active_with;
  int64_t ld_active_with;
  int32_t active_with_cols;
} gnn_agg_active;

gnn_status gnn_aggregate_active_f32(const gnn_graph* g, const gnn_agg_params* p, const float* x, int64_t ldx,
                                    int64_t F, float* y, int64_t ldy, const gnn_agg_active* act,
                                    gnn_stream_t stream);

gnn_status gnn_aggregate_bf16(const gnn_graph* g, const gnn_agg_params* p, const void* x, int64_t ldx,
                              int64_t F, void* y, int64_t ldy, gnn_stream_t stream);

gnn_status gnn_split_planes_f32(const float* x, int64_t ldx, int64_t rows, int64_t F, void* img, int64_t ld,
                                int64_t plane_stride, int64_t col0, int64_t width, gnn_stream_t stream);
gnn_status gnn_sage_mean_fwd_planes(const gnn_graph* g, const float* deg, const float* x, int64_t ldx, int64_t F,
                                    void* img, int64_t ld, int64_t plane_stride, int64_t width,
                                    gnn_stream_t stream);

gnn_status gnn_split_h2_f32(const float* x, int64_t ldx, int64_t rows, int64_t F, void* img, int64_t ld,
                            int64_t plane_stride, int64_t col0, int64_t width, int32_t scale_exp,
                            gnn_stream_t stream);
struct gnn_gemm_nt_params;
gnn_status gnn_sage_mean_fwd_h2(const gnn_graph* g, const float* deg, const float* x, int64_t ldx, int64_t F,
                                void* img, int64_t ld, int64_t plane_stride, int64_t width, int32_t scale_exp,
                                uint32_t* keep_mask, int64_t mask_cols, float dropout_p, uint64_t seed,
                                const uint64_t* seed_ptr, const struct gnn_gemm_nt_params* prep_b,
                                const gnn_split* hub, gnn_stream_t stream);
typedef enum {
  GNN_PLANES_SPLIT_BF16 = 0,
  GNN_PLANES_HALF_PAIR = 1
} gnn_planes_format;

gnn_status gnn_sage_out_mean_ce_f32(const gnn_graph* g, const float* deg, const float* z, int64_t ldz, int32_t C,
                                    const float* bias, float* logits, int64_t ldo, const int64_t* y,
                                    const uint8_t* mask, const float* class_w, float inv_denom, float* dlogits,
                                    int64_t ld_d, float* u, int64_t ldu, float* colsum, float* loss, void* workspace,
                                    size_t workspace_bytes, gnn_stream_t stream);

gnn_status gnn_sage_mean_fwd_f32(const gnn_graph* g, const float* deg, const float* x, int64_t ldx,
                                 int64_t F, float* out, int64_t ldo, gnn_stream_t stream);
gnn_status gnn_sage_mean_bwd_f32(const gnn_graph* g, const float* deg, const float* dout,
                                 int64_t ld_dout, int64_t F, float* dx, int64_t ld_dx,
                                 gnn_stream_t stream);

gnn_status gnn_edge_dot_f32(const gnn_graph* g, const int32_t* eid, const float* nodew, const float* a,
                            int64_t lda, const float* b, int64_t ldb, int64_t F, float* out,
                            gnn_stream_t stream);

gnn_status gnn_gat_scores_f32(int64_t N, int32_t H, int32_t C, const float* xh, int64_t ld_xh,
                              const float* att_src, const float* att_dst, float* a_src,
                              float* a_dst, gnn_stream_t stream);

gnn_status gnn_gat_fwd_f32(const gnn_graph* g, int32_t H, int32_t C, int32_t concat, float slope,
                           const float* xh, int64_t ld_xh, const float* a_src, const float* a_dst,
                           const float* bias, float* alpha, float* out, int64_t ldo,
                           gnn_stream_t stream);

typedef enum { GNN_ACT_NONE = 0, GNN_ACT_ELU = 1 } gnn_act;
typedef struct {
  int32_t heads, chans, concat;
  float slope;
  const float* xh; int64_t ld_xh;
  const float* att_src; const float* att_dst;
  const float* bias;
  gnn_act act;
  float dropout_p;
  uint64_t seed; const uint64_t* seed_ptr;
  float* a_src; float* a_dst;
  float* alpha;
  float* out; int64_t ldo;
  const float* edge_w;
  const float* proj; int32_t nproj;
  float* z; int64_t ldz;
} gnn_gat_fwd_params;
gnn_status gnn_gat_fwd_fused_f32(const gnn_graph* g, const gnn_gat_fwd_params* p, gnn_stream_t stream);
gnn_status gnn_gat_out_ce_f32(const gnn_graph* g, const gnn_gat_fwd_params* p, const int64_t* y, const uint8_t* mask,
                              const float* class_w, float inv_denom, float* dlogits, int64_t ld_d, float* colsum,
                              float* loss, void* workspace, size_t workspace_bytes, gnn_stream_t stream);

gnn_status gnn_gat_act_bwd_f32(int64_t N, int64_t F, gnn_act act, float dropout_p, uint64_t seed,
                               const uint64_t* seed_ptr, const float* y, int64_t ldy, const float* dy,
                               int64_t lddy, float* dpre, int64_t ld_dpre, gnn_stream_t stream);

gnn_status gnn_gat_bwd_workspace_size(int64_t N, int64_t S, int32_t H, int32_t C, size_t* bytes);
gnn_status gnn_gat_bwd_f32(const gnn_graph* g, int32_t H, int32_t C, int32_t concat, float slope,
                           const float* xh, int64_t ld_xh, const float* a_src, const float* a_dst,
                           const float* att_src, const float* att_dst, const float* alpha,
                           const float* dout, int64_t ld_dout, float* dxh, int64_t ld_dxh,
                           float* d_att_src, float* d_att_dst, void* workspace,
                           size_t workspace_bytes, gnn_stream_t stream);

gnn_status gnn_gat_bwd_act_f32(const gnn_graph* g, int32_t H, int32_t C, float slope, const float* xh,
                               int64_t ld_xh, const float* a_src, const float* a_dst, const float* att_src,
                               const float* att_dst, const float* alpha, gnn_act act, float dropout_p,
                               uint64_t seed, const uint64_t* seed_ptr, const float* y, int64_t ld_y,
                               const float* dy, int64_t ld_dy, float* dpre, int64_t ld_dpre, float* dxh,
                               int64_t ld_dxh, float* d_att_src, float* d_att_dst, void* workspace,
                               size_t workspace_bytes, gnn_stream_t stream);

gnn_status gnn_gat_bwd_act_proj_f32(const gnn_graph* g, int32_t H, int32_t C, float slope, const float* xh,
                                    int64_t ld_xh, const float* a_src, const float* a_dst, const float* att_src,
                                    const float* att_dst, const float* alpha, gnn_act act, float dropout_p,
                                    uint64_t seed, const uint64_t* seed_ptr, const float* y, int64_t ld_y,
                                    const float* dz, int64_t ld_dz, const float* proj, int32_t nproj, float* dpre,
                                    int64_t ld_dpre, float* dxh, int64_t ld_dxh, float* d_att_src, float* d_att_dst,
                                    uint32_t* dxh_rowmax, void* workspace, size_t workspace_bytes,
                                    gnn_stream_t stream);

gnn_status gnn_gat_bwd_ew_f32(const gnn_graph* g, int32_t H, int32_t C, int32_t concat, float slope,
                              const float* xh, int64_t ld_xh, const float* a_src, const float* a_dst,
                              const float* att_src, const float* att_dst, const float* alpha,
                              const float* dout, int64_t ld_dout, float* dxh, int64_t ld_dxh,
                              float* d_att_src, float* d_att_dst, const float* edge_w, float* d_edge_w,
                              void* workspace, size_t workspace_bytes, gnn_stream_t stream);

typedef enum { GNN_DTYPE_F32 = 0, GNN_DTYPE_BF16 = 1 } gnn_dtype;

typedef enum {
  GNN_MATH_SPLIT_BF16 = 0,
  GNN_MATH_F32 = 1,
  GNN_MATH_HALF_PAIR = 2
} gnn_gemm_math;

typedef struct gnn_gemm_nt_params {
  int64_t M, N;
  const float* a1; int64_t lda1; int64_t k1;
  const float* a2; int64_t lda2; int64_t k2;
  const float* bt; int64_t ldb;
  const float* w1; const float* w2;
  int64_t ldw1, ldw2;
  float* c; int64_t ldc;
  const float* bias;
  int32_t relu;
  float dropout_p;
  uint64_t seed;
  const uint64_t* seed_ptr;
  const float* proj; int32_t nproj;
  float* z; int64_t ldz;
  int32_t math;
  void* workspace; size_t workspace_bytes;
  int32_t a_dtype;
  int32_t c_dtype;
  const float* mask;
  int64_t ldmask;
  float mask_scale;
  const void* a_planes;
  int64_t planes_ld, planes_stride, planes_col2;
  int32_t planes_format;
  const uint32_t* keep_mask;
  int32_t b_ready;
  int32_t planes_exp;
  float* colsum_part; int64_t colsum_cap;
  int32_t* row_exp;
} gnn_gemm_nt_params;

gnn_status gnn_gemm_nt_colsum_blocks(const gnn_gemm_nt_params* p, int32_t* nb);
gnn_status gnn_gemm_nt_workspace_size(int64_t N, int64_t k1, int64_t k2, size_t* bytes);
gnn_status gnn_gemm_nt_f32(const gnn_gemm_nt_params* p, gnn_stream_t stream);
gnn_status gnn_gemm_nt_prep_b(const gnn_gemm_nt_params* p, gnn_stream_t stream);

typedef struct {
  int64_t M, Nr;
  const float* g; int64_t ldg;
  const float* dz; int64_t lddz;
  const float* proj; int32_t nproj;
  const float* h; int64_t ldh; float hscale;
  float* gout; int64_t ldgout;
  const float* a1; int64_t lda1; int64_t k1;
  const float* a2; int64_t lda2; int64_t k2;
  int32_t math;
  int32_t a_dtype;
  int32_t h_dtype;
  const void* a_planes;
  int64_t planes_ld, planes_stride, planes_col2;
  int32_t planes_format;
  int32_t g_dtype;
  int32_t planes_exp;
  float* sq_partial;
  const float* sq_step;
  int64_t sq_skip_lo, sq_skip_hi, sq_cap;
  const int32_t* row_exp;
  const uint32_t* g_rowmax;
  const gnn_graph* dz_graph;
  const float* dz_u; int64_t ldu;
  int32_t dz_cols;
} gnn_gemm_tn_params;

#define GNN_ROWMAX_ROWS 16

gnn_status gnn_gemm_tn_workspace_size(int64_t M, int64_t Nr, int64_t Kc, int32_t nproj, size_t* bytes);
gnn_status gnn_gemm_tn_f32(const gnn_gemm_tn_params* p, float* out, void* workspace, size_t workspace_bytes,
                           gnn_stream_t stream);
gnn_status gnn_gemm_tn_active_f32(const gnn_gemm_tn_params* p, const uint8_t* dz_active, float* out,
                                  void* workspace, size_t workspace_bytes, gnn_stream_t stream);
int gnn_gemm_tn_active_pays(int64_t M);
int gnn_gemm_tn_active_split(void);
int gnn_gemm_tn_active_ring(void);
gnn_status gnn_gemm_tn_sq_blocks(int64_t n_out, int32_t* nb);
int gnn_gemm_nt_planes_ok(const gnn_gemm_nt_params* p);
int gnn_gemm_tn_planes_ok(const gnn_gemm_tn_params* p);

gnn_status gnn_colsum_workspace_size(int64_t rows, int64_t F, size_t* bytes);
gnn_status gnn_colsum_finish_f32(const float* part, int32_t nblk, int64_t F, float* out, gnn_stream_t stream);
gnn_status gnn_colsum_f32(int64_t rows, int64_t F, const float* x, int64_t ldx, float* out,
                          void* workspace, size_t workspace_bytes, gnn_stream_t stream);

gnn_status gnn_bn_workspace_size(int64_t C, size_t* bytes);
gnn_status gnn_bn_stats_f32(const float* z, int64_t ldz, int64_t N, int64_t C, double* stats, int32_t finalize,
                            float eps, float momentum, float* mean, float* invstd, float* running_mean,
                            float* running_var, int64_t* num_batches_tracked, void* workspace,
                            size_t workspace_bytes, gnn_stream_t stream);
gnn_status gnn_bn_finalize_f32(const double* stats, int64_t C, float eps, float momentum, float* mean,
                               float* invstd, float* running_mean, float* running_var,
                               int64_t* num_batches_tracked, gnn_stream_t stream);
gnn_status gnn_bn_act_res_fwd_f32(const float* z, int64_t ldz, const float* r, int64_t ldr, int64_t N, int64_t C,
                                  const float* mean, const float* invstd, const float* weight, const float* bias,
                                  float dropout_p, uint64_t seed, const int64_t* seed_ptr, float* h, int64_t ldh,
                                  gnn_stream_t stream);
gnn_status gnn_bn_act_bwd_reduce_f32(const float* dh, int64_t lddh, const float* z, int64_t ldz, int64_t N,
                                     int64_t C, const float* mean, const float* invstd, const float* weight,
                                     const float* bias, float dropout_p, uint64_t seed, const int64_t* seed_ptr,
                                     float* sums, void* workspace, size_t workspace_bytes, gnn_stream_t stream);
gnn_status gnn_bn_act_bwd_f32(const float* dh, int64_t lddh, const float* z, int64_t ldz, int64_t N, int64_t C,
                              const float* mean, const float* invstd, const float* weight, const float* bias,
                              float dropout_p, uint64_t seed, const int64_t* seed_ptr, const float* sums,
                              const double* n_total, float* dz, int64_t lddz, gnn_stream_t stream);
gnn_status gnn_bn_act_bwd_colsum_blocks(int64_t N, int64_t C, int32_t* nb);
gnn_status gnn_bn_act_bwd_colsum_f32(const float* dh, int64_t lddh, const float* z, int64_t ldz, int64_t N, int64_t C,
                                     const float* mean, const float* invstd, const float* weight, const float* bias,
                                     float dropout_p, uint64_t seed, const int64_t* seed_ptr, const float* sums,
                                     const double* n_total, float* dz, int64_t lddz, float* colsum,
                                     gnn_stream_t stream);

gnn_status gnn_time_inject_sin_f32(const float* x, int64_t ldx, int64_t N, int64_t F, const int64_t* t_idx,
                                   int64_t dim, int64_t max_timestep, float* out, int64_t ldo, gnn_stream_t stream);

gnn_status gnn_masked_ce_workspace_size(int64_t N, size_t* bytes);
gnn_status gnn_masked_ce_finish(const float* partial, int32_t nblk, float inv_denom, float* loss, gnn_stream_t stream);
gnn_status gnn_gcn_out_ce_f32(const gnn_graph* g, const float* dinv, const float* t, int64_t ldt, int32_t C,
                              const float* bias, float* logits, int64_t ldo, const int64_t* y, const uint8_t* mask,
                              const float* class_w, float inv_denom, float* dlogits, int64_t ld_d, float* colsum,
                              float* loss, void* workspace, size_t workspace_bytes, gnn_stream_t stream);
gnn_status gnn_masked_ce_colsum_f32(int64_t N, int32_t C, const float* logits, int64_t ldx, const int64_t* y,
                                    const uint8_t* mask, const float* class_w, float inv_denom, float* dlogits,
                                    int64_t ld_d, float* loss, void* workspace, size_t workspace_bytes,
                                    float* colsum, gnn_stream_t stream);
gnn_status gnn_masked_ce_f32(int64_t N, int32_t C, const float* logits, int64_t ldx, const int64_t* y,
                             const uint8_t* mask, const float* class_w, float inv_denom, float* dlogits,
                             int64_t ld_d, float* loss, void* workspace, size_t workspace_bytes,
                             gnn_stream_t stream);

typedef struct {
  const int64_t* y;
  const uint8_t* mask;
  const float* class_w;
  const float* row_w;
  float inv_denom;
  int32_t focal;
  float focal_gamma;
  int32_t reserved[5];
} gnn_ce_spec;

gnn_status gnn_masked_ce_spec_f32(int64_t N, int32_t C, const float* logits, int64_t ldx, const gnn_ce_spec* spec,
                                  float* dlogits, int64_t ld_d, float* loss, void* workspace,
                                  size_t workspace_bytes, float* colsum, gnn_stream_t stream);
gnn_status gnn_sage_out_mean_ce_spec_f32(const gnn_graph* g, const float* deg, const float* z, int64_t ldz,
                                         int32_t C, const float* bias, float* logits, int64_t ldo,
                                         const gnn_ce_spec* spec, float* dlogits, int64_t ld_d, float* u,
                                         int64_t ldu, float* colsum, float* loss, void* workspace,
                                         size_t workspace_bytes, gnn_stream_t stream);
gnn_status gnn_gcn_out_ce_spec_f32(const gnn_graph* g, const float* dinv, const float* t, int64_t ldt, int32_t C,
                                   const float* bias, float* logits, int64_t ldo, const gnn_ce_spec* spec,
                                   float* dlogits, int64_t ld_d, float* colsum, float* loss, void* workspace,
                                   size_t workspace_bytes, gnn_stream_t stream);
gnn_status gnn_gat_out_ce_spec_f32(const gnn_graph* g, const gnn_gat_fwd_params* p, const gnn_ce_spec* spec,
                                   float* dlogits, int64_t ld_d, float* colsum, float* loss, void* workspace,
                                   size_t workspace_bytes, gnn_stream_t stream);

#define GNN_ADAM_MAX_TENSORS 24
typedef struct {
  float* param; float* grad; float* exp_avg; float* exp_avg_sq; int64_t numel;
} gnn_adam_tensor;
typedef struct {
  int32_t num_tensors;
  double lr, beta1, beta2, eps, weight_decay, max_norm;
  gnn_adam_tensor tensors[GNN_ADAM_MAX_TENSORS];
  int32_t skip_nonfinite;
  int64_t* bump_counter;
  const float* loss_partial; int32_t loss_nblk; float loss_scale; float* loss_out;
  const float* grad_sq_partial; int32_t grad_sq_nblk;
} gnn_adam_group;
gnn_status gnn_clip_adam_workspace_size(size_t* bytes);
gnn_status gnn_clip_adam_f32(const gnn_adam_group* group, float* step, float* norm_out, void* workspace,
                             size_t workspace_bytes, gnn_stream_t stream);
gnn_status gnn_clip_adam_prep_f32(const gnn_adam_group* group, float* step, float* norm_out, void* workspace,
                                  size_t workspace_bytes, const gnn_gemm_nt_params* nts, int32_t num_nts,
                                  gnn_stream_t stream);

gnn_status gnn_neighbor_sample_workspace_size(int64_t num_nodes, int64_t node_cap, int64_t edge_cap,
                                              size_t* bytes);

gnn_status gnn_neighbor_sample(const gnn_graph* g, const int32_t* csr_eid, const int32_t* seeds,
                               int64_t num_seeds, int32_t num_hops, const int32_t* fanout, uint64_t seed,
                               int32_t* n_id, int64_t node_cap, int32_t* e_src, int32_t* e_dst,
                               int32_t* e_id, int64_t edge_cap, int64_t* hop_nodes, int64_t* hop_edges,
                               void* workspace, size_t workspace_bytes, gnn_stream_t stream);

#define GNN_RANK_TILE 1024
#define GNN_RANK_BOOT_LDS_MAX_N 32768
#define GNN_RANK_STATUS_NAN 1
#define GNN_RANK_STATUS_SEGMENT 2
#define GNN_RANK_STATUS_INDEX 4

gnn_status gnn_rank_plan_workspace_size(int64_t n, int64_t num_segments, size_t* bytes);
gnn_status gnn_rank_plan_build(const float* scores, const uint8_t* include, const int32_t* segment,
                               int64_t n, int64_t num_segments, int32_t* order, uint8_t* flags,
                               int32_t* seg_ptr, int32_t* rank, int32_t* status, void* workspace,
                               size_t workspace_bytes, gnn_stream_t stream);

gnn_status gnn_rank_ap_workspace_size(int64_t n, int64_t num_segments, size_t* bytes);
gnn_status gnn_rank_ap(const int32_t* order, const uint8_t* flags, const int32_t* seg_ptr,
                       const uint8_t* positive, int64_t n, int64_t num_segments, int64_t k, double* ap,
                       int64_t* num_pos, int64_t* count, double* patk, void* workspace,
                       size_t workspace_bytes, gnn_stream_t stream);

gnn_status gnn_rank_bootstrap_workspace_size(int64_t n, int64_t num_replicates, size_t* bytes);
gnn_status gnn_rank_bootstrap(const int32_t* order_a, const int32_t* rank_a, const uint8_t* flags_a,
                              const int32_t* order_b, const int32_t* rank_b, const uint8_t* flags_b,
                              const uint8_t* positive, const int32_t* sample_idx, int64_t n,
                              int64_t num_replicates, int64_t k, double* ap_a, double* ap_b,
                              double* patk_a, double* patk_b, int32_t* status, void* workspace,
                              size_t workspace_bytes, gnn_stream_t stream);

gnn_status gnn_edge_drop_workspace_size(int64_t num_edges, size_t* bytes);
gnn_status gnn_edge_drop(const int64_t* edge_index, int64_t num_edges, int64_t drop_count, uint64_t key,
                         int64_t* out, void* workspace, size_t workspace_bytes, gnn_stream_t stream);

gnn_status gnn_feature_noise_f32(const float* x, int64_t ldx, int64_t rows, int64_t F, float noise_std,
                                 uint64_t key, float* out, int64_t ldo, gnn_stream_t stream);

#define GNN_EXPLAIN_STATUS_BLOCK 1

typedef struct {
  int64_t n;
  int64_t F;
  float* mask;
  int64_t ld_mask;
  const float* grad;
  const float* dh;
  int64_t ld_dh;
  const float* x;
  int64_t ld_x;
  float* h;
  int64_t ld_h;
  float* exp_avg;
  float* exp_avg_sq;
  int64_t ld_state;
  const uint8_t* hard;
  uint8_t* hard_out;
  int64_t ld_hard;
  const int32_t* block_of;
  int32_t num_blocks;
  int32_t t;
  const float* size_scale;
  const float* ent_scale;
  double lr, beta1, beta2, eps;
  int32_t* status;
} gnn_explain_step_params;

gnn_status gnn_explain_mask_step_f32(const gnn_explain_step_params* p, gnn_stream_t stream);

#define GNN_FIT_THREADS 1024
#define GNN_FIT_STATUS_LABEL 1
#define GNN_FIT_STATUS_NAN 2
#define GNN_FIT_STATUS_EMPTY 4
#define GNN_FIT_STATUS_FLAT 8
#define GNN_FIT_STATUS_CLAMP_LOW 16
#define GNN_FIT_STATUS_CLAMP_HIGH 32
#define GNN_FIT_STATUS_MAXIT 64
#define GNN_CURVE_OUTPUTS 8
#define GNN_CALIB_MAX_BINS 32

gnn_status gnn_temperature_fit_workspace_size(int64_t n, size_t* bytes);
gnn_status gnn_temperature_fit(const float* logits, int64_t ld, const int64_t* y, const uint8_t* include,
                               int64_t n, float* T, double* diag, int32_t* status, void* workspace,
                               size_t workspace_bytes, gnn_stream_t stream);

gnn_status gnn_rank_curve_workspace_size(int64_t n, size_t* bytes);
gnn_status gnn_rank_curve(const int32_t* order, const uint8_t* flags, const int32_t* seg_ptr,
                          const uint8_t* positive, const float* scores, int64_t n, int64_t num_segments,
                          double target_precision, double* out, void* workspace, size_t workspace_bytes,
                          gnn_stream_t stream);

gnn_status gnn_threshold_calibration_workspace_size(int64_t n, int32_t bins, size_t* bytes);
gnn_status gnn_threshold_calibration(const float* scores, const uint8_t* positive, const uint8_t* include,
                                     int64_t n, double thr, const double* edges, int32_t bins,
                                     int64_t* counts, int64_t* bin_count, int64_t* bin_pos, double* bin_sum,
                                     double* out, void* workspace, size_t workspace_bytes,
                                     gnn_stream_t stream);

gnn_status gnn_hub_rank_workspace_size(int64_t num_nodes, int64_t num_edges, size_t* bytes);
gnn_status gnn_hub_rank(const int64_t* edge_index, int64_t num_edges, int64_t num_nodes, int32_t* deg,
                        int32_t* order, int32_t* rank, int32_t* edge_rank, int32_t* removed_cum,
                        void* workspace, size_t workspace_bytes, gnn_stream_t stream);
gnn_status gnn_hub_ablate_workspace_size(int64_t num_edges, size_t* bytes);
gnn_status gnn_hub_ablate(const int64_t* edge_index, int64_t num_edges, const int32_t* edge_rank,
                          int64_t num_hubs, int64_t kept, int64_t* out, void* workspace,
                          size_t workspace_bytes, gnn_stream_t stream);

#define GNN_REPORT_MAX_SEGMENTS 2048
#define GNN_REPORT_STATUS_K 8
#define GNN_JOIN_STATUS_DUPLICATE 16
#define GNN_JOIN_STATUS_NEGATIVE 32
#define GNN_JOIN_STATUS_MISMATCH 64
#define GNN_ENSEMBLE_PROB 0
#define GNN_ENSEMBLE_LOGIT 1

gnn_status gnn_rank_hits_at_workspace_size(int64_t n, size_t* bytes);
gnn_status gnn_rank_hits_at(const int32_t* order, const int32_t* seg_ptr, const uint8_t* positive, int64_t n,
                            int64_t num_segments, const int64_t* ks, int64_t num_k, int64_t* k_eff,
                            int64_t* hits, double* precision, int32_t* status, void* workspace,
                            size_t workspace_bytes, gnn_stream_t stream);

gnn_status gnn_segment_threshold_counts_workspace_size(int64_t n, int64_t num_segments, size_t* bytes);
gnn_status gnn_segment_threshold_counts(const float* scores, const uint8_t* positive, const uint8_t* include,
                                        const int32_t* segment, int64_t n, int64_t num_segments, double thr,
                                        int64_t* counts, int32_t* status, void* workspace,
                                        size_t workspace_bytes, gnn_stream_t stream);

gnn_status gnn_id_join_workspace_size(int64_t n, size_t* bytes);
gnn_status gnn_id_join(const int64_t* base_ids, const int64_t* other_ids, int64_t n, int32_t* perm,
                       int32_t* status, void* workspace, size_t workspace_bytes, gnn_stream_t stream);

gnn_status gnn_ensemble_pair(const float* a, const float* b, const int32_t* perm_a, int64_t n, int32_t mode,
                             float* out, int32_t* status, gnn_stream_t stream);

#define GNN_LOGREG_MAX_D 255
#define GNN_LOGREG_ROWS 128
#define GNN_LOGREG_REDUCE_UNROLL 4
#define GNN_ISOTONIC_CHUNK 128
#define GNN_BASELINE_STATUS_ROW 1
#define GNN_BASELINE_STATUS_NAN 2

gnn_status gnn_column_moments_workspace_size(int64_t n, int64_t D, size_t* bytes);
gnn_status gnn_column_moments(const float* x, int64_t ld, int64_t num_rows, const int32_t* rows, int64_t n,
                              int64_t D, double* mu, double* sd, int32_t* status, void* workspace,
                              size_t workspace_bytes, gnn_stream_t stream);

gnn_status gnn_logreg_eval_workspace_size(int64_t n, int64_t D, size_t* bytes);
gnn_status gnn_logreg_eval(const float* x, int64_t ld, int64_t num_rows, const int32_t* rows, int64_t n,
                           int64_t D, const uint8_t* y, const double* mu, const double* sd, double w0,
                           double w1, double C, const double* theta, int32_t value_only, double* F, double* g,
                           double* H, int32_t* status, void* workspace, size_t workspace_bytes,
                           gnn_stream_t stream);

gnn_status gnn_logreg_predict(const float* x, int64_t ld, int64_t num_rows, const int32_t* rows, int64_t n,
                              int64_t D, const double* mu, const double* sd, const double* theta, double* p64,
                              float* p32, int32_t* status, gnn_stream_t stream);

gnn_status gnn_isotonic_fit_workspace_size(int64_t n, size_t* bytes);
gnn_status gnn_isotonic_fit(const float* scores, const int32_t* order, const uint8_t* flags,
                            const int32_t* seg_ptr, const uint8_t* positive, int64_t n, int64_t num_segments,
                            double* xs, double* ys, int64_t* K, void* workspace, size_t workspace_bytes,
                            gnn_stream_t stream);

gnn_status gnn_isotonic_apply(const double* xs, const double* ys, const int64_t* K, const float* queries,
                              int64_t n, double* out64, float* out32, int32_t* status, gnn_stream_t stream);

#define GNN_EPOCH_MAX_TENSORS 64
#define GNN_EPOCH_CHUNK_BYTES 16384

typedef struct {
  const void* src;
  void* dst;
  int64_t bytes;
} gnn_epoch_tensor;

typedef struct {
  int32_t num_tensors;
  int32_t reserved;
  gnn_epoch_tensor tensors[GNN_EPOCH_MAX_TENSORS];
} gnn_epoch_table;

typedef struct {
  int32_t epoch;
  int32_t bad;
  int32_t best_epoch;
  int32_t stop_epoch;
  int32_t status;
  int32_t reserved;
  double best_val;
} gnn_epoch_state;

gnn_status gnn_epoch_keep_best(const double* ap, const int32_t* ap_status, const float* loss,
                               const gnn_epoch_table* table, int32_t patience, int32_t max_epochs,
                               gnn_epoch_state* state, float* loss_log, double* ap_log, gnn_stream_t stream);

#ifdef __cplusplus
}
#endif
#endif
```

Measured before the change: 2.712 billion edges/s.

## Split active-flag TN GEMM across output-column groups with XCD-aware block mapping

Adds an SG template parameter to the flag-driven TN h2 kernel so that each row block's 128 output columns are split across 4 sibling blocks, instead of splitting K four ways. Block indices are remapped so siblings land on the same XCD, and waves are regrouped across K within a column slice. Column sums are written only by the kpart-0 block. The intent is to cut per-block work and the split-K reduction traffic, at the cost of re-staging the A tile in every sibling and extra guard logic. It is on by default and can be disabled by an environment variable; the Python side must honour the new gsplit query so the slab layout stays consistent.

After: 2.716 billion edges/s (median of 3 runs). About the same (+0.1%).

```diff
diff --git a/elliptic_gnn_project_amd/_lib.py b/elliptic_gnn_project_amd/_lib.py
--- a/elliptic_gnn_project_amd/_lib.py
+++ b/elliptic_gnn_project_amd/_lib.py
@@ -365,6 +365,7 @@
     "gnn_gemm_tn_active_f32": (ctypes.c_int, [ctypes.POINTER(GnnGemmTNParams), c_ptr, c_ptr, c_ptr, c_size, c_ptr]),
     "gnn_gemm_tn_active_pays": (ctypes.c_int, [c_i64]),
     "gnn_gemm_tn_active_split": (ctypes.c_int, []),
+    "gnn_gemm_tn_active_gsplit": (ctypes.c_int, []),
     "gnn_gemm_tn_active_ring": (ctypes.c_int, []),
     "gnn_gemm_nt_planes_ok": (ctypes.c_int, [ctypes.POINTER(GnnGemmNTParams)]),
     "gnn_gemm_nt_colsum_blocks": (ctypes.c_int, [ctypes.POINTER(GnnGemmNTParams), ctypes.POINTER(c_i32)]),
diff --git a/elliptic_gnn_project_amd/csrc/gemm_common.hpp b/elliptic_gnn_project_amd/csrc/gemm_common.hpp
--- a/elliptic_gnn_project_amd/csrc/gemm_common.hpp
+++ b/elliptic_gnn_project_amd/csrc/gemm_common.hpp
@@ -186,6 +186,7 @@
   const int32_t* cptr; const int32_t* cnbr; const float* cu; int64_t ldu; int32_t ccols;
   const uint8_t* dz_active;
   int32_t slab_empty;
+  int32_t act_xcd;
 };
 template <typename F>
 void tn_forms(const TNArgs& a, F&& f) {
@@ -236,7 +237,10 @@
 void launch_prep_h2(const H2Prep& p, hipStream_t st);
 bool tn_h2_ok(const TNArgs& a);
 constexpr int TN_ACT_SPLIT = 4, TN_ACT_RING = 1;
-void launch_tn_h2(const TNArgs& a, int nblk, hipStream_t st, bool ks = false, bool act_split = false);
+constexpr int TN_ACT_GSPLIT = 4, TN_ACT_GSPLIT_K = 1;
+inline int tn_act_gsplit_blocks(int nred) { return TN_ACT_GSPLIT * TN_ACT_GSPLIT_K * ((nred + 7) / 8 * 8); }
+void launch_tn_h2(const TNArgs& a, int nblk, hipStream_t st, bool ks = false, bool act_split = false,
+                  bool act_gsplit = false);
 bool tn_planes_ok(const TNArgs& a);
 void launch_tn_planes(const TNArgs& a, int nblk, hipStream_t st);
 bool tn_img16_ok(const TNArgs& a);
diff --git a/elliptic_gnn_project_amd/csrc/gemm_dispatch.hip b/elliptic_gnn_project_amd/csrc/gemm_dispatch.hip
--- a/elliptic_gnn_project_amd/csrc/gemm_dispatch.hip
+++ b/elliptic_gnn_project_amd/csrc/gemm_dispatch.hip
@@ -258,6 +258,7 @@
 }
 bool tn_active_split() { return !env_off("GNNMP_TN_ACTIVE_SPLIT"); }
 bool tn_empty_skip() { return !env_off("GNNMP_TN_EMPTY_SKIP"); }
+bool tn_active_gsplit() { return !env_off("GNNMP_TN_ACTIVE_GSPLIT"); }
 
 int64_t tn_out_floats(int64_t Nr, int64_t Kc, int32_t nproj) { return Nr * Kc + Nr + (int64_t)nproj * Nr + nproj; }
 int64_t tn_slab_stride(int64_t n_out) { return (n_out + 63) / 64 * 64; }
@@ -309,6 +310,7 @@
   int64_t rows_per_block;
   bool ksplit;
   bool act_split;
+  bool act_gsplit;
   bool empty;
   TNCsc csc;
   TNFlags flags;
@@ -354,7 +356,8 @@
       if (pl.ksplit) pl.blocks = 2 * pl.nred;
       if (pl.flags != TN_FLAGS_NONE) {
         pl.act_split = tn_active_split();
-        if (pl.act_split) pl.blocks = TN_ACT_SPLIT * pl.nred;
+        pl.act_gsplit = pl.act_split && tn_active_gsplit();
+        if (pl.act_split) pl.blocks = pl.act_gsplit ? tn_act_gsplit_blocks(pl.nred) : TN_ACT_SPLIT * pl.nred;
         pl.empty = tn_empty_skip() && a.slab_stride > tn_out_floats(a.Nr, a.k1 + a.k2, a.nproj);
       }
       return run(TN_IMG_H2);
@@ -431,7 +434,7 @@
   if (pl.kernel >= TN_SKINNY) a.ap = nullptr;
   if (pl.kernel <= TN_SKINNY) a.rowexp = nullptr;
   switch (pl.kernel) {
-    case TN_IMG_H2: launch_tn_h2(a, pl.blocks, st, pl.ksplit, pl.act_split); break;
+    case TN_IMG_H2: launch_tn_h2(a, pl.blocks, st, pl.ksplit, pl.act_split, pl.act_gsplit); break;
     case TN_IMG_BF16: launch_tn_img16(a, pl.blocks, st); break;
     case TN_IMG_SPLIT: launch_tn_planes(a, pl.blocks, st); break;
     case TN_SKINNY: launch_tn_skinny(a, pl.blocks, st); break;
@@ -457,7 +460,8 @@
 }
 
 extern "C" int gnn_gemm_tn_active_pays(int64_t M) { return tn_active_pays(M) ? 1 : 0; }
-extern "C" int gnn_gemm_tn_active_split(void) { return TN_ACT_SPLIT; }
+extern "C" int gnn_gemm_tn_active_split(void) { return tn_active_gsplit() ? TN_ACT_GSPLIT_K : TN_ACT_SPLIT; }
+extern "C" int gnn_gemm_tn_active_gsplit(void) { return tn_active_gsplit() ? TN_ACT_GSPLIT : 1; }
 extern "C" int gnn_gemm_tn_active_ring(void) { return TN_ACT_RING; }
 extern "C" gnn_status gnn_gemm_tn_sq_blocks(int64_t n_out, int32_t* nb) {
   if (!nb || n_out < 1) return fail(GNN_ERR_INVALID_ARG, __func__, "bad args");
diff --git a/elliptic_gnn_project_amd/csrc/gemm_planes.hip b/elliptic_gnn_project_amd/csrc/gemm_planes.hip
--- a/elliptic_gnn_project_amd/csrc/gemm_planes.hip
+++ b/elliptic_gnn_project_amd/csrc/gemm_planes.hip
@@ -479,9 +479,10 @@
 }
 
 template <int KT, bool GOUT, int LAB = 0, int NW = 4, bool GF = false, int KS = 1, bool CSC = false, bool ACT = false,
-          int RD = 1>
+          int RD = 1, int SG = 1>
 __global__ __launch_bounds__(64 * NW) void gemm_tn_h2_kernel(TNArgs a) {
   static_assert(NW == 4 || NW == 8, "4 or 8 waves");
+  static_assert(SG == 1 || (ACT && NW == 8 && RD == 1 && (SG == 2 || SG == 4)), "G-column blocks: the flag-driven form");
   static_assert(KS == 1 || (KS == 2 && NW == 8) || (ACT && KS <= 4), "split-K: the 8-wave form (ACT: up to 4 ways)");
   static_assert(!ACT || (NW == 8 && !GOUT && !GF && !CSC && !(LAB & 16)), "ACT: the plain dz form");
   static_assert(RD == 1 || (ACT && RD <= 4), "the deep register ring: the flag-driven form");
@@ -489,9 +490,15 @@
   constexpr int KTB = (KT + KS - 1) / KS;
   constexpr int NPA = ((ACT && KS > 1 ? 2 * PT_ROWS * 4 * KTB : 2 * PT_ROWS * (PT_MAXLD / 8)) + T - 1) / T;
   constexpr int RP = PT_ROWS / (T / 128);
-  constexpr int KTW = NW == 4 ? KTB : (KTB + 1) / 2;
-  __shared__ __attribute__((aligned(16))) uint16_t Gt[2][3 * PT_GPL];
-  __shared__ __attribute__((aligned(16))) uint16_t At[2][2 * PT_APL];
+  constexpr int NC = 128 / SG;
+  constexpr int RG = NC / 32, KG = SG == 1 ? 2 : NW / RG;
+  constexpr int KTW = NW == 4 ? KTB : (KTB + KG - 1) / KG;
+  constexpr int GPL = NC * PT_GP;
+  constexpr int AP = SG == 1 || KTB == 11 ? PT_AP : 32 * KTB + 32, APL = PT_ROWS * AP;
+  constexpr int APAD = SG == 1 || KTB == 11 ? PT_MAXLD : 32 * KTB;
+  static_assert((AP / 2) % 64 == 48 && AP >= APAD + 16, "A tile pitch");
+  __shared__ __attribute__((aligned(16))) uint16_t Gt[2][3 * GPL];
+  __shared__ __attribute__((aligned(16))) uint16_t At[2][2 * APL];
   __shared__ float dzL[2][256];
   __shared__ float redm[2 * NW];
   __shared__ int32_t clist[ACT ? TN_ACT_CAP : 1];
@@ -505,8 +512,18 @@
   const int lane = tid & 63;
   const int wave = tid >> 6;
   const int ld = a.ap_ld;
-  const int kpart = KS == 1 ? 0 : (int)(blockIdx.x % KS);
-  const int rblk = KS == 1 ? (int)blockIdx.x : (int)(blockIdx.x / KS);
+  int kpart = KS == 1 ? 0 : (int)(blockIdx.x % KS);
+  int rblk = KS == 1 ? (int)blockIdx.x : (int)(blockIdx.x / KS);
+  int gpart = 0;
+  if constexpr (SG > 1) {
+    constexpr int NS = SG * KS;
+    const int bid = (int)blockIdx.x;
+    const int sib = a.act_xcd ? (bid % (8 * NS)) / 8 : bid % NS;
+    rblk = a.act_xcd ? bid / (8 * NS) * 8 + bid % 8 : bid / NS;
+    kpart = sib % KS;
+    gpart = sib / KS;
+    if ((int64_t)rblk * a.rows_per_block >= a.M) return;
+  }
   const int kt0 = (kpart * KT + KS - 1) / KS;
   const int ktb = ((kpart + 1) * KT + KS - 1) / KS - kt0;
   const int pr = min(4 * ktb, (ld - 32 * kt0) >> 3);
@@ -534,15 +551,17 @@
     __syncthreads();
     nch = min(n_act, TN_ACT_CAP);
     if (a.slab_empty) {
-      if (kpart == 0 && tid == 0)
+      if (kpart == 0 && gpart == 0 && tid == 0)
         reinterpret_cast<uint32_t*>(a.slab + (int64_t)rblk * a.slab_stride)[a.slab_stride - 1] = nch == 0 ? 1u : 0u;
       if (nch == 0) return;
     }
+    if (SG > 1 && gpart * NC >= a.Nr) return;
   }
   typedef _Float16 f16x8 __attribute__((ext_vector_type(8)));
-  const int wrow = 32 * (wave & 3);
-  const int tbase = NW == 4 ? 0 : (wave >> 2) * KTW;
-  const int ntl = NW == 4 ? KT : max(0, min(KTW, ktb - tbase));
+  const int wrow = 32 * (wave % RG);
+  const int kgi = wave / RG;
+  const int tbase = NW == 4 ? 0 : SG == 1 ? (wave >> 2) * KTW : kgi * (ktb / KG) + min(kgi, ktb % KG);
+  const int ntl = NW == 4 ? KT : SG == 1 ? max(0, min(KTW, ktb - tbase)) : ktb / KG + (kgi < ktb % KG ? 1 : 0);
 
   floatx16 acc[KTW];
 #pragma unroll
@@ -561,12 +580,15 @@
     const int p = q / per_plane, rr = q - p * per_plane;
     const int row = rr / pr, c16 = rr - row * pr;
     goff[j] = ok ? (uint32_t)(((int64_t)p * a.ap_ps + (int64_t)row * ld + 32 * kt0 + 8 * c16) * 2) : 0u;
-    loff[j] = ok ? (uint32_t)((p * PT_APL + row * PT_AP + 8 * c16) * 2)
-                 : (uint32_t)(((tid & 15) * PT_AP + PT_MAXLD + 8 * ((tid >> 4) & 1)) * 2);
-  }
-
-  const int gn = tid & 127, go = tid >> 7;
-  const bool gcol = gn < a.Nr;
+    loff[j] = ok ? (uint32_t)((p * APL + row * AP + 8 * c16) * 2)
+                 : (uint32_t)(((tid & 15) * AP + APAD + 8 * ((tid >> 4) & 1)) * 2);
+  }
+
+  const int gnl = tid % NC, go = SG == 1 ? tid / NC : (tid / NC) & 3;
+  const int gn = gpart * NC + gnl;
+  const bool gact = SG == 1 || tid < 4 * NC;
+  const bool sums = SG == 1 || kpart == 0;
+  const bool gcol = gn < a.Nr && gact;
   const int gnc = gcol ? gn : 0;
   const float* hb = GF ? a.g + gnc : a.h + gnc;
   const int hld = GF ? (int)a.ldg : (int)a.ldh;
@@ -575,6 +597,11 @@
   float pcol[MAXPROJ];
 #pragma unroll
   for (int q = 0; q < MAXPROJ; ++q) pcol[q] = (!GF && q < a.nproj && gcol) ? a.proj[q * a.Nr + gn] : 0.0f;
+  float pall[SG == 1 ? 1 : MAXPROJ] = {};
+  if constexpr (SG > 1) {
+#pragma unroll
+    for (int q = 0; q < MAXPROJ; ++q) pall[q] = (q < a.nproj && (tid & 127) < a.Nr) ? fabsf(a.proj[q * a.Nr + (tid & 127)]) : 0.0f;
+  }
 
   float gsc = 1.f, gunsc = 1.f;
   float zm_fold = 0.f;
@@ -646,7 +673,10 @@
     }
     float pm = 0.f;
 #pragma unroll
-    for (int q = 0; q < MAXPROJ; ++q) pm = fmaxf(pm, fabsf(pcol[q]));
+    for (int q = 0; q < MAXPROJ; ++q) {
+      if constexpr (SG == 1) pm = fmaxf(pm, fabsf(pcol[q]));
+      else pm = fmaxf(pm, pall[q]);
+    }
 #pragma unroll
     for (int o = 32; o > 0; o >>= 1) {
       zm = fmaxf(zm, __shfl_xor(zm, o));
@@ -759,16 +789,18 @@
       g = fmaf(z.y, pcol[1], g);
       g = fmaf(z.z, pcol[2], g);
       e[i] = fmaf(z.w, pcol[3], g);
-      dw2[0] = fmaf(z.x, rg[sg][i], dw2[0]);
-      dw2[1] = fmaf(z.y, rg[sg][i], dw2[1]);
-      dw2[2] = fmaf(z.z, rg[sg][i], dw2[2]);
-      dw2[3] = fmaf(z.w, rg[sg][i], dw2[3]);
+      if (sums) {
+        dw2[0] = fmaf(z.x, rg[sg][i], dw2[0]);
+        dw2[1] = fmaf(z.y, rg[sg][i], dw2[1]);
+        dw2[2] = fmaf(z.z, rg[sg][i], dw2[2]);
+        dw2[3] = fmaf(z.w, rg[sg][i], dw2[3]);
+      }
       return;
     }
     float g = e[i];
-    dzs += gn < MAXPROJ ? zsv[i] : 0.0f;
+    if (sums) dzs += gn < MAXPROJ ? zsv[i] : 0.0f;
     g = rg[sg][i] > 0.0f ? g * a.hscale : 0.0f;
-    db += g;
+    if (sums) db += g;
     if constexpr (GOUT) {
       const int mb = ldbase(c);
       const int r = RP * go + i;
@@ -782,11 +814,11 @@
     w[j][0] = h2_scale_pair(w[j][1], 2048.0f);
   };
   auto g_put = [&](int c) __attribute__((always_inline)) {
-    uint16_t* gd = Gt[c & 1] + gn * PT_GP + RP * go;
+    uint16_t* gd = Gt[c & 1] + gnl * PT_GP + RP * go;
 #pragma unroll
     for (int p = 0; p < 3; ++p) {
-      if constexpr (RP == 8) *reinterpret_cast<uint4*>(gd + p * PT_GPL) = make_uint4(w[0][p], w[1][p], w[2][p], w[3][p]);
-      else *reinterpret_cast<uint2*>(gd + p * PT_GPL) = make_uint2(w[0][p], w[1][p]);
+      if constexpr (RP == 8) *reinterpret_cast<uint4*>(gd + p * GPL) = make_uint4(w[0][p], w[1][p], w[2][p], w[3][p]);
+      else *reinterpret_cast<uint2*>(gd + p * GPL) = make_uint2(w[0][p], w[1][p]);
     }
   };
   auto unit = [&](int k, int c, int par) __attribute__((always_inline)) {
@@ -801,6 +833,7 @@
       } else {
         put_a(sa, k >> 1, c + 1);
       }
+    } else if (k < P0 + 2 && !gact) {
     } else if (k < G0) {
       z_read(c + 1, 2 * (k - Z0), 2);
     } else if (k < S0) {
@@ -825,10 +858,10 @@
 
   const int gfo = (wrow + (lane & 31)) * PT_GP + 8 * (lane >> 5);
   const int grp = lane >> 4, li = lane & 15;
-  const int afo = (8 * (grp >> 1) + (li >> 2)) * PT_AP + 16 * (grp & 1) + 4 * (li & 3);
+  const int afo = (8 * (grp >> 1) + (li >> 2)) * AP + 16 * (grp & 1) + 4 * (li & 3);
   auto afrag = [&](const uint16_t* base, int t, int p) __attribute__((always_inline)) {
-    const uint16_t* q = base + p * PT_APL + t * 32;
-    return __builtin_bit_cast(f16x8, cat_frag(tr_read(q), tr_read(q + 4 * PT_AP)));
+    const uint16_t* q = base + p * APL + t * 32;
+    return __builtin_bit_cast(f16x8, cat_frag(tr_read(q), tr_read(q + 4 * AP)));
   };
 #define TH_FENCE __builtin_amdgcn_sched_barrier(0)
   auto compute = [&](int c, auto parc) __attribute__((always_inline)) {
@@ -842,7 +875,7 @@
     }
     f16x8 gf[3], af[2][2];
 #pragma unroll
-    for (int p = 0; p < 3; ++p) gf[p] = *reinterpret_cast<const f16x8*>(Gt[buf] + p * PT_GPL + gfo);
+    for (int p = 0; p < 3; ++p) gf[p] = *reinterpret_cast<const f16x8*>(Gt[buf] + p * GPL + gfo);
     const uint16_t* ab = At[buf] + afo;
 #pragma unroll
     for (int p = 0; p < 2; ++p) af[0][p] = afrag(ab, tbase, p);
@@ -886,7 +919,7 @@
 #pragma unroll
       for (int j = 0; j < NPA; ++j) load_a(s, j, min(s, clast));
     }
-    load_g(0, 0);
+    if (gact) load_g(0, 0);
 #pragma unroll
     for (int s = 1; s < RGN; ++s) load_g(s, min(s, clast));
     float* dzb = reinterpret_cast<float*>(&At[0][0]) + NW * 2 * 256;
@@ -913,22 +946,24 @@
     scan_scale();
 #pragma unroll
     for (int j = 0; j < NPA; ++j) put_a(0, j, 0);
-    z_read(0, 0, RP);
     if constexpr (ACT) {
       zrange(0, glo, az2hi);
       zrange(1, az2lo, az2hi);
     }
-#pragma unroll
-    for (int i = 0; i < RP; ++i) {
-      g_row(i, 0, 0, 0);
-      g_row(i, 0, 1, 0);
-    }
-#pragma unroll
-    for (int j = 0; j < RP / 2; ++j) split_pair(j);
-    g_put(0);
+    if (gact) {
+      z_read(0, 0, RP);
+#pragma unroll
+      for (int i = 0; i < RP; ++i) {
+        g_row(i, 0, 0, 0);
+        g_row(i, 0, 1, 0);
+      }
+#pragma unroll
+      for (int j = 0; j < RP / 2; ++j) split_pair(j);
+      g_put(0);
+    }
 #pragma unroll
     for (int j = 0; j < NPA; ++j) load_a(0, j, min(RING, clast));
-    load_g(0, min(RGN, clast));
+    if (gact) load_g(0, min(RGN, clast));
     __syncthreads();
     if constexpr (RD == 1) {
       for (int c = 0; c < nch; c += 2) {
@@ -962,7 +997,7 @@
     const bool s2 = kp >= a.ap_col2 && kp < a.ap_col2 + a.k2;
 #pragma unroll
     for (int r = 0; r < 16; ++r) {
-      const int row = wrow + (r & 3) + 8 * (r >> 2) + 4 * (lane >> 5);
+      const int row = gpart * NC + wrow + (r & 3) + 8 * (r >> 2) + 4 * (lane >> 5);
       const int64_t idx = s1 ? (int64_t)row * a.k1 + kp : (int64_t)a.Nr * a.k1 + (int64_t)row * a.k2 + (kp - a.ap_col2);
       if constexpr ((LAB & 128) != 0) {
         if (row < a.Nr && (s1 || s2) && acc[t][r] == 1.2345f) slab[idx] = 0.f;
@@ -971,28 +1006,31 @@
       }
     }
   }
+  if (SG > 1 && kpart != 0) return;
   __syncthreads();
   float* red = reinterpret_cast<float*>(&At[0][0]);
   constexpr int ns = 2 + MAXPROJ;
-  red[(go * 128 + gn) * ns + 0] = db;
-  red[(go * 128 + gn) * ns + 1] = dzs;
-#pragma unroll
-  for (int q = 0; q < MAXPROJ; ++q) red[(go * 128 + gn) * ns + 2 + q] = dw2[q];
+  if (gact) {
+    red[(go * NC + gnl) * ns + 0] = db;
+    red[(go * NC + gnl) * ns + 1] = dzs;
+#pragma unroll
+    for (int q = 0; q < MAXPROJ; ++q) red[(go * NC + gnl) * ns + 2 + q] = dw2[q];
+  }
   __syncthreads();
   constexpr int NGO = T / 128;
   auto comb = [&](int col, int f) __attribute__((always_inline)) {
     float v = red[col * ns + f];
 #pragma unroll
-    for (int o = 1; o < NGO; ++o) v += red[(o * 128 + col) * ns + f];
+    for (int o = 1; o < NGO; ++o) v += red[(o * NC + col) * ns + f];
     return v;
   };
   if (kpart != 0) return;
-  if (tid < 128 && tid < a.Nr) {
+  if (tid < NC && gn < a.Nr) {
     float* side = slab + (int64_t)a.Nr * Kc;
-    side[tid] = comb(tid, 0);
-    for (int q = 0; q < a.nproj; ++q) side[a.Nr + q * a.Nr + tid] = comb(tid, 2 + q);
-  }
-  if (tid < a.nproj) slab[(int64_t)a.Nr * Kc + a.Nr + a.nproj * a.Nr + tid] = comb(tid, 1);
+    side[gn] = comb(tid, 0);
+    for (int q = 0; q < a.nproj; ++q) side[a.Nr + q * a.Nr + gn] = comb(tid, 2 + q);
+  }
+  if (gpart == 0 && tid < a.nproj) slab[(int64_t)a.Nr * Kc + a.Nr + a.nproj * a.Nr + tid] = comb(tid, 1);
 }
 
 template <bool PROJ, bool MASK, int KT, bool GOUT, int D, bool GB = false>
@@ -1283,14 +1321,18 @@
   return (a.M + 32) * ldmax < ((int64_t)1 << 31);
 }
 
-void launch_tn_h2(const TNArgs& a, int nblk, hipStream_t st, bool ks, bool act_split) {
+void launch_tn_h2(const TNArgs& a, int nblk, hipStream_t st, bool ks, bool act_split, bool act_gsplit) {
   if (!a.dz) {
     if (a.ap_ld == 176) gemm_tn_h2_kernel<6, false, 0, 8, true><<<nblk, 512, 0, st>>>(a);
     else gemm_tn_h2_kernel<11, false, 0, 8, true><<<nblk, 512, 0, st>>>(a);
     return;
   }
   if (a.dz_active) {
-    if (act_split) gemm_tn_h2_kernel<11, false, 0, 8, false, TN_ACT_SPLIT, false, true, TN_ACT_RING><<<nblk, 512, 0, st>>>(a);
+    if (act_split && act_gsplit) {
+      TNArgs g = a;
+      g.act_xcd = 1;
+      gemm_tn_h2_kernel<11, false, 0, 8, false, TN_ACT_GSPLIT_K, false, true, 1, TN_ACT_GSPLIT><<<nblk, 512, 0, st>>>(g);
+    } else if (act_split) gemm_tn_h2_kernel<11, false, 0, 8, false, TN_ACT_SPLIT, false, true, TN_ACT_RING><<<nblk, 512, 0, st>>>(a);
     else gemm_tn_h2_kernel<11, false, 0, 8, false, 1, false, true><<<nblk, 512, 0, st>>>(a);
     return;
   }
diff --git a/elliptic_gnn_project_amd/csrc/lab/lab_tn_active.hip b/elliptic_gnn_project_amd/csrc/lab/lab_tn_active.hip
--- a/elliptic_gnn_project_amd/csrc/lab/lab_tn_active.hip
+++ b/elliptic_gnn_project_amd/csrc/lab/lab_tn_active.hip
@@ -39,6 +39,13 @@
 template <int LAB, int KS, int RD>
 void tn(const TNArgs& a) {
   gemm_tn_h2_kernel<11, false, LAB, 8, false, KS, false, true, RD><<<KS * NRB, 512>>>(a);
+}
+template <int LAB, int SG, int KS, bool XCD>
+void tn2(const TNArgs& a0) {
+  TNArgs a = a0;
+  a.act_xcd = XCD;
+  const int nrb = XCD ? (NRB + 7) / 8 * 8 : NRB;
+  gemm_tn_h2_kernel<11, false, LAB, 8, false, KS, false, true, 1, SG><<<SG * KS * nrb, 512>>>(a);
 }
 
 int main(int argc, char** argv) {
@@ -119,6 +126,24 @@
       {"TN split 4 ring 1, empty slabs skipped", tn<0, 4, 1>, true, {}},
       {"TN split 4 ring 1, no MFMA", tn<1, 4, 1>, false, {}, true},
       {"TN split 4 ring 1, no staging", tn<2, 4, 1>, false, {}, true},
+      {"TN 2 x 2", tn2<0, 2, 2, false>, false, {}},
+      {"TN 2 x 2 xcd", tn2<0, 2, 2, true>, false, {}},
+      {"TN 4 x 1", tn2<0, 4, 1, false>, false, {}},
+      {"TN 4 x 1 xcd", tn2<0, 4, 1, true>, false, {}},
+      {"TN 4 x 2", tn2<0, 4, 2, false>, false, {}},
+      {"TN 4 x 2 xcd", tn2<0, 4, 2, true>, false, {}},
+      {"TN 2 x 2, empty slabs skipped", tn2<0, 2, 2, false>, true, {}},
+      {"TN 2 x 2 xcd, empty slabs skipped", tn2<0, 2, 2, true>, true, {}},
+      {"TN 4 x 1, empty slabs skipped", tn2<0, 4, 1, false>, true, {}},
+      {"TN 4 x 1 xcd, empty slabs skipped", tn2<0, 4, 1, true>, true, {}},
+      {"TN 4 x 2, empty slabs skipped", tn2<0, 4, 2, false>, true, {}},
+      {"TN 4 x 2 xcd, empty slabs skipped", tn2<0, 4, 2, true>, true, {}},
+      {"TN 2 x 2, no MFMA", tn2<1, 2, 2, false>, false, {}, true},
+      {"TN 2 x 2, no staging", tn2<2, 2, 2, false>, false, {}, true},
+      {"TN 4 x 1, no MFMA", tn2<1, 4, 1, false>, false, {}, true},
+      {"TN 4 x 1, no staging", tn2<2, 4, 1, false>, false, {}, true},
+      {"TN 4 x 2, no MFMA", tn2<1, 4, 2, false>, false, {}, true},
+      {"TN 4 x 2, no staging", tn2<2, 4, 2, false>, false, {}, true},
   };
   const size_t nsl = (size_t)NRB * stride;
   std::vector<float> r0(nsl), r1(nsl);
diff --git a/include/gnnmp.h b/include/gnnmp.h
--- a/include/gnnmp.h
+++ b/include/gnnmp.h
@@ -305,6 +305,7 @@
 int gnn_gemm_tn_active_pays(int64_t M);
 int gnn_gemm_tn_active_split(void);
 int gnn_gemm_tn_active_ring(void);
+int gnn_gemm_tn_active_gsplit(void);
 gnn_status gnn_gemm_tn_sq_blocks(int64_t n_out, int32_t* nb);
 int gnn_gemm_nt_planes_ok(const gnn_gemm_nt_params* p);
 int gnn_gemm_tn_planes_ok(const gnn_gemm_tn_params* p);
```
